# Roy-Shubhajit/FIT-GNN

Hardware: NVIDIA B200
Metric: subgraph-inference nodes/sec (higher is better)
Workload: dtype fp16 planes for every operand of the two wide transforms (aggregated features, hidden state, weights: 1 MMA per product), fp16 hidden state x fp16 hi/lo weights (2 MMAs) in the head; f32 accumulate

## Files before the change

fitgnn_b200/_lib.py:

```python
from __future__ import annotations

import ctypes as C
import os

_HERE = os.path.dirname(os.path.abspath(__file__))
LIB_PATH = os.environ.get("FITGNN_B200_LIB", os.path.join(_HERE, "libfitgnn_b200.so"))

c_i64, c_i32, c_void, c_size = C.c_int64, C.c_int, C.c_void_p, C.c_size_t


class FitgnnError(RuntimeError):
    pass


class PackStruct(C.Structure):
    _fields_ = [("n_rows", c_i64), ("nnz", c_i64), ("n_sub", c_i64), ("n_core", c_i64), ("n_src", c_i64),
                ("rowptr", c_void), ("col", c_void), ("dinv", c_void), ("gid", c_void), ("sub_ptr", c_void),
                ("core_rows", c_void), ("is_core", c_void), ("mask", c_void)]


class WeightsStruct(C.Structure):
    _fields_ = [("n_layers", C.c_int), ("in_features", C.c_int), ("hidden", C.c_int), ("n_classes", C.c_int),
                ("conv_weight", C.POINTER(c_void)), ("conv_bias", C.POINTER(c_void)), ("lt1_weight", c_void),
                ("lt1_bias", c_void)]


class PlanStruct(C.Structure):
    _fields_ = [("n_rows", c_i64), ("nnz", c_i64), ("n_sub", c_i64), ("n_core", c_i64), ("n_src", c_i64),
                ("fill_ws_bytes", c_i64), ("priv", c_i64 * 27)]


SIGNATURES = {
    "fitgnn_abi_version": (c_i32, []),
    "fitgnn_last_error": (c_i32, [C.c_char_p, c_size]),
    "fitgnn_device_info": (c_i32, [C.POINTER(c_i32), C.POINTER(c_i32)]),
    "fitgnn_tuning_set": (c_i32, [C.c_char_p, c_i32]),
    "fitgnn_tuning_get": (c_i32, [C.c_char_p, C.POINTER(c_i32)]),
    "fitgnn_csr_workspace_bytes": (c_size, [c_i64, c_i64]),
    "fitgnn_csr_plan": (c_i32, [c_void, c_i64, c_i64, c_void, c_size, C.POINTER(c_i64), c_void]),
    "fitgnn_csr_fill": (c_i32, [c_i64, c_void, c_size, c_void, c_void, c_void, c_void]),
    "fitgnn_pack_workspace_bytes": (c_size, [c_i64, c_i64, c_i64, c_i32, c_i64]),
    "fitgnn_pack_plan": (c_i32, [c_void, c_i64, c_i64, c_void, c_i64, c_i32, c_void, c_void, c_i64, c_void, c_size,
                                 C.POINTER(PlanStruct), c_void]),
    "fitgnn_pack_fill": (c_i32, [C.POINTER(PlanStruct), C.POINTER(PackStruct), c_void, c_size, c_void, c_size, c_void]),
    "fitgnn_spmm_symnorm": (c_i32, [c_void, c_void, c_void, c_void, c_i64, c_i32, c_void, c_void, c_i32, c_void, c_i64,
                                    c_void, c_void, c_i64, c_void]),
    "fitgnn_spmm_symnorm_grouped": (c_i32, [c_void, c_void, c_void, c_void, c_i64, c_i32, c_void, c_i64, c_i32, c_void,
                                            c_void, c_i64, c_i32, C.c_float, c_void]),
    "fitgnn_spmm_symnorm_grouped_f16": (c_i32, [c_void, c_void, c_void, c_void, c_i64, c_i32, c_void, c_i64, c_i32, c_void,
                                                c_i64, c_i32, C.c_float, c_void]),
    "fitgnn_spmm_symnorm_blocked": (c_i32, [c_void, c_void, c_void, c_void, c_i64, c_i32, c_void, c_void, c_i64, c_void,
                                            c_void, c_i32, c_void, c_void, c_i64, c_void]),
    "fitgnn_spmm_symnorm_mma": (c_i32, [c_void, c_void, c_void, c_void, c_i64, c_i32, c_void, c_void, c_i64, c_void,
                                        c_i32, c_void, c_void, c_i64, c_void]),
    "fitgnn_spmm_hubs": (c_i32, [c_void, c_void, c_i64, c_i32, c_void, c_void, c_i32, c_void]),
    "fitgnn_spmm_symnorm_hub": (c_i32, [c_void, c_void, c_void, c_void, c_i64, c_i32, c_void, c_void, c_i32, c_void,
                                        c_i64, c_void, c_void, c_i64, c_void, c_i32, c_i32, c_void]),
    "fitgnn_spmm_symnorm_devhub": (c_i32, [c_void, c_void, c_void, c_void, c_i64, c_i32, c_void, c_void, c_i32, c_void,
                                           c_i64, c_void, c_void, c_i64, c_void, c_void, c_i32, c_i32, c_void]),
    "fitgnn_gcn_forward_workspace_bytes": (c_size, [C.POINTER(PackStruct), C.POINTER(WeightsStruct), c_i32]),
    "fitgnn_gcn_forward": (c_i32, [C.POINTER(PackStruct), c_void, c_i64, C.POINTER(WeightsStruct), c_i32, c_i32, c_void,
                                   c_i64, c_void, c_size, c_void]),
    "fitgnn_gemm_tn_workspace_bytes": (c_size, [c_i64, c_i32, c_i32]),
    "fitgnn_gemm_tn": (c_i32, [c_void, c_i64, c_void, c_i64, c_i64, c_i32, c_i32, c_void, c_i64, c_void, c_size, c_void]),
    "fitgnn_dropout": (c_i32, [c_void, c_i64, c_i64, c_i32, C.c_float, C.c_uint64, C.c_uint64, c_void, c_i64, c_void]),
    "fitgnn_elu_dropout_backward": (c_i32, [c_void, c_i64, c_void, c_i64, c_i64, c_i32, c_i32, C.c_float, C.c_uint64,
                                            C.c_uint64, c_void, c_i64, c_void]),
    "fitgnn_adam_step": (c_i32, [c_void, c_void, c_void, c_void, c_i64, C.c_float, C.c_float, C.c_float, C.c_float,
                                 C.c_float, c_i64, c_void]),
    "fitgnn_spmm_symnorm_f16": (c_i32, [c_void, c_void, c_void, c_void, c_i64, c_i32, c_void, c_void, c_i32, c_void, c_i64,
                                        c_void, c_i64, c_void, c_void, c_i32, c_i32, c_void]),
    "fitgnn_split_f16": (c_i32, [c_void, c_i64, c_i64, c_i32, c_void, c_void, c_i64, c_void]),
    "fitgnn_gemm_f16": (c_i32, [c_void, c_i64, c_void, c_void, c_i64, c_void, c_void, c_i64, c_i32, c_i32, c_i32, c_i32, c_void,
                                c_i64, c_i32, c_void, c_void]),
    "fitgnn_gemm_f16_head_rows_peers": (c_i32, [c_void, c_i64, c_void, c_void, c_i64, c_void, c_i64, c_i32, c_i32, c_i32, c_i32,
                                                c_void, C.POINTER(c_void), c_i32, c_i64, c_void]),
    "fitgnn_gcn_transform_aggregate_f16": (c_i32, [c_i32, c_void, c_void, c_i64, c_void, c_void, c_i64, c_void, c_i64, c_i32,
                                                   c_i32, c_i32, c_void, c_void, c_i32, c_void, c_i64, c_void]),
    "fitgnn_gcn_conv_aligned_f16": (c_i32, [c_void, c_i64, c_void, c_void, c_i64, c_void, c_i64, c_i32, c_i32, c_i32, c_void, c_void,
                                            c_void, c_i64, c_void]),
    "fitgnn_gemm_bias_act": (c_i32, [c_i32, c_void, c_void, c_i64, c_void, c_void, c_i64, c_void, c_i64, c_i32, c_i32,
                                     c_i32, c_i32, c_void, c_i64, c_void]),
    "fitgnn_gemm_bias_act_split": (c_i32, [c_i32, c_void, c_void, c_i64, c_void, c_void, c_i64, c_void, c_i64, c_i32,
                                           c_i32, c_i32, c_i32, c_void, c_void, c_i64, c_void]),
    "fitgnn_gcn_layer_fused": (c_i32, [c_void, c_void, c_void, c_void, c_i64, c_i32, c_void, c_void, c_i64, c_void, c_void,
                                       c_i64, c_void, c_i32, c_i32, c_void, c_void, c_i64, c_void]),
    "fitgnn_pack_align_workspace_bytes": (c_size, [c_i64, c_i64]),
    "fitgnn_pack_align_plan": (c_i32, [C.POINTER(PackStruct), c_i32, c_i32, c_void, C.POINTER(c_i64), C.POINTER(c_i32),
                                       c_void, c_size, c_void]),
    "fitgnn_pack_align_fill": (c_i32, [C.POINTER(PackStruct), c_void, c_i32, c_i64, C.POINTER(PackStruct), c_void, c_void,
                                       c_void, C.POINTER(c_i32), c_void, c_size, c_void]),
    "fitgnn_gcn_transform_aggregate": (c_i32, [c_void, c_void, c_i64, c_void, c_void, c_i64, c_void, c_i64, c_i32, c_i32,
                                               c_i32, c_void, c_void, c_i32, c_void, c_void, c_i64, c_void]),
    "fitgnn_gemm_rowscale_bias_act_split": (c_i32, [c_i32, c_void, c_void, c_i64, c_void, c_void, c_i64, c_void, c_void, c_i64,
                                                    c_i32, c_i32, c_i32, c_i32, c_void, c_void, c_i64, c_void]),
    "fitgnn_gemm_head_rows": (c_i32, [c_void, c_void, c_i64, c_void, c_void, c_i64, c_void, c_i64, c_i32, c_i32, c_i32,
                                      c_i32, c_void, c_void, c_i64, c_void]),
    "fitgnn_gemm_head_rows_peers": (c_i32, [c_void, c_void, c_i64, c_void, c_void, c_i64, c_void, c_i64, c_i32, c_i32, c_i32,
                                            c_i32, c_void, C.POINTER(c_void), c_i32, c_i64, c_void]),
    "fitgnn_peer_push": (c_i32, [c_void, C.POINTER(c_void), c_i32, c_size, c_i32, c_void]),
    "fitgnn_peer_alloc": (c_i32, [c_size, C.POINTER(c_void), C.c_char_p]),
    "fitgnn_peer_open": (c_i32, [C.c_char_p, C.POINTER(c_void)]),
    "fitgnn_peer_close": (c_i32, [c_void]),
    "fitgnn_peer_free": (c_i32, [c_void]),
    "fitgnn_split_bf16": (c_i32, [c_void, c_i64, c_i64, c_i32, c_void, c_void, c_i64, c_void]),
    "fitgnn_segment_pool": (c_i32, [c_void, c_i64, c_i32, c_void, c_void, c_i64, c_i32, c_void, c_i64, c_void]),
    "fitgnn_group_workspace_bytes": (c_size, [c_i64, c_i64]),
    "fitgnn_group_by_part": (c_i32, [c_void, c_i64, c_i64, c_void, c_void, c_void, c_size, c_void]),
    "fitgnn_project_features": (c_i32, [c_void, c_void, c_i64, c_void, c_void, c_i64, c_i32, c_void, c_i64, c_void]),
    "fitgnn_project_adj_workspace_bytes": (c_size, [c_i64]),
    "fitgnn_project_adj_plan": (c_i32, [c_void, c_i64, c_i64, c_void, c_i64, c_void, c_size, C.POINTER(c_i64), c_void]),
    "fitgnn_project_adj_fill": (c_i32, [c_void, c_size, c_i64, c_void, c_void, c_void, c_void, c_void]),
    "fitgnn_sort_workspace_bytes": (c_size, [c_i64]),
    "fitgnn_sort_u64": (c_i32, [c_void, c_void, c_i64, c_i32, c_void, c_size, c_void]),
    "fitgnn_scan_i32": (c_i32, [c_void, c_void, c_i64, c_i32, c_void, c_size, c_void]),
    "fitgnn_scan_workspace_bytes": (c_size, [c_i64]),
}

_lib = None


def lib():
    global _lib
    if _lib is None:
        if not os.path.exists(LIB_PATH):
            raise FitgnnError(
                f"{LIB_PATH} is missing: build it with `python -c 'import __graft_entry__ as g; g.build()'` "
                "(or `make -C fitgnn_b200/csrc`). fitgnn_b200 has no CPU fallback.")
        handle = C.CDLL(LIB_PATH)
        for name, (res, args) in SIGNATURES.items():
            fn = getattr(handle, name)
            fn.restype, fn.argtypes = res, args
        if handle.fitgnn_abi_version() != 1:
            raise FitgnnError("libfitgnn_b200.so ABI version mismatch")
        _lib = handle
    return _lib


def last_error() -> str:
    buf = C.create_string_buffer(512)
    lib().fitgnn_last_error(buf, 512)
    return buf.value.decode(errors="replace")


def set_tuning(name: str, value: int) -> int:
    old = C.c_int(0)
    check(lib().fitgnn_tuning_get(name.encode(), C.byref(old)))
    check(lib().fitgnn_tuning_set(name.encode(), int(value)))
    return old.value


_CODES = {-1: "EINVAL", -2: "ECUDA", -3: "ERANGE", -4: "EWS", -5: "EUNSUP"}


def check(rc: int):
    if rc != 0:
        raise FitgnnError(f"fitgnn {_CODES.get(rc, rc)}: {last_error()}")


def ptr(t):
    if t is None:
        return None
    if not t.is_cuda:
        raise FitgnnError("fitgnn_b200 kernels take CUDA tensors only (there is no CPU path)")
    if not t.is_contiguous():
        raise FitgnnError("tensor must be contiguous")
    return C.c_void_p(t.data_ptr())


def stream_ptr():
    import torch
    return C.c_void_p(torch.cuda.current_stream().cuda_stream)
```

fitgnn_b200/csrc/capi.cu:

```cuda
#include <stdarg.h>
#include <stdio.h>
#include <stdlib.h>
#include <string.h>
#include "common.cuh"

namespace fitgnn {

static thread_local char g_err[512] = "";

void set_error(const char* fmt, ...) {
  va_list ap;
  va_start(ap, fmt);
  vsnprintf(g_err, sizeof(g_err), fmt, ap);
  va_end(ap);
}

int sm_count() {
  static int cached[64] = {};
  int dev = 0;
  if (cudaGetDevice(&dev) != cudaSuccess || dev < 0 || dev >= 64) return 148;
  if (!cached[dev]) {
    int n = 0;
    if (cudaDeviceGetAttribute(&n, cudaDevAttrMultiProcessorCount, dev) != cudaSuccess || n <= 0) n = 148;
    cached[dev] = n;
  }
  return cached[dev];
}

static int env_int(const char* name, int dflt) {
  const char* e = getenv(name);
  return (e && e[0]) ? atoi(e) : dflt;
}
static Tuning& tuning_mut() {
  static Tuning t{env_int("FITGNN_GEMM_WS", 1),   getenv("FITGNN_HEAD_BULK") ? 0 : 1, env_int("FITGNN_AGG_WIDE", 0),
                  env_int("FITGNN_GEMM_WIDE", 0), env_int("FITGNN_GEMM_PAIR", 1), env_int("FITGNN_SM_RESERVE", 0),
                  env_int("FITGNN_GEMM_PAIR_WS", 1), 0, env_int("FITGNN_GEMM_PREFETCH", 0)};
  return t;
}
const Tuning& tuning() { return tuning_mut(); }
static int* tuning_field(const char* name) {
  Tuning& t = tuning_mut();
  if (!name) return nullptr;
  if (!strcmp(name, "gemm_ws")) return &t.gemm_ws;
  if (!strcmp(name, "head_bulk")) return &t.head_bulk;
  if (!strcmp(name, "agg_wide")) return &t.agg_wide;
  if (!strcmp(name, "gemm_wide")) return &t.gemm_wide;
  if (!strcmp(name, "gemm_pair")) return &t.gemm_pair;
  if (!strcmp(name, "sm_reserve")) return &t.sm_reserve;
  if (!strcmp(name, "gemm_pair_ws")) return &t.gemm_pair_ws;
  if (!strcmp(name, "gemm_prefetch")) return &t.gemm_prefetch;
  if (!strcmp(name, "gemm_debug")) return &t.gemm_debug;
  return nullptr;
}

int gemm_fp32(const float* A, int64_t lda, const float* W, int64_t ldw, const float* bias, int64_t M, int K, int N,
              int act, float* Y, int64_t ldy, cudaStream_t st);
int row_softmax(float* Y, int64_t ldy, int64_t M, int N, int head, cudaStream_t st);
int gemm_bf16x3(const void* A_hi, const void* A_lo, int64_t lda, const void* W_hi, const void* W_lo, int64_t ldw,
                const float* bias, int64_t M, int K, int N, int act, int head, float* Y, void* Y_lo, int64_t ldy,
                const uint64_t* agg_desc, const float* agg_dinv, const int32_t* row_map, float* const* peers, int n_peers,
                const float* row_scale, int agg_defer_scale, cudaStream_t st, int64_t m_batch_rows = 0, int w_batch_rows = 0,
                int64_t w_rows_total = 0, int in_f16 = 0, int out_f16 = 0, int agg_pre = 0);

int gcn_layer_fused(const int32_t* rowptr, const int32_t* col, const float* dinv, const float* X, int64_t ldx, int width,
                    const int32_t* src_index, const int32_t* out_rows, int64_t M, const void* W_hi, const void* W_lo,
                    int64_t ldw, const float* bias, int N, int act, float* Y, void* Y_lo, int64_t ldy, cudaStream_t st);

}

using namespace fitgnn;

extern "C" int fitgnn_abi_version(void) { return FITGNN_ABI_VERSION; }

extern "C" int fitgnn_last_error(char* buf, size_t n) {
  const size_t len = strlen(g_err);
  if (buf && n > 0) {
    const size_t c = len < n - 1 ? len : n - 1;
    memcpy(buf, g_err, c);
    buf[c] = 0;
  }
  return (int)len;
}

extern "C" int fitgnn_tuning_set(const char* name, int value) {
  int* f = tuning_field(name);
  FG_REQUIRE(f, FITGNN_EINVAL, "tuning_set: unknown switch '%s'", name ? name : "(null)");
  *f = value;
  return FITGNN_OK;
}
extern "C" int fitgnn_tuning_get(const char* name, int* value) {
  int* f = tuning_field(name);
  FG_REQUIRE(f && value, FITGNN_EINVAL, "tuning_get: unknown switch '%s'", name ? name : "(null)");
  *value = *f;
  return FITGNN_OK;
}

extern "C" int fitgnn_device_info(int* sm_count, int* cc) {
  int dev = 0;
  FG_CUDA(cudaGetDevice(&dev));
  cudaDeviceProp p;
  FG_CUDA(cudaGetDeviceProperties(&p, dev));
  if (sm_count) *sm_count = p.multiProcessorCount;
  if (cc) *cc = p.major * 10 + p.minor;
  return FITGNN_OK;
}

extern "C" int fitgnn_gemm_rowscale_bias_act_split(int precision, const void* A, const void* A_lo, int64_t lda,
                                                   const void* W, const void* W_lo, int64_t ldw, const float* row_scale,
                                                   const float* bias, int64_t M, int K, int N, int act, int head, void* Yv,
                                                   void* Y_lo, int64_t ldy, void* stream) {
  float* Y = static_cast<float*>(Yv);
  FG_REQUIRE(!row_scale || precision == FITGNN_GEMM_BF16X3, FITGNN_EUNSUP, "gemm: row_scale needs FITGNN_GEMM_BF16X3");
  FG_REQUIRE(A && W && Y && M >= 0 && K > 0 && N > 0, FITGNN_EINVAL, "gemm: bad arguments (M=%lld K=%d N=%d)",
             (long long)M, K, N);
  FG_REQUIRE(lda >= K && ldw >= K && ldy >= N, FITGNN_EINVAL, "gemm: leading dimension smaller than the extent");
  FG_REQUIRE(act == FITGNN_ACT_NONE || act == FITGNN_ACT_ELU, FITGNN_EINVAL, "gemm: unknown act %d", act);
  FG_REQUIRE(head >= FITGNN_HEAD_IDENTITY && head <= FITGNN_HEAD_SOFTMAX, FITGNN_EINVAL, "gemm: unknown head %d", head);
  if (M == 0) return FITGNN_OK;
  cudaStream_t st = as_stream(stream);
  if (precision == FITGNN_GEMM_FP32) {
    FG_REQUIRE(!Y_lo, FITGNN_EUNSUP, "gemm: bf16 hi/lo output planes need FITGNN_GEMM_BF16X3");
    FG_TRY(gemm_fp32(static_cast<const float*>(A), lda, static_cast<const float*>(W), ldw, bias, M, K, N, act, Y, ldy,
                     st));
    return row_softmax(Y, ldy, M, N, head, st);
  }
  if (precision == FITGNN_GEMM_BF16X3) {
    FG_REQUIRE(A_lo && W_lo, FITGNN_EINVAL, "gemm: BF16X3 needs the lo planes");
    return gemm_bf16x3(A, A_lo, lda, W, W_lo, ldw, bias, M, K, N, act, head, Y, Y_lo, ldy, nullptr, nullptr, nullptr, nullptr, 0,
                       row_scale, 0, st);
  }
  set_error("gemm: unknown precision %d", precision);
  return FITGNN_EINVAL;
}

extern "C" int fitgnn_gemm_bias_act_split(int precision, const void* A, const void* A_lo, int64_t lda, const void* W,
                                          const void* W_lo, int64_t ldw, const float* bias, int64_t M, int K, int N,
                                          int act, int head, void* Yv, void* Y_lo, int64_t ldy, void* stream) {
  return fitgnn_gemm_rowscale_bias_act_split(precision, A, A_lo, lda, W, W_lo, ldw, nullptr, bias, M, K, N, act, head, Yv, Y_lo,
                                             ldy, stream);
}

extern "C" int fitgnn_gcn_transform_aggregate(const void* A_hi, const void* A_lo, int64_t lda, const void* W_hi,
                                              const void* W_lo, int64_t ldw, const float* bias, int64_t M, int K, int N,
                                              int act, const uint64_t* agg_desc, const float* dinv, int defer_row_scale,
                                              void* Y, void* Y_lo, int64_t ldy, void* stream) {
  FG_REQUIRE(A_hi && A_lo && W_hi && W_lo && Y && agg_desc && dinv && M >= 0 && K > 0 && N > 0, FITGNN_EINVAL,
             "gcn_transform_aggregate: bad arguments (M=%lld K=%d N=%d)", (long long)M, K, N);
  FG_REQUIRE(lda >= K && ldw >= K && ldy >= N, FITGNN_EINVAL, "gcn_transform_aggregate: leading dimension too small");
  FG_REQUIRE(act == FITGNN_ACT_NONE || act == FITGNN_ACT_ELU, FITGNN_EINVAL, "gcn_transform_aggregate: unknown act %d", act);
  if (M == 0) return FITGNN_OK;
  return gemm_bf16x3(A_hi, A_lo, lda, W_hi, W_lo, ldw, bias, M, K, N, act, FITGNN_HEAD_IDENTITY, static_cast<float*>(Y),
                     Y_lo, ldy, agg_desc, dinv, nullptr, nullptr, 0, nullptr, defer_row_scale, as_stream(stream));
}

extern "C" int fitgnn_gemm_head_rows(const void* A_hi, const void* A_lo, int64_t lda, const void* W_hi, const void* W_lo,
                                     int64_t ldw, const float* bias, int64_t M, int K, int N, int act, int head,
                                     const int32_t* row_map, float* Y, int64_t ldy, void* stream) {
  FG_REQUIRE(A_hi && A_lo && W_hi && W_lo && Y && row_map && M >= 0 && K > 0 && N > 0, FITGNN_EINVAL,
             "gemm_head_rows: bad arguments (M=%lld K=%d N=%d)", (long long)M, K, N);
  FG_REQUIRE(lda >= K && ldw >= K && ldy >= N, FITGNN_EINVAL, "gemm_head_rows: leading dimension too small");
  FG_REQUIRE(act == FITGNN_ACT_NONE || act == FITGNN_ACT_ELU, FITGNN_EINVAL, "gemm_head_rows: unknown act %d", act);
  FG_REQUIRE(head >= FITGNN_HEAD_IDENTITY && head <= FITGNN_HEAD_SOFTMAX, FITGNN_EINVAL, "gemm_head_rows: unknown head %d",
             head);
  if (M == 0) return FITGNN_OK;
  return gemm_bf16x3(A_hi, A_lo, lda, W_hi, W_lo, ldw, bias, M, K, N, act, head, Y, nullptr, ldy, nullptr, nullptr,
                     row_map, nullptr, 0, nullptr, 0, as_stream(stream));
}

extern "C" int fitgnn_gemm_head_rows_peers(const void* A_hi, const void* A_lo, int64_t lda, const void* W_hi,
                                           const void* W_lo, int64_t ldw, const float* bias, int64_t M, int K, int N,
                                           int act, int head, const int32_t* row_map, float* const* host_peer_bases,
                                           int n_peers, int64_t ldy, void* stream) {
  FG_REQUIRE(A_hi && A_lo && W_hi && W_lo && row_map && host_peer_bases && M >= 0 && K > 0 && N > 0, FITGNN_EINVAL,
             "gemm_head_rows_peers: bad arguments (M=%lld K=%d N=%d)", (long long)M, K, N);
  FG_REQUIRE(n_peers >= 1 && n_peers <= 8, FITGNN_EINVAL, "gemm_head_rows_peers: 1..8 peers (got %d)", n_peers);
  for (int p = 0; p < n_peers; ++p)
    FG_REQUIRE(host_peer_bases[p], FITGNN_EINVAL, "gemm_head_rows_peers: peer base %d is null", p);
  FG_REQUIRE(lda >= K && ldw >= K && ldy >= N, FITGNN_EINVAL, "gemm_head_rows_peers: leading dimension too small");
  FG_REQUIRE(act == FITGNN_ACT_NONE || act == FITGNN_ACT_ELU, FITGNN_EINVAL, "gemm_head_rows_peers: unknown act %d", act);
  FG_REQUIRE(head >= FITGNN_HEAD_IDENTITY && head <= FITGNN_HEAD_SOFTMAX, FITGNN_EINVAL,
             "gemm_head_rows_peers: unknown head %d", head);
  if (M == 0) return FITGNN_OK;
  return gemm_bf16x3(A_hi, A_lo, lda, W_hi, W_lo, ldw, bias, M, K, N, act, head, nullptr, nullptr, ldy, nullptr, nullptr,
                     row_map, host_peer_bases, n_peers, nullptr, 0, as_stream(stream));
}

extern "C" int fitgnn_gemm_bias_act(int precision, const void* A, const void* A_lo, int64_t lda, const void* W,
                                    const void* W_lo, int64_t ldw, const float* bias, int64_t M, int K, int N, int act,
                                    int head, float* Y, int64_t ldy, void* stream) {
  return fitgnn_gemm_bias_act_split(precision, A, A_lo, lda, W, W_lo, ldw, bias, M, K, N, act, head, Y, nullptr, ldy,
                                    stream);
}

extern "C" int fitgnn_gcn_layer_fused(const int32_t* rowptr, const int32_t* col, const float* dinv, const float* X,
                                      int64_t ldx, int width, const int32_t* src_index, const int32_t* out_rows,
                                      int64_t n_out, const void* W_hi, const void* W_lo, int64_t ldw, const float* bias,
                                      int N, int act, void* Y, void* Y_lo, int64_t ldy, void* stream) {
  FG_REQUIRE(rowptr && col && dinv && X && W_hi && W_lo && Y && n_out >= 0 && N > 0 && width > 0, FITGNN_EINVAL,
             "gcn_layer_fused: bad arguments");
  FG_REQUIRE(act == FITGNN_ACT_NONE || act == FITGNN_ACT_ELU, FITGNN_EINVAL, "gcn_layer_fused: unknown act %d", act);
  if (n_out == 0) return FITGNN_OK;
  return gcn_layer_fused(rowptr, col, dinv, X, ldx, width, src_index, out_rows, n_out, W_hi, W_lo, ldw, bias, N, act,
                         static_cast<float*>(Y), Y_lo, ldy, as_stream(stream));
}

extern "C" int fitgnn_gemm_f16(const void* A, int64_t lda, const void* W_hi, const void* W_lo, int64_t ldw,
                               const float* row_scale, const float* bias, int64_t M, int K, int N, int act, int head, void* Y,
                               int64_t ldy, int out_f16, const int32_t* row_map, void* stream) {
  FG_REQUIRE(A && W_hi && Y && M >= 0 && K > 0 && N > 0, FITGNN_EINVAL, "gemm_f16: bad arguments (M=%lld K=%d N=%d)",
             (long long)M, K, N);
  FG_REQUIRE(lda >= K && ldw >= K && ldy >= N, FITGNN_EINVAL, "gemm_f16: leading dimension smaller than the extent");
  FG_REQUIRE(act == FITGNN_ACT_NONE || act == FITGNN_ACT_ELU, FITGNN_EINVAL, "gemm_f16: unknown act %d", act);
  FG_REQUIRE(head >= FITGNN_HEAD_IDENTITY && head <= FITGNN_HEAD_SOFTMAX, FITGNN_EINVAL, "gemm_f16: unknown head %d", head);
  if (M == 0) return FITGNN_OK;
  return gemm_bf16x3(A, nullptr, lda, W_hi, W_lo, ldw, bias, M, K, N, act, head, static_cast<float*>(Y), nullptr, ldy, nullptr,
                     nullptr, row_map, nullptr, 0, row_scale, 0, as_stream(stream), 0, 0, 0, 1, out_f16 ? 1 : 0);
}

extern "C" int fitgnn_gcn_transform_aggregate_f16(int in_f16, const void* A_hi, const void* A_lo, int64_t lda, const void* W_hi,
                                                  const void* W_lo, int64_t ldw, const float* bias, int64_t M, int K, int N,
                                                  int act, const uint64_t* agg_desc, const float* dinv, int defer_row_scale,
                                                  void* Y, int64_t ldy, void* stream) {
  FG_REQUIRE(A_hi && W_hi && (W_lo || in_f16) && Y && (!agg_desc || dinv) && M >= 0 && K > 0 && N > 0, FITGNN_EINVAL,
             "gcn_transform_aggregate_f16: bad arguments (M=%lld K=%d N=%d)", (long long)M, K, N);
  FG_REQUIRE(in_f16 ? !A_lo : A_lo != nullptr, FITGNN_EINVAL, "gcn_transform_aggregate_f16: A_lo must match in_f16");
  FG_REQUIRE(lda >= K && ldw >= K && ldy >= N, FITGNN_EINVAL, "gcn_transform_aggregate_f16: leading dimension too small");
  FG_REQUIRE(act == FITGNN_ACT_NONE || act == FITGNN_ACT_ELU, FITGNN_EINVAL, "gcn_transform_aggregate_f16: unknown act %d", act);
  if (M == 0) return FITGNN_OK;
  return gemm_bf16x3(A_hi, A_lo, lda, W_hi, W_lo, ldw, bias, M, K, N, act, FITGNN_HEAD_IDENTITY, static_cast<float*>(Y), nullptr,
                     ldy, agg_desc, agg_desc ? dinv : nullptr, nullptr, nullptr, 0, nullptr, agg_desc ? defer_row_scale : 0,
                     as_stream(stream), 0, 0, 0, in_f16 ? 1 : 0, 1);
}

extern "C" int fitgnn_gcn_conv_aligned_f16(const void* A, int64_t lda, const void* W_hi, const void* W_lo, int64_t ldw,
                                           const float* bias, int64_t M, int K, int N, int act, const uint64_t* agg_desc,
                                           const float* dinv, void* Y, int64_t ldy, void* stream) {
  FG_REQUIRE(A && W_hi && Y && agg_desc && dinv && M >= 0 && K > 0 && N > 0, FITGNN_EINVAL,
             "gcn_conv_aligned_f16: bad arguments (M=%lld K=%d N=%d)", (long long)M, K, N);
  FG_REQUIRE(lda >= K && ldw >= K && ldy >= N, FITGNN_EINVAL, "gcn_conv_aligned_f16: leading dimension too small");
  FG_REQUIRE(act == FITGNN_ACT_NONE || act == FITGNN_ACT_ELU, FITGNN_EINVAL, "gcn_conv_aligned_f16: unknown act %d", act);
  if (M == 0) return FITGNN_OK;
  return gemm_bf16x3(A, nullptr, lda, W_hi, W_lo, ldw, bias, M, K, N, act, FITGNN_HEAD_IDENTITY, static_cast<float*>(Y), nullptr,
                     ldy, agg_desc, dinv, nullptr, nullptr, 0, dinv, 1, as_stream(stream), 0, 0, 0, 1, 1, 1);
}

extern "C" int fitgnn_gemm_f16_head_rows_peers(const void* A, int64_t lda, const void* W_hi, const void* W_lo, int64_t ldw,
                                               const float* bias, int64_t M, int K, int N, int act, int head,
                                               const int32_t* row_map, float* const* host_peer_bases, int n_peers, int64_t ldy,
                                               void* stream) {
  FG_REQUIRE(A && W_hi && W_lo && row_map && host_peer_bases && M >= 0 && K > 0 && N > 0, FITGNN_EINVAL,
             "gemm_f16_head_rows_peers: bad arguments (M=%lld K=%d N=%d)", (long long)M, K, N);
  FG_REQUIRE(n_peers >= 1 && n_peers <= 8, FITGNN_EINVAL, "gemm_f16_head_rows_peers: 1..8 peers (got %d)", n_peers);
  for (int p = 0; p < n_peers; ++p)
    FG_REQUIRE(host_peer_bases[p], FITGNN_EINVAL, "gemm_f16_head_rows_peers: peer base %d is null", p);
  FG_REQUIRE(lda >= K && ldw >= K && ldy >= N, FITGNN_EINVAL, "gemm_f16_head_rows_peers: leading dimension too small");
  FG_REQUIRE(act == FITGNN_ACT_NONE || act == FITGNN_ACT_ELU, FITGNN_EINVAL, "gemm_f16_head_rows_peers: unknown act %d", act);
  FG_REQUIRE(head >= FITGNN_HEAD_IDENTITY && head <= FITGNN_HEAD_SOFTMAX, FITGNN_EINVAL,
             "gemm_f16_head_rows_peers: unknown head %d", head);
  if (M == 0) return FITGNN_OK;
  return gemm_bf16x3(A, nullptr, lda, W_hi, W_lo, ldw, bias, M, K, N, act, head, nullptr, nullptr, ldy, nullptr, nullptr, row_map,
                     host_peer_bases, n_peers, nullptr, 0, as_stream(stream), 0, 0, 0, 1, 0);
}
```

fitgnn_b200/csrc/gemm_tcgen05.cu:

```cuda
#include <cuda.h>
#include <stdio.h>
#include <stdlib.h>
#include <cuda_bf16.h>
#include <type_traits>
#include "common.cuh"

namespace fitgnn {

namespace tc {

constexpr int BLOCK_M = 128;
constexpr int BLOCK_K = 64;
constexpr int UMMA_K = 16;
constexpr int EPI_WARPS = 8;
constexpr int EPI_WARPS_WIDE = 16;
constexpr int EPI_WARPS_12 = 12;
constexpr int THREADS = 64 + 32 * EPI_WARPS;
constexpr int GATHER_WARPS = 4;
constexpr int GATHER_WARP0 = 2 + EPI_WARPS;
constexpr int THREADS_GATHER = THREADS + 32 * GATHER_WARPS;

struct GatherArgs {
  const int32_t* rowptr;
  const int32_t* col;
  const float* dinv;
  const float* X;
  const int32_t* src_index;
  const int32_t* out_rows;
  int64_t ldx;
  int nq;
};
struct EpiArgs {
  const unsigned long long* agg_desc;
  const float* agg_dinv;
  const int32_t* row_map;
  float* peers[8];
  int n_peers;
  int bulk_rows;
  const float* row_scale;
  int agg_defer_scale;
  int64_t m_batch_rows;
  int w_batch_rows;
  int64_t w_rows_total;
  int a_planes;
  int f16;
  int out_f16;
  int w_planes;
  int l2_prefetch;
  int debug;
};
constexpr int EPI_WARP0 = 2;
constexpr int ACC_STAGES = 2;
constexpr uint32_t A_PLANE_BYTES = BLOCK_M * BLOCK_K * 2;
constexpr long long WAIT_BUDGET_CYCLES = 4000000000ll;

__device__ __forceinline__ uint32_t smem_u32(const void* p) { return (uint32_t)__cvta_generic_to_shared(p); }

__device__ __forceinline__ void mbar_init(uint32_t bar, uint32_t count) {
  asm volatile("mbarrier.init.shared::cta.b64 [%0], %1;" ::"r"(bar), "r"(count));
}
__device__ __forceinline__ void mbar_arrive(uint32_t bar) {
  asm volatile("mbarrier.arrive.shared::cta.b64 _, [%0];" ::"r"(bar) : "memory");
}
__device__ __forceinline__ void mbar_arrive_expect_tx(uint32_t bar, uint32_t bytes) {
  asm volatile("mbarrier.arrive.expect_tx.shared::cta.b64 _, [%0], %1;" ::"r"(bar), "r"(bytes) : "memory");
}
__device__ __forceinline__ bool mbar_try_wait(uint32_t bar, uint32_t parity) {
  uint32_t ok;
  asm volatile(
      "{\n\t.reg .pred p;\n\t"
      "mbarrier.try_wait.parity.shared::cta.b64 p, [%1], %2;\n\t"
      "selp.u32 %0, 1, 0, p;\n\t}"
      : "=r"(ok)
      : "r"(bar), "r"(parity)
      : "memory");
  return ok != 0;
}
__device__ __forceinline__ void mbar_wait(uint32_t bar, uint32_t parity) {
  if (mbar_try_wait(bar, parity)) return;
  const long long t0 = clock64();
  while (!mbar_try_wait(bar, parity)) {
    if (clock64() - t0 > WAIT_BUDGET_CYCLES) {
      printf("fitgnn gemm_bf16x3: mbarrier wait timed out (block %d thread %d)\n", blockIdx.x, threadIdx.x);
      __trap();
    }
  }
}

__device__ __forceinline__ void tma_load_2d(uint32_t dst, const CUtensorMap* map, uint32_t bar, int c0, int c1) {
  asm volatile(
      "cp.async.bulk.tensor.2d.shared::cluster.global.mbarrier::complete_tx::bytes [%0], [%1, {%3, %4}], [%2];"
      ::"r"(dst), "l"(map), "r"(bar), "r"(c0), "r"(c1)
      : "memory");
}

__device__ __forceinline__ void tma_prefetch_2d(const CUtensorMap* map, int c0, int c1) {
  asm volatile("cp.async.bulk.prefetch.tensor.2d.L2.global [%0, {%1, %2}];" ::"l"(map), "r"(c0), "r"(c1) : "memory");
}

__device__ __forceinline__ void tma_store_2d(const CUtensorMap* map, uint32_t src, int c0, int c1) {
  asm volatile("cp.async.bulk.tensor.2d.global.shared::cta.bulk_group [%0, {%2, %3}], [%1];" ::"l"(map), "r"(src),
               "r"(c0), "r"(c1)
               : "memory");
}
__device__ __forceinline__ void bulk_store_1d(void* dst, uint32_t src, uint32_t bytes) {
  asm volatile("cp.async.bulk.global.shared::cta.bulk_group [%0], [%1], %2;" ::"l"(dst), "r"(src), "r"(bytes) : "memory");
}
__device__ __forceinline__ void bulk_commit() { asm volatile("cp.async.bulk.commit_group;" ::: "memory"); }
template <int N>
__device__ __forceinline__ void bulk_wait_read() {
  asm volatile("cp.async.bulk.wait_group.read %0;" ::"n"(N) : "memory");
}
__device__ __forceinline__ void bulk_wait_all() { asm volatile("cp.async.bulk.wait_group 0;" ::: "memory"); }
__device__ __forceinline__ void fence_proxy_async() { asm volatile("fence.proxy.async.shared::cta;" ::: "memory"); }

__device__ __forceinline__ uint64_t umma_desc_sw128(uint32_t smem_addr) {
  uint64_t d = 0;
  d |= (uint64_t)((smem_addr & 0x3FFFFu) >> 4);
  d |= (uint64_t)0 << 16;
  d |= (uint64_t)(1024u >> 4) << 32;
  d |= (uint64_t)1 << 46;
  d |= (uint64_t)2 << 61;
  return d;
}

__host__ __device__ constexpr uint32_t umma_idesc_bf16(int m, int n) {
  return (1u << 4) | (1u << 7) | (1u << 10) | ((uint32_t)(n >> 3) << 17) | ((uint32_t)(m >> 4) << 24);
}

__host__ __device__ constexpr uint32_t umma_idesc_f16(int m, int n) {
  return (1u << 4) | ((uint32_t)(n >> 3) << 17) | ((uint32_t)(m >> 4) << 24);
}

__device__ __forceinline__ void umma_bf16(uint32_t tmem_d, uint64_t a_desc, uint64_t b_desc, uint32_t idesc,
                                          uint32_t accumulate) {
  asm volatile(
      "{\n\t.reg .pred p;\n\t"
      "setp.ne.b32 p, %4, 0;\n\t"
      "tcgen05.mma.cta_group::1.kind::f16 [%0], %1, %2, %3, p;\n\t}"
      ::"r"(tmem_d), "l"(a_desc), "l"(b_desc), "r"(idesc), "r"(accumulate)
      : "memory");
}
__device__ __forceinline__ uint32_t cluster_ctarank() {
  uint32_t r;
  asm volatile("mov.u32 %0, %%cluster_ctarank;" : "=r"(r));
  return r;
}
__device__ __forceinline__ uint32_t mapa_rank(uint32_t local_addr, uint32_t rank) {
  uint32_t r;
  asm volatile("mapa.shared::cluster.u32 %0, %1, %2;" : "=r"(r) : "r"(local_addr), "r"(rank));
  return r;
}
__device__ __forceinline__ void cluster_sync_all() {
  asm volatile("barrier.cluster.arrive.release.aligned;" ::: "memory");
  asm volatile("barrier.cluster.wait.acquire.aligned;" ::: "memory");
}
__device__ __forceinline__ void tma_load_2d_pair(uint32_t dst, const CUtensorMap* map, uint32_t leader_bar, int c0, int c1) {
  asm volatile(
      "cp.async.bulk.tensor.2d.cta_group::2.shared::cluster.global.mbarrier::complete_tx::bytes [%0], [%1, {%3, %4}], [%2];"
      ::"r"(dst), "l"(map), "r"(leader_bar), "r"(c0), "r"(c1)
      : "memory");
}
__device__ __forceinline__ void umma_bf16_pair(uint32_t tmem_d, uint64_t a_desc, uint64_t b_desc, uint32_t idesc,
                                               uint32_t accumulate) {
  asm volatile(
      "{\n\t.reg .pred p;\n\t"
      "setp.ne.b32 p, %4, 0;\n\t"
      "tcgen05.mma.cta_group::2.kind::f16 [%0], %1, %2, %3, p;\n\t}"
      ::"r"(tmem_d), "l"(a_desc), "l"(b_desc), "r"(idesc), "r"(accumulate)
      : "memory");
}
__device__ __forceinline__ void umma_commit_pair(uint32_t bar) {
  const uint16_t mask = 3;
  asm volatile("tcgen05.commit.cta_group::2.mbarrier::arrive::one.shared::cluster.multicast::cluster.b64 [%0], %1;" ::"r"(bar),
               "h"(mask)
               : "memory");
}
__device__ __forceinline__ void mbar_arrive_remote(uint32_t cluster_addr) {
  asm volatile("mbarrier.arrive.shared::cluster.b64 _, [%0];" ::"r"(cluster_addr) : "memory");
}
__device__ __forceinline__ bool elect_one() {
  uint32_t pred;
  asm volatile("{\n\t.reg .pred p;\n\telect.sync _|p, 0xffffffff;\n\tselp.b32 %0, 1, 0, p;\n\t}" : "=r"(pred));
  return pred != 0;
}
__device__ __forceinline__ void umma_commit(uint32_t bar) {
  asm volatile("tcgen05.commit.cta_group::1.mbarrier::arrive::one.shared::cluster.b64 [%0];" ::"r"(bar) : "memory");
}
__device__ __forceinline__ void tmem_ld16(uint32_t taddr, float (&v)[16]) {
  uint32_t r[16];
  asm volatile(
      "tcgen05.ld.sync.aligned.32x32b.x16.b32 {%0,%1,%2,%3,%4,%5,%6,%7,%8,%9,%10,%11,%12,%13,%14,%15}, [%16];"
      : "=r"(r[0]), "=r"(r[1]), "=r"(r[2]), "=r"(r[3]), "=r"(r[4]), "=r"(r[5]), "=r"(r[6]), "=r"(r[7]), "=r"(r[8]),
        "=r"(r[9]), "=r"(r[10]), "=r"(r[11]), "=r"(r[12]), "=r"(r[13]), "=r"(r[14]), "=r"(r[15])
      : "r"(taddr));
  asm volatile("tcgen05.wait::ld.sync.aligned;" ::: "memory");
#pragma unroll
  for (int i = 0; i < 16; ++i) v[i] = __uint_as_float(r[i]);
}
__device__ __forceinline__ void tmem_ld32(uint32_t taddr, float (&v)[32]) {
  uint32_t r[32];
  asm volatile(
      "tcgen05.ld.sync.aligned.32x32b.x32.b32 {%0,%1,%2,%3,%4,%5,%6,%7,%8,%9,%10,%11,%12,%13,%14,%15,%16,%17,%18,%19,"
      "%20,%21,%22,%23,%24,%25,%26,%27,%28,%29,%30,%31}, [%32];"
      : "=r"(r[0]), "=r"(r[1]), "=r"(r[2]), "=r"(r[3]), "=r"(r[4]), "=r"(r[5]), "=r"(r[6]), "=r"(r[7]), "=r"(r[8]),
        "=r"(r[9]), "=r"(r[10]), "=r"(r[11]), "=r"(r[12]), "=r"(r[13]), "=r"(r[14]), "=r"(r[15]), "=r"(r[16]),
        "=r"(r[17]), "=r"(r[18]), "=r"(r[19]), "=r"(r[20]), "=r"(r[21]), "=r"(r[22]), "=r"(r[23]), "=r"(r[24]),
        "=r"(r[25]), "=r"(r[26]), "=r"(r[27]), "=r"(r[28]), "=r"(r[29]), "=r"(r[30]), "=r"(r[31])
      : "r"(taddr));
  asm volatile("tcgen05.wait::ld.sync.aligned;" ::: "memory");
#pragma unroll
  for (int i = 0; i < 32; ++i) v[i] = __uint_as_float(r[i]);
}
__device__ __forceinline__ void tmem_ld32_issue(uint32_t taddr, uint32_t (&r)[32]) {
  asm volatile(
      "tcgen05.ld.sync.aligned.32x32b.x32.b32 {%0,%1,%2,%3,%4,%5,%6,%7,%8,%9,%10,%11,%12,%13,%14,%15,%16,%17,%18,%19,"
      "%20,%21,%22,%23,%24,%25,%26,%27,%28,%29,%30,%31}, [%32];"
      : "=r"(r[0]), "=r"(r[1]), "=r"(r[2]), "=r"(r[3]), "=r"(r[4]), "=r"(r[5]), "=r"(r[6]), "=r"(r[7]), "=r"(r[8]),
        "=r"(r[9]), "=r"(r[10]), "=r"(r[11]), "=r"(r[12]), "=r"(r[13]), "=r"(r[14]), "=r"(r[15]), "=r"(r[16]),
        "=r"(r[17]), "=r"(r[18]), "=r"(r[19]), "=r"(r[20]), "=r"(r[21]), "=r"(r[22]), "=r"(r[23]), "=r"(r[24]),
        "=r"(r[25]), "=r"(r[26]), "=r"(r[27]), "=r"(r[28]), "=r"(r[29]), "=r"(r[30]), "=r"(r[31])
      : "r"(taddr));
}
__device__ __forceinline__ void tmem_ld32_wait(uint32_t (&r)[32]) {
  asm volatile("tcgen05.wait::ld.sync.aligned;"
               : "+r"(r[0]), "+r"(r[1]), "+r"(r[2]), "+r"(r[3]), "+r"(r[4]), "+r"(r[5]), "+r"(r[6]), "+r"(r[7]), "+r"(r[8]),
                 "+r"(r[9]), "+r"(r[10]), "+r"(r[11]), "+r"(r[12]), "+r"(r[13]), "+r"(r[14]), "+r"(r[15]), "+r"(r[16]),
                 "+r"(r[17]), "+r"(r[18]), "+r"(r[19]), "+r"(r[20]), "+r"(r[21]), "+r"(r[22]), "+r"(r[23]), "+r"(r[24]),
                 "+r"(r[25]), "+r"(r[26]), "+r"(r[27]), "+r"(r[28]), "+r"(r[29]), "+r"(r[30]), "+r"(r[31])
               :
               : "memory");
}
__device__ __forceinline__ void fence_before() { asm volatile("tcgen05.fence::before_thread_sync;" ::: "memory"); }
__device__ __forceinline__ void fence_after() { asm volatile("tcgen05.fence::after_thread_sync;" ::: "memory"); }

__device__ __forceinline__ float elu1(float x) { return elu_fast(x); }

__host__ __device__ constexpr int tmem_cols(int n) { return n <= 32 ? 32 : n <= 64 ? 64 : n <= 128 ? 128 : n <= 256 ? 256 : 512; }
__host__ __device__ constexpr uint32_t stage_bytes(int block_n) { return 2 * A_PLANE_BYTES + 2 * (uint32_t)block_n * BLOCK_K * 2; }
constexpr uint32_t EPI_BOX_BYTES = 32 * 32 * 4;
__host__ __device__ constexpr int num_stages(int block_n) {
  int s = (int)((192 * 1024) / stage_bytes(block_n));
  return s > 8 ? 8 : s;
}

template <int BLOCK_N, bool GATHER, int AGG, int EW, bool CTA2 = false>
__global__ void __launch_bounds__(64 + 32 * EW + (GATHER ? 32 * GATHER_WARPS : 0), 1)
gemm_bf16x3_kernel(const GatherArgs ga, const EpiArgs ea, const __grid_constant__ CUtensorMap map_a_hi, const __grid_constant__ CUtensorMap map_a_lo,
                   const __grid_constant__ CUtensorMap map_w_hi, const __grid_constant__ CUtensorMap map_w_lo,
                   const __grid_constant__ CUtensorMap map_y, const __grid_constant__ CUtensorMap map_y_lo,
                   int tma_store, const float* __restrict__ bias, int64_t M, int K, int N, int act, int head,
                   float* __restrict__ Y, int64_t ldy, int w_stationary, int n_stages) {
  constexpr int STAGES = num_stages(BLOCK_N);
  constexpr int MAX_STAGES = 8;
  constexpr int B_ROWS = CTA2 ? BLOCK_N / 2 : BLOCK_N;
  constexpr uint32_t B_PLANE_BYTES = (uint32_t)B_ROWS * BLOCK_K * 2;
  constexpr int TMEM_COLS = tmem_cols(ACC_STAGES * BLOCK_N);
  constexpr uint32_t IDESC_BF16 = umma_idesc_bf16(CTA2 ? 2 * BLOCK_M : BLOCK_M, BLOCK_N);
  constexpr uint32_t IDESC_F16 = umma_idesc_f16(CTA2 ? 2 * BLOCK_M : BLOCK_M, BLOCK_N);
  const uint32_t IDESC = ea.f16 ? IDESC_F16 : IDESC_BF16;
  const bool a_single = ea.a_planes == 1;
  const bool w_single = ea.w_planes == 1;
  static_assert(!CTA2 || (!GATHER && BLOCK_N % 32 == 0), "CTA pairs: streaming plan, UMMA N multiple of 32 for M=256");
  const uint32_t cta_rank = CTA2 ? cluster_ctarank() : 0u;
  const bool leader = cta_rank == 0;
  static_assert(BLOCK_N % 16 == 0 && BLOCK_N >= 16 && BLOCK_N <= 256, "UMMA N for M=128");
  static_assert(STAGES >= 2, "need at least two smem stages");
  static_assert(EW == EPI_WARPS || (EW == EPI_WARPS_WIDE && !GATHER) || (EW == EPI_WARPS_12 && !GATHER && BLOCK_N == 256),
                "2, 3 (256-column tile with an fp16-plane output) or 4 epilogue warps per TMEM lane quadrant");
  constexpr bool HALF_STAGE = BLOCK_N == 256 && (EW == EPI_WARPS_12 || (AGG && EW == EPI_WARPS_WIDE));
  const uint32_t WARP_STAGE = (HALF_STAGE || (CTA2 && ea.out_f16)) ? EPI_BOX_BYTES / 2 : EPI_BOX_BYTES;
  const uint32_t STAGING_BYTES = EW * WARP_STAGE;

  extern __shared__ uint8_t smem_raw[];
  uint8_t* smem = reinterpret_cast<uint8_t*>(((uintptr_t)smem_raw + 1023) & ~(uintptr_t)1023);
  const int k_blocks = (K + BLOCK_K - 1) / BLOCK_K;
  const uint32_t b_bytes = (w_single ? 1u : 2u) * B_PLANE_BYTES;
  const uint32_t w_region_bytes = w_stationary ? (uint32_t)k_blocks * b_bytes : 0u;
  const uint32_t a_bytes = (a_single ? 1u : 2u) * A_PLANE_BYTES;
  const uint32_t stage_bytes_rt = w_stationary ? a_bytes : a_bytes + b_bytes;
  uint8_t* staging = smem + w_region_bytes + (size_t)n_stages * stage_bytes_rt;
  uint64_t* bars = reinterpret_cast<uint64_t*>(staging + STAGING_BYTES);
  uint32_t* tmem_slot = reinterpret_cast<uint32_t*>(bars + 2 * MAX_STAGES + 2 * ACC_STAGES + 1);
  const uint32_t smem_base = smem_u32(smem) + w_region_bytes;
  const uint32_t w_base = smem_u32(smem);
  const uint32_t bar_base = smem_u32(bars);
  auto full_bar = [&](int s) { return bar_base + 8u * s; };
  auto empty_bar = [&](int s) { return bar_base + 8u * (MAX_STAGES + s); };
  auto tfull_bar = [&](int s) { return bar_base + 8u * (2 * MAX_STAGES + s); };
  auto tempty_bar = [&](int s) { return bar_base + 8u * (2 * MAX_STAGES + ACC_STAGES + s); };
  const uint32_t wfull_bar = bar_base + 8u * (2 * MAX_STAGES + 2 * ACC_STAGES);

  const int warp = threadIdx.x >> 5, lane = threadIdx.x & 31;
  const int n_tiles = (N + BLOCK_N - 1) / BLOCK_N;
  constexpr int TILE_M = CTA2 ? 2 * BLOCK_M : BLOCK_M;
  const int64_t m_tiles = (M + TILE_M - 1) / TILE_M;
  const int64_t tiles = m_tiles * n_tiles;
  struct Walk { int mb, nt; };
  const int ctas_per_n = (int)gridDim.x / n_tiles;
  Walk w0;
  int walk_dm, walk_dn, walk_carry;
  if (CTA2) {
    const int p = (int)(blockIdx.x >> 1), np = (int)(gridDim.x >> 1);
    if (w_stationary) { w0 = Walk{p / n_tiles, p % n_tiles}; walk_dm = np / n_tiles; walk_dn = 0; walk_carry = 0; }
    else { w0 = Walk{p, 0}; walk_dm = 0; walk_dn = 1; walk_carry = np; }
  } else if (w_stationary) {
    w0 = Walk{(int)blockIdx.x / n_tiles, (int)blockIdx.x % n_tiles}; walk_dm = ctas_per_n; walk_dn = 0; walk_carry = 0;
  } else {
    w0 = Walk{(int)blockIdx.x / n_tiles, (int)blockIdx.x % n_tiles};
    walk_dm = (int)gridDim.x / n_tiles; walk_dn = (int)gridDim.x % n_tiles; walk_carry = 1;
  }
  auto advance = [&](Walk& w) {
    w.nt += walk_dn;
    w.mb += walk_dm;
    if (w.nt >= n_tiles) { w.nt -= n_tiles; w.mb += walk_carry; }
  };
  auto valid = [&](const Walk& w) { return (int64_t)w.mb < m_tiles; };
  auto tile_row0 = [&](const Walk& w) { return (int64_t)w.mb * TILE_M + (int64_t)cta_rank * BLOCK_M; };
  auto w_batch_off = [&](const Walk& w) -> int {
    return ea.m_batch_rows ? (int)(((int64_t)w.mb * TILE_M) / ea.m_batch_rows) * ea.w_batch_rows : 0;
  };
  const int64_t t_first = blockIdx.x;
  const int64_t t_step = (int64_t)ctas_per_n * n_tiles;

  if (warp == 0 && lane == 0) {
    for (int s = 0; s < n_stages; ++s) {
      mbar_init(full_bar(s), GATHER ? GATHER_WARPS : 1);
      mbar_init(empty_bar(s), 1);
    }
    mbar_init(wfull_bar, 1);
    for (int s = 0; s < ACC_STAGES; ++s) {
      mbar_init(tfull_bar(s), 1);
      mbar_init(tempty_bar(s), CTA2 ? 2 * EW : EW);
    }
    asm volatile("fence.mbarrier_init.release.cluster;" ::: "memory");
  }
  if (warp == 1) {
    if (CTA2) {
      asm volatile("tcgen05.alloc.cta_group::2.sync.aligned.shared::cta.b32 [%0], %1;" ::"r"(smem_u32(tmem_slot)),
                   "r"((uint32_t)TMEM_COLS)
                   : "memory");
      asm volatile("tcgen05.relinquish_alloc_permit.cta_group::2.sync.aligned;" ::: "memory");
    } else {
      asm volatile("tcgen05.alloc.cta_group::1.sync.aligned.shared::cta.b32 [%0], %1;" ::"r"(smem_u32(tmem_slot)),
                   "r"((uint32_t)TMEM_COLS)
                   : "memory");
      asm volatile("tcgen05.relinquish_alloc_permit.cta_group::1.sync.aligned;" ::: "memory");
    }
  }
  fence_before();
  __syncthreads();
  if (CTA2) cluster_sync_all();
  fence_after();
  const uint32_t tmem_base = *tmem_slot;

  if (warp == 0) {
    {
      uint32_t stage = 0, phase = 0;
      if (w_stationary && valid(w0)) {
        const int n0 = w0.nt * BLOCK_N;
        if (elect_one()) {
          if (CTA2) {
            const uint32_t lbar = mapa_rank(wfull_bar, 0);
            if (leader) mbar_arrive_expect_tx(wfull_bar, 2 * w_region_bytes);
            for (int kb = 0; kb < k_blocks; ++kb) {
              tma_load_2d_pair(w_base + kb * b_bytes, &map_w_hi, lbar, kb * BLOCK_K, n0 + (int)cta_rank * B_ROWS);
              if (!w_single)
                tma_load_2d_pair(w_base + kb * b_bytes + B_PLANE_BYTES, &map_w_lo, lbar, kb * BLOCK_K, n0 + (int)cta_rank * B_ROWS);
            }
          } else {
            mbar_arrive_expect_tx(wfull_bar, w_region_bytes);
            for (int kb = 0; kb < k_blocks; ++kb) {
              tma_load_2d(w_base + kb * b_bytes, &map_w_hi, wfull_bar, kb * BLOCK_K, n0);
              if (!w_single) tma_load_2d(w_base + kb * b_bytes + B_PLANE_BYTES, &map_w_lo, wfull_bar, kb * BLOCK_K, n0);
            }
          }
        }
        __syncwarp();
      }
      int prev_mb = -1;
      for (Walk w = w0; valid(w) && !GATHER; advance(w)) {
        const int m0 = (int)tile_row0(w);
        const int n0 = w.nt * BLOCK_N + w_batch_off(w);
        int pf_m0 = -1;
        if (w.mb != prev_mb) {
          Walk pf = w;
          for (int i = 0; i < n_tiles && valid(pf) && pf.mb == w.mb; ++i) advance(pf);
          if (valid(pf) && pf.mb != w.mb) pf_m0 = (int)tile_row0(pf);
        }
        prev_mb = w.mb;
        for (int kb = 0; kb < k_blocks; ++kb) {
          if (pf_m0 >= 0 && ea.l2_prefetch) {
            if (elect_one()) {
              tma_prefetch_2d(&map_a_hi, kb * BLOCK_K, pf_m0);
              if (!a_single) tma_prefetch_2d(&map_a_lo, kb * BLOCK_K, pf_m0);
            }
            __syncwarp();
          }
          mbar_wait(empty_bar(stage), phase ^ 1);
          const uint32_t dst = smem_base + stage * stage_bytes_rt;
          const uint32_t tx_bytes = stage_bytes_rt;
          __syncwarp();
          if (elect_one()) {
            if (CTA2) {
              const uint32_t lbar = mapa_rank(full_bar(stage), 0);
              if (leader) mbar_arrive_expect_tx(full_bar(stage), 2 * tx_bytes);
              tma_load_2d_pair(dst, &map_a_hi, lbar, kb * BLOCK_K, m0);
              if (!a_single) tma_load_2d_pair(dst + A_PLANE_BYTES, &map_a_lo, lbar, kb * BLOCK_K, m0);
              if (!w_stationary) {
                tma_load_2d_pair(dst + a_bytes, &map_w_hi, lbar, kb * BLOCK_K, n0 + (int)cta_rank * B_ROWS);
                if (!w_single)
                  tma_load_2d_pair(dst + a_bytes + B_PLANE_BYTES, &map_w_lo, lbar, kb * BLOCK_K, n0 + (int)cta_rank * B_ROWS);
              }
            } else {
              mbar_arrive_expect_tx(full_bar(stage), tx_bytes);
              tma_load_2d(dst, &map_a_hi, full_bar(stage), kb * BLOCK_K, m0);
              if (!a_single) tma_load_2d(dst + A_PLANE_BYTES, &map_a_lo, full_bar(stage), kb * BLOCK_K, m0);
              if (!w_stationary) {
                tma_load_2d(dst + a_bytes, &map_w_hi, full_bar(stage), kb * BLOCK_K, n0);
                if (!w_single) tma_load_2d(dst + a_bytes + B_PLANE_BYTES, &map_w_lo, full_bar(stage), kb * BLOCK_K, n0);
              }
            }
          }
          __syncwarp();
          if (++stage == (uint32_t)n_stages) { stage = 0; phase ^= 1; }
        }
      }
    }
  } else if (warp == 1) {
    auto mma_loop = [&](auto a1_t, auto w1_t) {
      constexpr bool A1 = decltype(a1_t)::value, W1 = decltype(w1_t)::value;
      uint32_t stage = 0, phase = 0;
      uint32_t it = 0;
      if (w_stationary && valid(w0)) mbar_wait(wfull_bar, 0);
      for (Walk w = w0; valid(w); ++it, advance(w)) {
        const uint32_t acc = it % ACC_STAGES;
        const uint32_t acc_phase = (it / ACC_STAGES) & 1u;
        mbar_wait(tempty_bar(acc), acc_phase ^ 1);
        fence_after();
        const uint32_t tmem_d = tmem_base + acc * BLOCK_N;
        for (int kb = 0; kb < k_blocks; ++kb) {
          mbar_wait(full_bar(stage), phase);
          fence_after();
          const uint32_t a_hi = smem_base + stage * stage_bytes_rt;
          const uint32_t w_hi = w_stationary ? w_base + kb * b_bytes : a_hi + a_bytes;
          const uint64_t d_a_hi = umma_desc_sw128(a_hi);
          const uint64_t d_a_lo = umma_desc_sw128(a_hi + A_PLANE_BYTES);
          const uint64_t d_w_hi = umma_desc_sw128(w_hi);
          const uint64_t d_w_lo = umma_desc_sw128(w_hi + B_PLANE_BYTES);
          __syncwarp();
          if (elect_one()) {
#pragma unroll
            for (int k = 0; k < BLOCK_K / UMMA_K; ++k) {
              const uint64_t adv = (uint64_t)((k * UMMA_K * 2) >> 4);
              if (CTA2) {
                umma_bf16_pair(tmem_d, d_a_hi + adv, d_w_hi + adv, IDESC, (kb | k) != 0);
                if (!A1) umma_bf16_pair(tmem_d, d_a_lo + adv, d_w_hi + adv, IDESC, 1);
                if (!W1) umma_bf16_pair(tmem_d, d_a_hi + adv, d_w_lo + adv, IDESC, 1);
              } else {
                umma_bf16(tmem_d, d_a_hi + adv, d_w_hi + adv, IDESC, (kb | k) != 0);
                if (!A1) umma_bf16(tmem_d, d_a_lo + adv, d_w_hi + adv, IDESC, 1);
                if (!W1) umma_bf16(tmem_d, d_a_hi + adv, d_w_lo + adv, IDESC, 1);
              }
            }
            if (CTA2) {
              umma_commit_pair(empty_bar(stage));
              if (kb == k_blocks - 1) umma_commit_pair(tfull_bar(acc));
            } else {
              umma_commit(empty_bar(stage));
              if (kb == k_blocks - 1) umma_commit(tfull_bar(acc));
            }
          }
          __syncwarp();
          if (++stage == (uint32_t)n_stages) { stage = 0; phase ^= 1; }
        }
      }
    };
    if (leader) {
      if (a_single && w_single) mma_loop(std::true_type{}, std::true_type{});
      else if (a_single) mma_loop(std::true_type{}, std::false_type{});
      else mma_loop(std::false_type{}, std::false_type{});
    }
    __syncwarp();
  } else if (GATHER && warp >= GATHER_WARP0) {
    constexpr int LPR = 8, STEPS = BLOCK_M / (GATHER_WARPS * 4);
    constexpr unsigned FULL = 0xffffffffu;
    const int gw = warp - GATHER_WARP0, sub = lane & (LPR - 1), grp = lane / LPR;
    const int64_t my_tiles = (t_first < tiles) ? (tiles - 1 - t_first) / t_step + 1 : 0;
    const int64_t total_steps = my_tiles * STEPS;
    struct RI { int beg, end; float dr; };
    auto load_info = [&](int64_t step) {
      RI ri{0, 0, 0.f};
      if (step < total_steps) {
        const int64_t t = t_first + (step / STEPS) * t_step;
        const int64_t i = (t / n_tiles) * BLOCK_M + gw * 32 + (int)(step % STEPS) * 4 + grp;
        if (i < M) {
          const int r = ga.out_rows ? __ldg(ga.out_rows + i) : (int)i;
          ri.beg = __ldg(ga.rowptr + r);
          ri.end = __ldg(ga.rowptr + r + 1);
          ri.dr = __ldg(ga.dinv + r);
        }
      }
      return ri;
    };
    auto load_col = [&](const RI& ri, int e0) { return (e0 + sub < ri.end) ? __ldg(ga.col + e0 + sub) : -1; };
    auto load_w = [&](int c) { return c >= 0 ? __ldg(ga.dinv + c) : 0.f; };
    auto load_s = [&](int c) { return c >= 0 ? (ga.src_index ? __ldg(ga.src_index + c) : c) : 0; };
    auto gather_chunk = [&](float4 (&acc)[4], int cnt, float w, int sidx) {
      const int maxcnt = __reduce_max_sync(FULL, cnt);
      for (int j = 0; j < maxcnt; j += 2) {
        float wj[2];
        const float* pj[2];
        bool on[2];
#pragma unroll
        for (int u = 0; u < 2; ++u) {
          wj[u] = __shfl_sync(FULL, w, j + u, LPR);
          const int sj = __shfl_sync(FULL, sidx, j + u, LPR);
          pj[u] = ga.X + (int64_t)sj * ga.ldx;
          on[u] = j + u < cnt;
        }
        float4 x[2][4];
#pragma unroll
        for (int u = 0; u < 2; ++u)
#pragma unroll
          for (int v = 0; v < 4; ++v) {
            const int q = sub + LPR * v;
            x[u][v] = (on[u] && q < ga.nq) ? __ldg(reinterpret_cast<const float4*>(pj[u]) + q) : make_float4(0.f, 0.f, 0.f, 0.f);
          }
#pragma unroll
        for (int u = 0; u < 2; ++u)
#pragma unroll
          for (int v = 0; v < 4; ++v) {
            acc[v].x = fmaf(wj[u], x[u][v].x, acc[v].x); acc[v].y = fmaf(wj[u], x[u][v].y, acc[v].y);
            acc[v].z = fmaf(wj[u], x[u][v].z, acc[v].z); acc[v].w = fmaf(wj[u], x[u][v].w, acc[v].w);
          }
      }
    };
    RI ia = load_info(0), ib = load_info(1), ic = load_info(2);
    int ca = load_col(ia, ia.beg), cb = load_col(ib, ib.beg);
    float wa = load_w(ca);
    int sa = load_s(ca);
    uint32_t stage = 0, phase = 0;
    for (int64_t step = 0; step < total_steps; ++step) {
      const RI id = load_info(step + 3);
      const int cc = load_col(ic, ic.beg);
      const float wb = load_w(cb);
      const int sb = load_s(cb);
      const int s_in_tile = (int)(step % STEPS);
      if (s_in_tile == 0) {
        if (lane == 0)
          for (int kb = 0; kb < k_blocks; ++kb) mbar_wait(empty_bar(stage + kb), phase ^ 1);
        __syncwarp();
      }
      const int deg = ia.end - ia.beg;
      float4 acc[4];
#pragma unroll
      for (int v = 0; v < 4; ++v) acc[v] = make_float4(0.f, 0.f, 0.f, 0.f);
      gather_chunk(acc, min(deg, LPR), wa, sa);
      const bool long_row = deg > LPR;
      for (int e0 = ia.beg + LPR; __any_sync(FULL, long_row && e0 < ia.end); e0 += LPR) {
        const int c = long_row ? load_col(ia, e0) : -1;
        gather_chunk(acc, long_row ? max(0, min(ia.end - e0, LPR)) : 0, load_w(c), load_s(c));
      }
      const int lr = gw * 32 + s_in_tile * 4 + grp;
#pragma unroll
      for (int v = 0; v < 4; ++v) {
        const int c = 4 * (sub + LPR * v);
        const int kb = c >> 6;
        if (kb < k_blocks) {
          const float x[4] = {acc[v].x * ia.dr, acc[v].y * ia.dr, acc[v].z * ia.dr, acc[v].w * ia.dr};
          uint32_t hi[2], lo[2];
#pragma unroll
          for (int u = 0; u < 2; ++u) split_bf16x2(x[2 * u], x[2 * u + 1], hi[u], lo[u]);
          const int cc64 = c & 63;
          const uint32_t a = smem_base + (stage + kb) * stage_bytes_rt + lr * 128 +
                             ((uint32_t)(cc64 >> 3) ^ (uint32_t)(lr & 7)) * 16 + ((cc64 & 7) >> 2) * 8;
          asm volatile("st.shared.v2.b32 [%0], {%1, %2};" ::"r"(a), "r"(hi[0]), "r"(hi[1]) : "memory");
          asm volatile("st.shared.v2.b32 [%0], {%1, %2};" ::"r"(a + A_PLANE_BYTES), "r"(lo[0]), "r"(lo[1]) : "memory");
        }
      }
      if (s_in_tile == STEPS - 1) {
        fence_proxy_async();
        __syncwarp();
        if (lane == 0)
          for (int kb = 0; kb < k_blocks; ++kb) mbar_arrive(full_bar(stage + kb));
        stage += k_blocks;
        if (stage >= (uint32_t)n_stages) { stage = 0; phase ^= 1; }
      }
      ia = ib; ib = ic; ic = id;
      ca = cb; cb = cc;
      wa = wb; sa = sb;
    }
  } else {
    const int quad = warp & 3;
    const int row_in_tile = quad * 32 + lane;
    bool vec_ok = (ldy % 4 == 0) && (((uintptr_t)Y & 15) == 0);
#pragma unroll
    for (int p = 0; p < 8; ++p)
      if (p < ea.n_peers) vec_ok = vec_ok && (((uintptr_t)ea.peers[p] & 15) == 0);
    const bool bias_vec = (((uintptr_t)bias & 15) == 0);
    constexpr int N_BOXES = (BLOCK_N + 31) / 32;
    constexpr bool FAST_HEAD = N_BOXES <= 2 && EW == EPI_WARPS;
    const bool use_fast_head = FAST_HEAD && head != FITGNN_HEAD_IDENTITY;
    float2* exch = reinterpret_cast<float2*>(reinterpret_cast<uint8_t*>(bars) + 256);
    const int ew = warp - EPI_WARP0;
    const int col_group = ew >> 2;
    constexpr int GROUPS = EW / 4;
    constexpr int BOXES_PER_GROUP = (N_BOXES + GROUPS - 1) / GROUPS;
    const bool one_group = head != FITGNN_HEAD_IDENTITY && !FAST_HEAD;
    const int box_beg = one_group ? (col_group == 0 ? 0 : N_BOXES) : min(N_BOXES, col_group * BOXES_PER_GROUP);
    const int box_end = one_group ? N_BOXES : min(N_BOXES, box_beg + BOXES_PER_GROUP);
    uint32_t it = 0;
    unsigned long long desc_next = 0ull;
    float dr_next = 0.f, rs_next = 1.f;
    auto load_agg = [&](const Walk& wt) {
      desc_next = 0ull;
      dr_next = 0.f;
      rs_next = 1.f;
      if ((AGG || ea.row_scale) && valid(wt)) {
        const int64_t mm = tile_row0(wt) + row_in_tile;
        if (mm < M) {
          if (AGG) {
            desc_next = __ldg(ea.agg_desc + mm);
            dr_next = __ldg(ea.agg_dinv + mm);
          }
          if (ea.row_scale) rs_next = __ldg(ea.row_scale + mm);
        }
      }
    };
    load_agg(w0);
    Walk w_next = w0;
    for (Walk w = w0; valid(w); ++it, w = w_next) {
      const uint32_t acc = it % ACC_STAGES;
      const uint32_t acc_phase = (it / ACC_STAGES) & 1u;
      const int64_t tile_m0 = tile_row0(w);
      const int64_t m = tile_m0 + row_in_tile;
      const int n0 = w.nt * BLOCK_N;
      const unsigned long long desc = desc_next;
      const float dr = dr_next;
      const float rs = rs_next;
      advance(w_next);
      load_agg(w_next);
      const int agg_cnt = (int)(desc & 15ull);
      const int agg_max = AGG ? __reduce_max_sync(0xffffffffu, agg_cnt) : 0;
      mbar_wait(tfull_bar(acc), acc_phase);
      fence_after();
      const uint32_t taddr = tmem_base + ((uint32_t)(quad * 32) << 16) + acc * BLOCK_N;
      const int64_t dest_row = (ea.row_map && m < M) ? (int64_t)__ldg(ea.row_map + m) : m;
      float* yrow = Y + dest_row * ldy + n0;
      float row_max = -INFINITY, row_sum = 0.f;
      bool exchanged = false, staged = false;
      const bool bulk_rows = FAST_HEAD && ea.bulk_rows != 0;
      const uint32_t qbuf = smem_u32(staging) + (uint32_t)quad * 2u * EPI_BOX_BYTES;
      const uint32_t row_bytes = (uint32_t)ldy * 4u;
      auto stage_and_store = [&](const float (&vals)[32], bool have, int c0, int ncols) {
        if (col_group == 0 && lane == 0) bulk_wait_read<0>();
        asm volatile("bar.sync %0, 64;" ::"r"(1 + quad) : "memory");
        if (have) {
#pragma unroll
          for (int j = 0; j < 32; j += 4) {
            if (j < ncols && c0 + j < (int)ldy) {
              const float x0 = (n0 + c0 + j < N) ? vals[j] : 0.f, x1 = (n0 + c0 + j + 1 < N) ? vals[j + 1] : 0.f;
              const float x2 = (n0 + c0 + j + 2 < N) ? vals[j + 2] : 0.f, x3 = (n0 + c0 + j + 3 < N) ? vals[j + 3] : 0.f;
              asm volatile("st.shared.v4.f32 [%0], {%1, %2, %3, %4};" ::"r"(qbuf + lane * row_bytes + (uint32_t)(c0 + j) * 4u),
                           "f"(x0), "f"(x1), "f"(x2), "f"(x3) : "memory");
            }
          }
        }
        fence_proxy_async();
        asm volatile("bar.sync %0, 64;" ::"r"(1 + quad) : "memory");
        if (col_group == 0) {
          const int dr_ = (m < M) ? (int)dest_row : -1;
          const int prev = __shfl_up_sync(0xffffffffu, dr_, 1);
          const unsigned valid = __ballot_sync(0xffffffffu, dr_ >= 0);
          const unsigned starts = __ballot_sync(0xffffffffu, dr_ >= 0 && (lane == 0 || prev < 0 || dr_ != prev + 1));
          unsigned rem = starts;
          while (rem) {
            const int s0 = __ffs(rem) - 1;
            rem &= rem - 1;
            const unsigned stop = (rem | ~valid) & ~((2u << s0) - 1u);
            const int s1 = stop ? __ffs(stop) - 1 : 32;
            const int d0 = __shfl_sync(0xffffffffu, dr_, s0);
            if (lane == 0) {
              const int n_dst = ea.n_peers > 0 ? ea.n_peers : 1;
#pragma unroll
              for (int p = 0; p < 8; ++p) {
                if (p < n_dst) {
                  float* base = ea.n_peers > 0 ? ea.peers[p] : Y;
                  bulk_store_1d(base + (int64_t)d0 * ldy, qbuf + (uint32_t)s0 * row_bytes, (uint32_t)(s1 - s0) * row_bytes);
                }
              }
            }
          }
          if (lane == 0) bulk_commit();
        }
        staged = true;
      };
      auto exchange_stats = [&](float lmax, float lsum) {
        float2* mine = exch + ((it & 1) * EW + ew) * 32 + lane;
        const float2* theirs = exch + ((it & 1) * EW + (ew ^ 4)) * 32 + lane;
        *mine = make_float2(lmax, lsum);
        asm volatile("bar.sync %0, 64;" ::"r"(1 + quad) : "memory");
        const float2 o = *theirs;
        row_max = fmaxf(lmax, o.x);
        row_sum = (lsum > 0.f ? lsum * __expf(lmax - row_max) : 0.f) + (o.y > 0.f ? o.y * __expf(o.x - row_max) : 0.f);
        exchanged = true;
      };
      if (head != FITGNN_HEAD_IDENTITY && !FAST_HEAD && col_group == 0) {
        for (int c0 = 0; c0 < BLOCK_N; c0 += 16) {
          float v[16];
          tmem_ld16(taddr + c0, v);
#pragma unroll
          for (int j = 0; j < 16; ++j) {
            const int n = n0 + c0 + j;
            if (n < N) {
              float x = v[j] + (bias ? __ldg(bias + n) : 0.f);
              if (act == FITGNN_ACT_ELU) x = elu1(x);
              const float nm = fmaxf(row_max, x);
              row_sum = row_sum * __expf(row_max - nm) + __expf(x - nm);
              row_max = nm;
            }
          }
        }
      }
      float log_sum = 0.f, inv_sum = 0.f;
      if (head != FITGNN_HEAD_IDENTITY && !FAST_HEAD) {
        log_sum = logf(row_sum);
        inv_sum = 1.f / row_sum;
      }
      const uint32_t buf = smem_u32(staging) + (uint32_t)(warp - EPI_WARP0) * WARP_STAGE;
      const int m_base = (int)tile_m0 + quad * 32;
      for (int box = box_beg; box < box_end; ++box) {
        const int c0 = box * 32;
        if (n0 + c0 >= N) break;
        const int box_cols = (BLOCK_N - c0 >= 32) ? 32 : 16;
        float v[32];
        constexpr bool BIAS_PRE = !(AGG && EW != EPI_WARPS);
        const bool bias_full = bias && bias_vec && n0 + c0 + 32 <= N;
        const bool bias_pre = BIAS_PRE && bias_full;
        float4 bq[8];
        auto bias4 = [&](int j) -> float4 {
          return BIAS_PRE ? bq[j >> 2] : __ldg(reinterpret_cast<const float4*>(bias + n0 + c0 + j));
        };
        if (box_cols == 32) {
          uint32_t r[32];
          tmem_ld32_issue(taddr + c0, r);
          if (bias_pre) {
#pragma unroll
            for (int j = 0; j < 8; ++j) bq[j] = __ldg(reinterpret_cast<const float4*>(bias + n0 + c0) + j);
          }
          tmem_ld32_wait(r);
#pragma unroll
          for (int j = 0; j < 32; ++j) v[j] = __uint_as_float(r[j]);
        } else {
          if (bias_pre) {
#pragma unroll
            for (int j = 0; j < 8; ++j) bq[j] = __ldg(reinterpret_cast<const float4*>(bias + n0 + c0) + j);
          }
          float lo16[16];
          tmem_ld16(taddr + c0, lo16);
#pragma unroll
          for (int j = 0; j < 16; ++j) { v[j] = lo16[j]; v[16 + j] = 0.f; }
        }
        auto aggregate = [&](float (&v)[32]) {
#ifndef FG_AGG_W12
#define FG_AGG_W12 32
#endif
          constexpr int AGG_W = EW == EPI_WARPS_WIDE ? 16 : EW == EPI_WARPS_12 ? FG_AGG_W12 : 32;
#pragma unroll
          for (int h0 = 0; h0 < 32; h0 += AGG_W) {
            float u[AGG_W];
#pragma unroll
            for (int j = 0; j < AGG_W; ++j) {
              u[j] = v[h0 + j] * dr;
              v[h0 + j] = u[j];
            }
            for (int sl = 0; sl < agg_max; ++sl) {
              const bool on = sl < agg_cnt;
              const int src = on ? (int)((desc >> (4 + 5 * sl)) & 31ull) : lane;
#pragma unroll
              for (int j = 0; j < AGG_W; ++j) {
                const float tv = __shfl_sync(0xffffffffu, u[j], src);
                if (on) v[h0 + j] += tv;
              }
            }
            if (!ea.agg_defer_scale) {
#pragma unroll
              for (int j = 0; j < AGG_W; ++j) v[h0 + j] *= dr;
            }
          }
        };
        if (AGG == 2) aggregate(v);
        if (ea.row_scale) {
          if (bias_full) {
#pragma unroll
            for (int j = 0; j < 32; j += 4) {
              const float4 b4 = bias4(j);
              v[j] = fmaf(v[j], rs, b4.x); v[j + 1] = fmaf(v[j + 1], rs, b4.y);
              v[j + 2] = fmaf(v[j + 2], rs, b4.z); v[j + 3] = fmaf(v[j + 3], rs, b4.w);
            }
          } else {
#pragma unroll
            for (int j = 0; j < 32; ++j) v[j] = fmaf(v[j], rs, (bias && n0 + c0 + j < N) ? __ldg(bias + n0 + c0 + j) : 0.f);
          }
        } else if (bias) {
          if (bias_full) {
#pragma unroll
            for (int j = 0; j < 32; j += 4) {
              const float4 b4 = bias4(j);
              v[j] += b4.x; v[j + 1] += b4.y; v[j + 2] += b4.z; v[j + 3] += b4.w;
            }
          } else {
#pragma unroll
            for (int j = 0; j < 32; ++j)
              if (n0 + c0 + j < N) v[j] += __ldg(bias + n0 + c0 + j);
          }
        }
        if (act == FITGNN_ACT_ELU) {
#pragma unroll
          for (int j = 0; j < 32; ++j) v[j] = elu1(v[j]);
        }
        if (AGG == 1) aggregate(v);
        if (use_fast_head) {
          float lmax = -INFINITY, lsum = 0.f;
#pragma unroll
          for (int j = 0; j < 32; ++j)
            if (j < box_cols && n0 + c0 + j < N) lmax = fmaxf(lmax, v[j]);
#pragma unroll
          for (int j = 0; j < 32; ++j)
            if (j < box_cols && n0 + c0 + j < N) lsum += __expf(v[j] - lmax);
          exchange_stats(lmax, lsum);
          log_sum = logf(row_sum);
          inv_sum = 1.f / row_sum;
        }
        if (head == FITGNN_HEAD_LOG_SOFTMAX) {
#pragma unroll
          for (int j = 0; j < 32; ++j) v[j] = v[j] - row_max - log_sum;
        } else if (head == FITGNN_HEAD_SOFTMAX) {
#pragma unroll
          for (int j = 0; j < 32; ++j) v[j] = __expf(v[j] - row_max) * inv_sum;
        }
        if (bulk_rows) {
          stage_and_store(v, true, c0, box_cols);
        } else if (tma_store) {
          if (elect_one()) bulk_wait_read<0>();
          __syncwarp();
          if (tma_store == 3) {
#pragma unroll
            for (int j = 0; j < 4; ++j) {
              uint32_t h[4];
#pragma unroll
              for (int u = 0; u < 4; ++u) h[u] = pack_f16x2_rn(v[8 * j + 2 * u], v[8 * j + 2 * u + 1]);
              const uint32_t a = buf + lane * 64 + ((uint32_t)j ^ (uint32_t)((lane >> 1) & 3)) * 16;
              asm volatile("st.shared.v4.b32 [%0], {%1, %2, %3, %4};" ::"r"(a), "r"(h[0]), "r"(h[1]), "r"(h[2]), "r"(h[3])
                           : "memory");
            }
          } else if (tma_store == 2) {
#pragma unroll
            for (int j = 0; j < 4; ++j) {
              uint32_t hi[4], lo[4];
#pragma unroll
              for (int u = 0; u < 4; ++u) split_bf16x2(v[8 * j + 2 * u], v[8 * j + 2 * u + 1], hi[u], lo[u]);
              const uint32_t a = buf + lane * 64 + ((uint32_t)j ^ (uint32_t)((lane >> 1) & 3)) * 16;
              asm volatile("st.shared.v4.b32 [%0], {%1, %2, %3, %4};" ::"r"(a), "r"(hi[0]), "r"(hi[1]), "r"(hi[2]),
                           "r"(hi[3]) : "memory");
              asm volatile("st.shared.v4.b32 [%0], {%1, %2, %3, %4};" ::"r"(a + EPI_BOX_BYTES / 2), "r"(lo[0]),
                           "r"(lo[1]), "r"(lo[2]), "r"(lo[3]) : "memory");
            }
          } else {
#pragma unroll
            for (int j = 0; j < 8; ++j) {
              const uint32_t a = buf + lane * 128 + ((uint32_t)j ^ (uint32_t)(lane & 7)) * 16;
              asm volatile("st.shared.v4.f32 [%0], {%1, %2, %3, %4};" ::"r"(a), "f"(v[4 * j]), "f"(v[4 * j + 1]),
                           "f"(v[4 * j + 2]), "f"(v[4 * j + 3]) : "memory");
            }
          }
          fence_proxy_async();
          __syncwarp();
          if (elect_one() && !(ea.debug & 1)) {
            tma_store_2d(&map_y, buf, n0 + c0, m_base);
            if (tma_store == 2) tma_store_2d(&map_y_lo, buf + EPI_BOX_BYTES / 2, n0 + c0, m_base);
            bulk_commit();
          }
        } else if (m < M && dest_row >= 0) {
          const int n_end = (ea.row_map && ldy == (int64_t)((N + 3) & ~3)) ? (int)ldy : N;
          if (n0 + c0 + 32 > N) {
#pragma unroll
            for (int j = 0; j < 32; ++j)
              if (n0 + c0 + j >= N) v[j] = 0.f;
          }
          const int n_dst = ea.n_peers > 0 ? ea.n_peers : 1;
#pragma unroll
          for (int p = 0; p < 8; ++p) {
            if (p >= n_dst) break;
            float* yp = ea.n_peers > 0 ? ea.peers[p] + dest_row * ldy + n0 : yrow;
#pragma unroll
            for (int j = 0; j < 32; j += 4) {
              if (vec_ok && j + 4 <= box_cols && n0 + c0 + j + 4 <= n_end) {
                *reinterpret_cast<float4*>(yp + c0 + j) = make_float4(v[j], v[j + 1], v[j + 2], v[j + 3]);
              } else {
#pragma unroll
                for (int u = 0; u < 4; ++u)
                  if (j + u < box_cols && n0 + c0 + j + u < n_end) yp[c0 + j + u] = v[j + u];
              }
            }
          }
        }
      }
      if (use_fast_head && !exchanged) exchange_stats(-INFINITY, 0.f);
      if (bulk_rows && !staged) {
        const float none[32] = {};
        stage_and_store(none, false, 0, 0);
      }
      fence_before();
      __syncwarp();
      if (lane == 0) {
        if (CTA2 && !leader) mbar_arrive_remote(mapa_rank(tempty_bar(acc), 0));
        else mbar_arrive(tempty_bar(acc));
      }
    }
    if (tma_store || ea.bulk_rows) {
      if (lane == 0) bulk_wait_all();
      __syncwarp();
      if (elect_one()) bulk_wait_all();
    }
  }

  fence_before();
  __syncthreads();
  if (CTA2) cluster_sync_all();
  if (warp == 1) {
    fence_after();
    if (CTA2)
      asm volatile("tcgen05.dealloc.cta_group::2.sync.aligned.b32 %0, %1;" ::"r"(tmem_base), "r"((uint32_t)TMEM_COLS)
                   : "memory");
    else
      asm volatile("tcgen05.dealloc.cta_group::1.sync.aligned.b32 %0, %1;" ::"r"(tmem_base), "r"((uint32_t)TMEM_COLS)
                   : "memory");
  }
}

typedef CUresult (*EncodeTiledFn)(CUtensorMap*, CUtensorMapDataType, cuuint32_t, void*, const cuuint64_t*,
                                  const cuuint64_t*, const cuuint32_t*, const cuuint32_t*, CUtensorMapInterleave,
                                  CUtensorMapSwizzle, CUtensorMapL2promotion, CUtensorMapFloatOOBfill);

static EncodeTiledFn encode_fn() {
  static EncodeTiledFn fn = nullptr;
  if (!fn) {
    void* p = nullptr;
    cudaDriverEntryPointQueryResult q;
    if (cudaGetDriverEntryPoint("cuTensorMapEncodeTiled", &p, cudaEnableDefault, &q) == cudaSuccess &&
        q == cudaDriverEntryPointSuccess)
      fn = reinterpret_cast<EncodeTiledFn>(p);
  }
  return fn;
}

static int make_map(CUtensorMap* map, const void* base, int64_t rows, int64_t cols, int64_t ld, int box_rows) {
  EncodeTiledFn fn = encode_fn();
  FG_REQUIRE(fn, FITGNN_ECUDA, "gemm_bf16x3: cuTensorMapEncodeTiled is not available from the driver");
  FG_REQUIRE(((uintptr_t)base & 15) == 0 && (ld * 2) % 16 == 0, FITGNN_EUNSUP,
             "gemm_bf16x3: bf16 planes need 16-byte aligned bases and a pitch that is a multiple of 8 elements");
  const cuuint64_t dims[2] = {(cuuint64_t)cols, (cuuint64_t)rows};
  const cuuint64_t strides[1] = {(cuuint64_t)ld * 2};
  const cuuint32_t box[2] = {(cuuint32_t)BLOCK_K, (cuuint32_t)box_rows};
  const cuuint32_t estr[2] = {1, 1};
  CUresult r = fn(map, CU_TENSOR_MAP_DATA_TYPE_BFLOAT16, 2, const_cast<void*>(base), dims, strides, box, estr,
                  CU_TENSOR_MAP_INTERLEAVE_NONE, CU_TENSOR_MAP_SWIZZLE_128B, CU_TENSOR_MAP_L2_PROMOTION_L2_256B,
                  CU_TENSOR_MAP_FLOAT_OOB_FILL_NONE);
  FG_REQUIRE(r == CUDA_SUCCESS, FITGNN_ECUDA, "gemm_bf16x3: cuTensorMapEncodeTiled failed (%d)", (int)r);
  return FITGNN_OK;
}

static int make_store_map(CUtensorMap* map, float* base, int64_t rows, int64_t cols, int64_t ld) {
  EncodeTiledFn fn = encode_fn();
  FG_REQUIRE(fn, FITGNN_ECUDA, "gemm_bf16x3: cuTensorMapEncodeTiled is not available from the driver");
  const cuuint64_t dims[2] = {(cuuint64_t)cols, (cuuint64_t)rows};
  const cuuint64_t strides[1] = {(cuuint64_t)ld * 4};
  const cuuint32_t box[2] = {32, 32};
  const cuuint32_t estr[2] = {1, 1};
  CUresult r = fn(map, CU_TENSOR_MAP_DATA_TYPE_FLOAT32, 2, base, dims, strides, box, estr, CU_TENSOR_MAP_INTERLEAVE_NONE,
                  CU_TENSOR_MAP_SWIZZLE_128B, CU_TENSOR_MAP_L2_PROMOTION_NONE, CU_TENSOR_MAP_FLOAT_OOB_FILL_NONE);
  FG_REQUIRE(r == CUDA_SUCCESS, FITGNN_ECUDA, "gemm_bf16x3: cuTensorMapEncodeTiled (store) failed (%d)", (int)r);
  return FITGNN_OK;
}

static int make_store_map_bf16(CUtensorMap* map, void* base, int64_t rows, int64_t cols, int64_t ld) {
  EncodeTiledFn fn = encode_fn();
  FG_REQUIRE(fn, FITGNN_ECUDA, "gemm_bf16x3: cuTensorMapEncodeTiled is not available from the driver");
  const cuuint64_t dims[2] = {(cuuint64_t)cols, (cuuint64_t)rows};
  const cuuint64_t strides[1] = {(cuuint64_t)ld * 2};
  const cuuint32_t box[2] = {32, 32};
  const cuuint32_t estr[2] = {1, 1};
  CUresult r = fn(map, CU_TENSOR_MAP_DATA_TYPE_BFLOAT16, 2, base, dims, strides, box, estr, CU_TENSOR_MAP_INTERLEAVE_NONE,
                  CU_TENSOR_MAP_SWIZZLE_64B, CU_TENSOR_MAP_L2_PROMOTION_NONE, CU_TENSOR_MAP_FLOAT_OOB_FILL_NONE);
  FG_REQUIRE(r == CUDA_SUCCESS, FITGNN_ECUDA, "gemm_bf16x3: cuTensorMapEncodeTiled (bf16 store) failed (%d)", (int)r);
  return FITGNN_OK;
}

#ifndef FG_AGG12_DEFAULT
#define FG_AGG12_DEFAULT 1
#endif
template <int BLOCK_N, bool GATHER, int AGG, int EW = EPI_WARPS, bool CTA2 = false>
static int launch(const GatherArgs& ga, const EpiArgs& ea, const CUtensorMap& a_hi, const CUtensorMap& a_lo, const void* W_hi, const void* W_lo, int64_t ldw,
                  const float* bias, int64_t M, int K, int N, int act, int head, float* Y, void* Y_lo, int64_t ldy,
                  int sms, cudaStream_t st) {
  CUtensorMap w_hi, w_lo;
  const int64_t w_rows = ea.m_batch_rows ? ea.w_rows_total : (int64_t)N;
  FG_TRY(make_map(&w_hi, W_hi, w_rows, K, ldw, CTA2 ? BLOCK_N / 2 : BLOCK_N));
  FG_TRY(make_map(&w_lo, W_lo ? W_lo : W_hi, w_rows, K, ldw, CTA2 ? BLOCK_N / 2 : BLOCK_N));
  const size_t w_planes = ea.w_planes == 1 ? 1 : 2;
  CUtensorMap y_map, y_lo_map;
  int tma_store = ((ldy * 4) % 16 == 0 && ((uintptr_t)Y & 15) == 0) ? 1 : 0;
  y_map = w_hi;
  y_lo_map = w_hi;
  if (ea.out_f16) {
    FG_REQUIRE(!Y_lo && !ea.row_map && (ldy * 2) % 16 == 0 && ((uintptr_t)Y & 15) == 0, FITGNN_EUNSUP,
               "gemm: fp16-plane output needs a 16-byte aligned plane with a pitch that is a multiple of 8, and no row map");
    tma_store = 3;
    FG_TRY(make_store_map_bf16(&y_map, Y, M, N, ldy));
  } else if (Y_lo) {
    FG_REQUIRE((ldy * 2) % 16 == 0 && ((uintptr_t)Y & 15) == 0 && ((uintptr_t)Y_lo & 15) == 0, FITGNN_EUNSUP,
               "gemm_bf16x3: split output needs 16-byte aligned planes and a pitch that is a multiple of 8");
    tma_store = 2;
    FG_TRY(make_store_map_bf16(&y_map, Y, M, N, ldy));
    FG_TRY(make_store_map_bf16(&y_lo_map, Y_lo, M, N, ldy));
  } else if (ea.row_map) {
    tma_store = 0;
  } else if (tma_store) {
    FG_TRY(make_store_map(&y_map, Y, M, N, ldy));
  }
  constexpr size_t SMEM_LIMIT = 227 * 1024;
  constexpr bool HALF_STAGE = BLOCK_N == 256 && (EW == EPI_WARPS_12 || (AGG && EW == EPI_WARPS_WIDE));
  const bool half_stage = HALF_STAGE || (CTA2 && ea.out_f16);
  const size_t FIXED = (size_t)EW * (half_stage ? EPI_BOX_BYTES / 2 : EPI_BOX_BYTES) + 1024 + 256 +
                       (BLOCK_N <= 64 ? 2 * EW * 32 * 8 : 0);
  FG_REQUIRE(!HALF_STAGE || ea.out_f16, FITGNN_EINVAL, "gemm: the 12/16-epilogue-warp 256-column tile stages one fp16 plane only");
  constexpr int NTHREADS = 64 + 32 * EW + (GATHER ? 32 * GATHER_WARPS : 0);
  const int k_blocks = (K + BLOCK_K - 1) / BLOCK_K;
  const int n_tiles = (int)ceil_div(N, BLOCK_N);
  const int64_t m_tiles = ceil_div(M, BLOCK_M);
  const int64_t tiles = m_tiles * n_tiles;
  const size_t a_bytes = (size_t)(ea.a_planes == 1 ? 1 : 2) * A_PLANE_BYTES;
  const size_t stage_b = a_bytes + w_planes * BLOCK_N * BLOCK_K * 2;
  int n_stages = (int)((SMEM_LIMIT - FIXED) / stage_b);
  if (n_stages > 8) n_stages = 8;
  int grid = (int)(tiles < sms ? tiles : sms);
  size_t smem = (size_t)n_stages * stage_b + FIXED;
  int w_stationary = 0;
  const size_t w_bytes = (size_t)k_blocks * w_planes * BLOCK_N * BLOCK_K * 2;
  if (!ea.m_batch_rows && w_bytes + 2 * a_bytes + FIXED <= SMEM_LIMIT && sms >= n_tiles && m_tiles >= 4 * (sms / n_tiles)) {
    w_stationary = 1;
    n_stages = (int)((SMEM_LIMIT - FIXED - w_bytes) / a_bytes);
    if (n_stages > 8) n_stages = 8;
    grid = (sms / n_tiles) * n_tiles;
    smem = w_bytes + (size_t)n_stages * a_bytes + FIXED;
  }
  if (!tuning().gemm_ws && w_stationary) {
    w_stationary = 0;
    n_stages = (int)((SMEM_LIMIT - FIXED) / stage_b);
    if (n_stages > 8) n_stages = 8;
    grid = (int)(tiles < sms ? tiles : sms);
    smem = (size_t)n_stages * stage_b + FIXED;
  }
  if (GATHER) {
    FG_REQUIRE(w_stationary && k_blocks <= 2 && n_stages >= k_blocks, FITGNN_EUNSUP,
               "gcn_layer_fused: shape not eligible (needs K <= 128 and enough row blocks for the W-stationary plan)");
    n_stages = (n_stages / k_blocks) * k_blocks;
    smem = w_bytes + (size_t)n_stages * a_bytes + FIXED;
  }
  auto kern = gemm_bf16x3_kernel<BLOCK_N, GATHER, AGG, EW, CTA2>;
  static size_t smem_configured = 0;
  if (smem > smem_configured) {
    FG_CUDA(cudaFuncSetAttribute(kern, cudaFuncAttributeMaxDynamicSharedMemorySize, (int)SMEM_LIMIT));
    smem_configured = SMEM_LIMIT;
  }
  if (CTA2) {
    const size_t b_half = w_planes * (size_t)(BLOCK_N / 2) * BLOCK_K * 2;
    const size_t STAGE2 = a_bytes + b_half;
    w_stationary = 0;
    n_stages = (int)((SMEM_LIMIT - FIXED) / STAGE2);
    if (n_stages > 8) n_stages = 8;
    smem = (size_t)n_stages * STAGE2 + FIXED;
    const int64_t m_pair_tiles = ceil_div(M, 2 * BLOCK_M);
    const int64_t pair_tiles = m_pair_tiles * n_tiles;
    int64_t pairs = pair_tiles < sms / 2 ? pair_tiles : sms / 2;
    const size_t w_res = (size_t)k_blocks * b_half;
    const int64_t ws_pairs = (pairs / n_tiles) * n_tiles;
    if (tuning().gemm_pair_ws && !ea.m_batch_rows && w_res + 3 * a_bytes + FIXED <= SMEM_LIMIT && ws_pairs >= n_tiles &&
        m_pair_tiles >= 4 * (ws_pairs / n_tiles)) {
      w_stationary = 1;
      pairs = ws_pairs;
      n_stages = (int)((SMEM_LIMIT - FIXED - w_res) / a_bytes);
      if (n_stages > 8) n_stages = 8;
      smem = w_res + (size_t)n_stages * a_bytes + FIXED;
    }
    cudaLaunchConfig_t cfg = {};
    cfg.gridDim = dim3((unsigned)(2 * pairs));
    cfg.blockDim = dim3(NTHREADS);
    cfg.dynamicSmemBytes = smem;
    cfg.stream = st;
    cudaLaunchAttribute attr[1];
    attr[0].id = cudaLaunchAttributeClusterDimension;
    attr[0].val.clusterDim.x = 2;
    attr[0].val.clusterDim.y = 1;
    attr[0].val.clusterDim.z = 1;
    cfg.attrs = attr;
    cfg.numAttrs = 1;
    FG_CUDA(cudaLaunchKernelEx(&cfg, kern, ga, ea, a_hi, a_lo, w_hi, w_lo, y_map, y_lo_map, tma_store, bias, M, K, N, act, head,
                               Y, ldy, w_stationary, n_stages));
    return FITGNN_OK;
  }
  kern<<<grid, NTHREADS, smem, st>>>(ga, ea, a_hi, a_lo, w_hi, w_lo, y_map, y_lo_map, tma_store, bias,
                                                              M, K, N, act, head, Y, ldy, w_stationary, n_stages);
  FG_LAUNCH_CHECK();
  return FITGNN_OK;
}

}

int gemm_bf16x3(const void* A_hi, const void* A_lo, int64_t lda, const void* W_hi, const void* W_lo, int64_t ldw,
                const float* bias, int64_t M, int K, int N, int act, int head, float* Y, void* Y_lo, int64_t ldy,
                const uint64_t* agg_desc, const float* agg_dinv, const int32_t* row_map, float* const* peers, int n_peers,
                const float* row_scale, int agg_defer_scale, cudaStream_t st, int64_t m_batch_rows, int w_batch_rows,
                int64_t w_rows_total, int in_f16, int out_f16, int agg_pre) {
  FG_REQUIRE(!agg_pre || agg_desc, FITGNN_EINVAL, "gemm: agg_pre needs the aggregation descriptors");
  FG_REQUIRE(W_lo || in_f16, FITGNN_EINVAL, "gemm: a single-plane W (W_lo = NULL) needs the fp16 operand format");
  FG_REQUIRE(!in_f16 || !A_lo, FITGNN_EINVAL, "gemm: FP16X2 takes ONE fp16 A plane (A_lo must be NULL)");
  FG_REQUIRE(in_f16 || A_lo, FITGNN_EINVAL, "gemm: BF16X3 needs the A_lo plane");
  FG_REQUIRE(!out_f16 || (head == FITGNN_HEAD_IDENTITY && !Y_lo && !row_map), FITGNN_EUNSUP,
             "gemm: an fp16-plane output cannot carry a head, a lo plane or a row map");
  FG_REQUIRE(m_batch_rows == 0 || (m_batch_rows % 256 == 0 && M % m_batch_rows == 0 && w_batch_rows >= N && !agg_desc &&
                                   !row_map && head == FITGNN_HEAD_IDENTITY && w_rows_total >= (M / m_batch_rows) * w_batch_rows),
             FITGNN_EINVAL, "gemm_bf16x3: bad batching (m_batch_rows must be a multiple of 256 dividing M)");
  FG_REQUIRE(!Y_lo || head == FITGNN_HEAD_IDENTITY, FITGNN_EUNSUP, "gemm_bf16x3: split output cannot carry a head");
  FG_REQUIRE(n_peers >= 0 && n_peers <= 8 && (n_peers == 0 || (peers && row_map)), FITGNN_EINVAL,
             "gemm_bf16x3: peer stores need 1..8 peer bases and a row map");
  FG_REQUIRE(!agg_desc || (agg_dinv && head == FITGNN_HEAD_IDENTITY && !row_map && N > 128), FITGNN_EUNSUP,
             "gemm_bf16x3: the fused aggregation needs dinv, no head, no row map and a wide output (N > 128)");
  FG_REQUIRE(!row_map || !Y_lo, FITGNN_EUNSUP, "gemm_bf16x3: a row map needs fp32 output");
  FG_REQUIRE(head == FITGNN_HEAD_IDENTITY || N <= 256, FITGNN_EUNSUP,
             "gemm_bf16x3: a fused (log-)softmax head needs N <= 256 (got %d)", N);
  FG_REQUIRE(M < (1ll << 31) - 128, FITGNN_ERANGE, "gemm_bf16x3: M exceeds the TMA coordinate range");
  int sms = sm_count() - tuning().sm_reserve;
  if (sms < 2) sms = 2;
  CUtensorMap a_hi, a_lo;
  FG_TRY(tc::make_map(&a_hi, A_hi, M, K, lda, tc::BLOCK_M));
  FG_TRY(tc::make_map(&a_lo, A_lo ? A_lo : A_hi, M, K, lda, tc::BLOCK_M));
  const tc::GatherArgs ga{};
  tc::EpiArgs ea{reinterpret_cast<const unsigned long long*>(agg_desc), agg_dinv, row_map, {}, n_peers, 0, row_scale,
                 agg_defer_scale, m_batch_rows, w_batch_rows, w_rows_total, in_f16 ? 1 : 2, in_f16 ? 1 : 0, out_f16 ? 1 : 0,
                 W_lo ? 2 : 1, tuning().gemm_prefetch, tuning().gemm_debug};
  for (int p = 0; p < n_peers; ++p) ea.peers[p] = peers[p];
  if (n_peers > 0) Y = peers[0];
  if (row_map && N <= 64 && ldy == (N + 3) / 4 * 4 && tuning().head_bulk) {
    bool aligned = ((uintptr_t)Y & 15) == 0;
    for (int p = 0; p < n_peers; ++p) aligned = aligned && ((uintptr_t)peers[p] & 15) == 0;
    ea.bulk_rows = aligned ? 1 : 0;
  }
  if (agg_desc && agg_pre) {
    if (K > 128 && out_f16 && in_f16 && M >= 4096 && tuning().gemm_pair)
      return tc::launch<256, false, 2, tc::EPI_WARPS_12, true>(ga, ea, a_hi, a_lo, W_hi, W_lo, ldw, bias, M, K, N, act, head, Y,
                                                               Y_lo, ldy, sms, st);
    return tc::launch<256, false, 2>(ga, ea, a_hi, a_lo, W_hi, W_lo, ldw, bias, M, K, N, act, head, Y, Y_lo, ldy, sms, st);
  }
  if (agg_desc) {
    if (tuning().agg_wide == 1)
      return tc::launch<128, false, true, tc::EPI_WARPS_WIDE>(ga, ea, a_hi, a_lo, W_hi, W_lo, ldw, bias, M, K, N, act, head, Y,
                                                              Y_lo, ldy, sms, st);
    if (out_f16 && tuning().agg_wide == 3)
      return tc::launch<256, false, true, tc::EPI_WARPS_WIDE>(ga, ea, a_hi, a_lo, W_hi, W_lo, ldw, bias, M, K, N, act, head, Y,
                                                              Y_lo, ldy, sms, st);
    if (out_f16 && (tuning().agg_wide == 2 || (tuning().agg_wide == 0 && FG_AGG12_DEFAULT)))
      return tc::launch<256, false, true, tc::EPI_WARPS_12>(ga, ea, a_hi, a_lo, W_hi, W_lo, ldw, bias, M, K, N, act, head, Y,
                                                            Y_lo, ldy, sms, st);
    return tc::launch<256, false, true>(ga, ea, a_hi, a_lo, W_hi, W_lo, ldw, bias, M, K, N, act, head, Y, Y_lo, ldy, sms, st);
  }
#define FG_TC(BN) \
  return tc::launch<BN, false, false>(ga, ea, a_hi, a_lo, W_hi, W_lo, ldw, bias, M, K, N, act, head, Y, Y_lo, ldy, sms, st)
  if (N <= 16) FG_TC(16);
  if (N <= 32) FG_TC(32);
  if (N <= 48) FG_TC(48);
  if (N <= 64) FG_TC(64);
  if (N <= 128) FG_TC(128);
  if (K <= 128 && out_f16 && head == FITGNN_HEAD_IDENTITY && !row_map && tuning().gemm_wide >= 0 && FG_AGG12_DEFAULT)
    return tc::launch<256, false, false, tc::EPI_WARPS_12>(ga, ea, a_hi, a_lo, W_hi, W_lo, ldw, bias, M, K, N, act, head, Y,
                                                           Y_lo, ldy, sms, st);
  if (K <= 128 && head == FITGNN_HEAD_IDENTITY && tuning().gemm_wide)
    return tc::launch<128, false, false, tc::EPI_WARPS_WIDE>(ga, ea, a_hi, a_lo, W_hi, W_lo, ldw, bias, M, K, N, act, head, Y,
                                                             Y_lo, ldy, sms, st);
  if (K > 128 && head == FITGNN_HEAD_IDENTITY && !row_map && M >= 4096 && tuning().gemm_pair && out_f16 && tuning().gemm_wide >= 0)
    return tc::launch<256, false, false, tc::EPI_WARPS_12, true>(ga, ea, a_hi, a_lo, W_hi, W_lo, ldw, bias, M, K, N, act, head, Y,
                                                                 Y_lo, ldy, sms, st);
  if (K > 128 && head == FITGNN_HEAD_IDENTITY && !row_map && M >= 4096 && tuning().gemm_pair)
    return tc::launch<256, false, false, tc::EPI_WARPS, true>(ga, ea, a_hi, a_lo, W_hi, W_lo, ldw, bias, M, K, N, act, head, Y,
                                                              Y_lo, ldy, sms, st);
  FG_TC(256);
#undef FG_TC
}


int gcn_layer_fused(const int32_t* rowptr, const int32_t* col, const float* dinv, const float* X, int64_t ldx, int width,
                    const int32_t* src_index, const int32_t* out_rows, int64_t M, const void* W_hi, const void* W_lo,
                    int64_t ldw, const float* bias, int N, int act, float* Y, void* Y_lo, int64_t ldy, cudaStream_t st) {
  FG_REQUIRE(width % 4 == 0 && width <= 128 && ldx % 4 == 0 && ((uintptr_t)X & 15) == 0, FITGNN_EUNSUP,
             "gcn_layer_fused: feature width must be a multiple of 4 and <= 128 (got %d)", width);
  FG_REQUIRE(N > 128, FITGNN_EUNSUP, "gcn_layer_fused: only the wide-output tile (N > 128) is instantiated");
  FG_REQUIRE(M < (1ll << 31) - 128, FITGNN_ERANGE, "gcn_layer_fused: M exceeds the coordinate range");
  const int sms = sm_count();
  const int K = (width + 7) / 8 * 8;
  tc::GatherArgs ga{rowptr, col, dinv, X, src_index, out_rows, ldx, width / 4};
  CUtensorMap dummy;
  FG_TRY(tc::make_map(&dummy, W_hi, N, K, ldw, 16));
  const tc::EpiArgs ea{nullptr, nullptr, nullptr, {}, 0, 0, nullptr, 0, 0, 0, 0, 2, 0, 0, 2, 0, 0};
  return tc::launch<256, true, false>(ga, ea, dummy, dummy, W_hi, W_lo, ldw, bias, M, K, N, act, FITGNN_HEAD_IDENTITY, Y,
                                      Y_lo, ldy, sms, st);
}

}
```

fitgnn_b200/engine.py:

```python
from __future__ import annotations

import torch

from . import ops
from .pack import Pack

_HEADS = {"identity": ops.HEAD_IDENTITY, "log_softmax": ops.HEAD_LOG_SOFTMAX, "softmax": ops.HEAD_SOFTMAX}


def conv_layers(sd):
    return len({k.split(".")[1] for k in sd if k.startswith("conv.")})


class PackedForward:

    def __init__(self, pack: Pack, state_dict, head="log_softmax", rows="core", precision="bf16x3",
                 with_head=True, fuse_layer0=False, fuse_aggregate="auto", align_policy="degree", out_map=None,
                 blocked_spmm="auto", dense_spmm="lds", conv_fused=False):
        if precision not in ("bf16x3", "fp32", "fp16x2", "fp16"):
            raise ValueError(f"precision={precision!r}")
        self.pack = pack
        dev = pack.device
        self.f16_hidden = precision in ("fp16x2", "fp16")
        self.w_single = precision == "fp16"
        self.precision = ops.GEMM_FP32 if precision == "fp32" else ops.GEMM_BF16X3
        self.kalign = 8 if self.precision == ops.GEMM_BF16X3 else 4
        self.L = conv_layers(state_dict)
        assert self.L >= 1
        self.head = _HEADS[head]
        self.with_head = with_head
        f32 = dict(dtype=torch.float32, device=dev)
        self.W, self.b = [], []
        for i in range(self.L):
            w = state_dict[f"conv.{i}.lin.weight"].detach().to(**f32)
            self.W.append(self._prep_weight(w))
            self.b.append(state_dict[f"conv.{i}.bias"].detach().to(**f32).contiguous())
        self.F = state_dict["conv.0.lin.weight"].shape[1]
        self.H = state_dict["conv.0.lin.weight"].shape[0]
        assert self.H % 4 == 0, "hidden width must be a multiple of 4"
        if with_head:
            self.Wl = self._prep_weight(state_dict["lt1.weight"].detach().to(**f32))
            self.bl = state_dict["lt1.bias"].detach().to(**f32).contiguous()
            self.C = state_dict["lt1.weight"].shape[0]
        if rows == "core":
            self.out_rows = pack.core_rows
        elif rows == "mask":
            self.out_rows = pack.mask_rows()
        elif rows == "all":
            self.out_rows = None
        else:
            self.out_rows = rows.to(device=dev, dtype=torch.int32).contiguous()
        if self.out_rows is not None and self.out_rows.numel() == pack.n_rows and bool(
                (self.out_rows.long() == torch.arange(pack.n_rows, device=dev)).all()):
            self.out_rows = None
        self.n_out = pack.n_rows if self.out_rows is None else self.out_rows.numel()
        self.Fp = self._kpad(self.F)
        self.transform_first = self.F > self.H
        self.hubs_all = ops.find_hubs(pack.rowptr, None, pack.n_rows)
        self.hubs_out = self.hubs_all if self.out_rows is None else ops.find_hubs(pack.rowptr, self.out_rows, self.n_out)
        self.launches = 0
        self._blk = None
        import os
        min_deg = float(os.environ.get("FITGNN_BLOCKED_MIN", "8"))
        if blocked_spmm is True or (blocked_spmm == "auto" and pack.n_rows > 0 and pack.nnz >= min_deg * pack.n_rows):
            if bool((pack.sub_ptr[1:] >= pack.sub_ptr[:-1]).all()):
                self._blk = ops.row_blocks(pack.sub_ptr, pack.n_rows, window=16, compact=True)
                self._blk_order = ops.block_row_order(pack.rowptr, self._blk)
        import os
        self._dense_spmm = os.environ.get("FITGNN_DENSE_SPMM", dense_spmm)
        self.fused_layer0 = None if fuse_layer0 else False
        self.prof = None
        self._nnz_cache = {}
        self.apack = None
        self._planes0 = None
        eligible = (self.precision == ops.GEMM_BF16X3 and self.L >= 2 and not self.transform_first and with_head
                    and self.out_rows is None and self.H > 128 and self.H % 8 == 0 and pack.n_rows > 0)
        if fuse_aggregate and eligible:
            ap = pack.aligned(32, align_policy)
            if ap is not None and ap.agg_ok:
                self.apack = ap
                self.hubs_aligned = ops.find_hubs(ap.rowptr, None, ap.n_rows)
                import os
                tricks = os.environ.get("FITGNN_ENGINE_TRICKS", "1") != "0"
                self.grouped_spmm = os.environ.get("FITGNN_SPMM_GROUPED", "1") != "0"
                self.defer_scale = tricks
                self.fold_bias = tricks and self.Fp > ops.pad4(self.F)
                if self.fold_bias:
                    w0 = state_dict["conv.0.lin.weight"].detach().to(**f32)
                    w0 = torch.nn.functional.pad(w0, (0, ops.pad4(self.F) - self.F))
                    self.W0_fold = self._prep_weight(torch.cat([w0, self.b[0][:, None]], 1))
        if fuse_aggregate is True and self.apack is None:
            raise ValueError("fuse_aggregate=True but the pack / model is not eligible for the fused aggregation")
        self.f16_classic = (self.f16_hidden and self.apack is None and self.precision == ops.GEMM_BF16X3 and self.L >= 2
                            and not self.transform_first and with_head and self.H % 8 == 0 and self.H >= 32)
        if self.f16_hidden and self.apack is None and not self.f16_classic:
            self.f16_hidden = False
        self.f16_layer0 = bool(self.f16_hidden and self.w_single and self.apack is not None
                               and getattr(self, "grouped_spmm", False) and ops.pad4(self.F) <= 128
                               and os.environ.get("FITGNN_F16_LAYER0", "1") != "0")
        if self.f16_layer0:
            w0 = state_dict["conv.0.lin.weight"].detach().to(**f32)
            if self.fold_bias:
                w0 = torch.cat([torch.nn.functional.pad(w0, (0, ops.pad4(self.F) - self.F)), self.b[0][:, None]], 1)
            self.W0_f16 = ops.split_f16(w0.contiguous(), ldo=self._kpad(w0.shape[1]), lo=False)
        if self.f16_hidden:
            for i in range(1, self.L):
                self.W[i] = ops.split_f16(state_dict[f"conv.{i}.lin.weight"].detach().to(**f32).contiguous(), ldo=self._kpad(self.H),
                                          lo=not self.w_single)
            self.Wl = ops.split_f16(state_dict["lt1.weight"].detach().to(**f32).contiguous(), ldo=self._kpad(self.H),
                                    lo=not (self.w_single and os.environ.get("FITGNN_HEAD_W1", "0") == "1"))
        import os
        cf = os.environ.get("FITGNN_CONV_FUSED", "")
        conv_fused = {"0": False, "1": True}.get(cf, conv_fused)
        self.conv_fused = bool(conv_fused) and self.f16_hidden and self.apack is not None and self.H > 128
        self.out_map = None
        if out_map is not None:
            assert with_head, "out_map needs the head"
            self.out_map = out_map.to(device=dev, dtype=torch.int32).contiguous()
            assert self.out_map.numel() == self.n_out
        self._head_map = None
        if self.apack is not None:
            self._head_map = self.apack.orig_row
            if self.out_map is not None:
                o = self.apack.orig_row.long()
                self._head_map = torch.where(o >= 0, self.out_map.long()[o.clamp(min=0)], o).to(torch.int32).contiguous()

    def enable_profile(self, on=True):
        self.prof = {} if on else None

    def _timed(self, name, fn, nbytes=0, flops=0):
        if self.prof is None:
            return fn()
        st = torch.cuda.current_stream()
        a, b = torch.cuda.Event(enable_timing=True), torch.cuda.Event(enable_timing=True)
        a.record(st)
        out = fn()
        b.record(st)
        rec = self.prof.setdefault(name, dict(events=[], bytes=nbytes, flops=flops))
        rec["events"].append((a, b))
        return out

    def profile_summary(self):
        out = {}
        for name, rec in (self.prof or {}).items():
            ms = [a.elapsed_time(b) for a, b in rec["events"]]
            out[name] = dict(ms=sum(ms) / len(ms), launches=len(ms), bytes=rec["bytes"], flops=rec["flops"])
        return out

    def _spmm_bytes(self, width, src_index, last, n_src_rows, out_elem=4, in_elem=4):
        p = self.pack
        key = ("nnz", last)
        if key not in self._nnz_cache:
            if last and self.out_rows is not None:
                r = self.out_rows.long()
                rp = p.rowptr.long()
                nnz = int((rp[r + 1] - rp[r]).sum())
            else:
                nnz = p.nnz
            self._nnz_cache[key] = nnz
        nnz = self._nnz_cache[key]
        r_out = self.n_out if last else p.n_rows
        b = 4 * (r_out + 1) + 4 * nnz + in_elem * n_src_rows * width + out_elem * r_out * width + 4 * width + 4 * n_src_rows
        if src_index is not None:
            b += 4 * p.n_rows
        if last and self.out_rows is not None:
            b += 4 * r_out
        return b

    def _spmm_bytes_aligned(self, width, src_index, n_src_rows):
        ap = self.apack
        b = 4 * (ap.n_rows + 1) + 4 * ap.nnz + 4 * ap.n_rows + 4 * (n_src_rows if src_index is not None else ap.n_rows) * width \
            + 4 * ap.n_rows * width
        return b + (4 * ap.n_rows if src_index is not None else 0)

    def _kpad(self, k):
        return (k + self.kalign - 1) // self.kalign * self.kalign

    def _prep_weight(self, w):
        kp = self._kpad(w.shape[1])
        if self.precision == ops.GEMM_BF16X3:
            return ops.split_bf16(w.contiguous(), ldo=kp)
        if kp != w.shape[1]:
            w = torch.nn.functional.pad(w, (0, kp - w.shape[1]))
        return w.contiguous()

    def _gemm(self, A, W, bias, act, head=ops.HEAD_IDENTITY, N=None, K=None, name="gemm", out=None, split_out=False,
              row_scale=None):
        self.launches += 1 + (1 if (head != ops.HEAD_IDENTITY and self.precision == ops.GEMM_FP32) else 0)
        M = (A[0] if isinstance(A, tuple) else A).shape[0]
        return self._timed(name, lambda: ops.gemm_bias_act(A, W, bias, act, head, precision=self.precision, N=N, K=K,
                                                           out=out, split_out=split_out, row_scale=row_scale),
                           nbytes=4 * (M * K + K * N + M * N), flops=2 * M * K * N)

    def _spmm(self, X, width, src_index, bias, act, last, split, name="spmm", pack=None, out=None):
        p = self.pack if pack is None else pack
        rows = self.out_rows if last else None
        hubs = self.hubs_out if last else self.hubs_all
        if pack is not None:
            hubs = self.hubs_aligned
        n_src_rows = X.shape[0] if src_index is not None else p.n_rows
        if rows is None and pack is None and self._blk is not None and self._dense_spmm == "mma":
            self.launches += 1
            return self._timed(name, lambda: ops.spmm_symnorm_mma(p.rowptr, p.col, p.dinv, X, self._blk, width, src_index, bias,
                                                                  act, out=out, split=split),
                               nbytes=self._spmm_bytes(width, src_index, last, n_src_rows))
        if rows is None and pack is None and self._blk is not None:
            self.launches += 1
            return self._timed(name, lambda: ops.spmm_symnorm_blocked(p.rowptr, p.col, p.dinv, X, self._blk, width, src_index,
                                                                      bias, act, out=out, split=split,
                                                                      row_order=self._blk_order),
                               nbytes=self._spmm_bytes(width, src_index, last, n_src_rows))
        self.launches += 1 + (1 if hubs[1] > 0 else 0)
        return self._timed(name, lambda: ops.spmm_symnorm(p.rowptr, p.col, p.dinv, X, width, src_index, bias, act, rows,
                                                          split=split, hubs=hubs, out=out),
                           nbytes=self._spmm_bytes(width, src_index, last, n_src_rows))

    def _fused_layer0(self, X, last):
        from ._lib import FitgnnError
        p = self.pack
        rows = self.out_rows if last else None
        n_rows = self.n_out if last else p.n_rows
        to_head = last and self.with_head and self.H % 8 == 0
        nbytes = self._spmm_bytes(self.Fp, p.gid, last, X.shape[0], out_elem=0) + 4 * n_rows * self.H
        flops = 2 * n_rows * self.Fp * self.H
        try:
            out = self._timed("layer0_fused", lambda: ops.gcn_layer_fused(
                p.rowptr, p.col, p.dinv, X, self.Fp, self.W[0], self.b[0], ops.ACT_ELU, src_index=p.gid, out_rows=rows,
                N=self.H, split_out=to_head), nbytes=nbytes, flops=flops)
        except FitgnnError as e:
            if "EUNSUP" not in str(e):
                raise
            self.fused_layer0 = False
            if self.prof is not None:
                self.prof.pop("layer0_fused", None)
            return None
        self.fused_layer0 = True
        self.launches += 1
        return out

    def pad_features(self, X):
        if X.shape[1] == self.Fp and X.is_contiguous():
            return X
        Xp = torch.zeros(X.shape[0], self.Fp, dtype=torch.float32, device=X.device)
        Xp[:, : X.shape[1]].copy_(X)
        return Xp

    def pack_features(self, X):
        ap = self.apack if self.apack is not None else self.pack
        if X.shape[1] % 4 != 0:
            X = torch.nn.functional.pad(X, (0, ops.pad4(X.shape[1]) - X.shape[1]))
        return X[ap.gid.long().clamp_(min=0)].contiguous()

    def _forward_aligned(self, X, out, peer_ptrs=None, packed=False):
        ap = self.apack
        M = ap.n_rows
        Wd = ops.pad4(self.F)
        fold = self.fold_bias
        src = None if packed else ap.gid
        if self.f16_layer0:
            if self._planes0 is None or self._planes0.device != X.device:
                self._planes0 = torch.zeros(M, self.Fp, dtype=torch.float16, device=X.device)
                if fold:
                    self._planes0[:, Wd] = 1.0
            self.launches += 1
            b4 = self._spmm_bytes_aligned(Wd, src, X.shape[0])
            A = self._timed("spmm0", lambda: ops.spmm_symnorm_grouped_f16(ap.rowptr, ap.col, ap.dinv, X, Wd, src, out=self._planes0,
                                                                          pad_value=(1.0 if fold else 0.0)),
                            nbytes=b4 - 2 * ap.n_rows * Wd)
        elif self._planes0 is None or self._planes0[0].device != X.device:
            hi = torch.zeros(M, self.Fp, dtype=torch.bfloat16, device=X.device)
            lo = torch.zeros(M, self.Fp, dtype=torch.bfloat16, device=X.device)
            if fold:
                hi[:, Wd] = 1.0
            self._planes0 = (hi, lo)
        if self.f16_layer0:
            pass
        elif self.grouped_spmm and Wd <= 128:
            self.launches += 1
            A = self._timed("spmm0", lambda: ops.spmm_symnorm_grouped(ap.rowptr, ap.col, ap.dinv, X, Wd, src, split=True,
                                                                      out=self._planes0,
                                                                      pad_value=(1.0 if fold else 0.0)),
                            nbytes=self._spmm_bytes_aligned(Wd, src, X.shape[0]))
        else:
            A = self._spmm(X, Wd, src, None, ops.ACT_NONE, False, split=True, name="spmm0", pack=ap, out=self._planes0)
        K = Wd + 1 if fold else Wd
        if self.conv_fused:
            return self._tail_conv_fused(A, K, M, X, out, peer_ptrs)
        for i in range(self.L - 1):
            Ai, Ki = A, K
            Wi, bi = (self.W0_fold, None) if (i == 0 and fold) else (self.W[i], self.b[i])
            if i == 0 and self.f16_layer0:
                Wi = self.W0_f16
            defer = self.defer_scale and i == self.L - 2
            self.launches += 1
            if self.f16_hidden:
                a_b = 2 if not isinstance(Ai, tuple) else 4
                A = self._timed(f"gemm{i}_agg", lambda: ops.gcn_transform_aggregate_f16(
                    Ai, Wi, bi, ops.ACT_ELU, ap.agg_desc, ap.dinv, K=Ki, N=self.H, defer_row_scale=defer),
                    nbytes=a_b * M * Ki + 4 * Ki * self.H + 2 * M * self.H + 12 * M, flops=2 * M * Ki * self.H)
            else:
                A = self._timed(f"gemm{i}_agg", lambda: ops.gcn_transform_aggregate(
                    Ai, Wi, bi, ops.ACT_ELU, ap.agg_desc, ap.dinv, K=Ki, N=self.H, defer_row_scale=defer),
                    nbytes=4 * (M * Ki + Ki * self.H + M * self.H) + 12 * M, flops=2 * M * Ki * self.H)
            K = self.H
        i = self.L - 1
        if self.f16_hidden:
            self.launches += 2
            h = self._timed(f"gemm{i}", lambda: ops.gemm_f16(A, self.W[i], self.b[i], ops.ACT_ELU, row_scale=ap.dinv if self.defer_scale else None,
                                                              out_f16=True, K=K, N=self.H),
                            nbytes=2 * M * K + 4 * K * self.H + 2 * M * self.H, flops=2 * M * K * self.H)
            nb16 = 2 * M * self.H + 4 * self.H * self.C + 4 * self.n_out * self.C + 4 * M
            if peer_ptrs is not None:
                self._timed("head", lambda: ops.gemm_f16_head_rows_peers(h, self.Wl, self.bl, ops.ACT_NONE, self.head, self._head_map,
                                                                         peer_ptrs, ops.pad4(self.C), K=self.H, N=self.C),
                            nbytes=nb16 + 4 * (len(peer_ptrs) - 1) * self.n_out * self.C, flops=2 * M * self.H * self.C)
                return None
            view = None
            if out is None:
                out = torch.empty(self.n_out, ops.pad4(self.C), dtype=torch.float32, device=X.device)
                view = out[:, : self.C]
            self._timed("head", lambda: ops.gemm_f16(h, self.Wl, self.bl, ops.ACT_NONE, self.head, row_map=self._head_map, out=out,
                                                     K=self.H, N=self.C),
                        nbytes=nb16, flops=2 * M * self.H * self.C)
            return out if view is None else view
        h = self._gemm(A, self.W[i], self.b[i], ops.ACT_ELU, N=self.H, K=K, name=f"gemm{i}", split_out=True,
                       row_scale=ap.dinv if self.defer_scale else None)
        view = None
        self.launches += 1
        nb = 4 * (M * self.H + self.H * self.C + self.n_out * self.C) + 4 * M
        if peer_ptrs is not None:
            self._timed("head", lambda: ops.gemm_head_rows_peers(h, self.Wl, self.bl, ops.ACT_NONE, self.head, self._head_map,
                                                                 peer_ptrs, ops.pad4(self.C), K=self.H, N=self.C),
                        nbytes=nb + 4 * (len(peer_ptrs) - 1) * self.n_out * self.C, flops=2 * M * self.H * self.C)
            return None
        if out is None:
            out = torch.empty(self.n_out, ops.pad4(self.C), dtype=torch.float32, device=X.device)
            view = out[:, : self.C]
        self._timed("head", lambda: ops.gemm_head_rows(h, self.Wl, self.bl, ops.ACT_NONE, self.head, self._head_map, out,
                                                       K=self.H, N=self.C), nbytes=nb, flops=2 * M * self.H * self.C)
        return out if view is None else view

    def _tail_conv_fused(self, A, K, M, X, out, peer_ptrs):
        ap, H = self.apack, self.H
        fold = self.fold_bias
        W0, b0 = (self.W0_fold, None) if fold else (self.W[0], self.b[0])
        if self.f16_layer0:
            W0 = self.W0_f16
        self.launches += 1
        h = self._timed("gemm0", lambda: ops.gcn_transform_aggregate_f16(A, W0, b0, ops.ACT_ELU, None, None, K=K, N=H),
                        nbytes=4 * M * K + 4 * K * H + 2 * M * H, flops=2 * M * K * H)
        for i in range(1, self.L):
            hi_, Wi, bi = h, self.W[i], self.b[i]
            self.launches += 1
            h = self._timed(f"conv{i}", lambda: ops.gcn_conv_aligned_f16(hi_, Wi, bi, ops.ACT_ELU, ap.agg_desc, ap.dinv, K=H, N=H),
                            nbytes=2 * M * H + 4 * H * H + 2 * M * H + 12 * M, flops=2 * M * H * H)
        self.launches += 1
        nb16 = 2 * M * H + 4 * H * self.C + 4 * self.n_out * self.C + 4 * M
        if peer_ptrs is not None:
            self._timed("head", lambda: ops.gemm_f16_head_rows_peers(h, self.Wl, self.bl, ops.ACT_NONE, self.head, self._head_map,
                                                                     peer_ptrs, ops.pad4(self.C), K=H, N=self.C),
                        nbytes=nb16 + 4 * (len(peer_ptrs) - 1) * self.n_out * self.C, flops=2 * M * H * self.C)
            return None
        view = None
        if out is None:
            out = torch.empty(self.n_out, ops.pad4(self.C), dtype=torch.float32, device=X.device)
            view = out[:, : self.C]
        self._timed("head", lambda: ops.gemm_f16(h, self.Wl, self.bl, ops.ACT_NONE, self.head, row_map=self._head_map, out=out,
                                                 K=H, N=self.C), nbytes=nb16, flops=2 * M * H * self.C)
        return out if view is None else view

    @torch.no_grad()
    def __call__(self, X, out=None, peer_ptrs=None, packed=False):
        assert peer_ptrs is None or self.apack is not None, "peer stores need the group-aligned schedule"
        assert self.out_map is None or (out is not None and peer_ptrs is None), "out_map needs the `out` tensor"
        p = self.pack
        assert X.is_cuda and X.dtype == torch.float32
        n_in = (self.apack if self.apack is not None else p).n_rows if packed else p.n_src
        assert X.shape[0] == n_in and X.shape[1] in (self.F, ops.pad4(self.F), self.Fp), tuple(X.shape)
        bf = self.precision == ops.GEMM_BF16X3
        if self.apack is not None:
            if not (X.is_contiguous() and X.shape[1] % 4 == 0):
                X = self.pad_features(X)
            return self._forward_aligned(X, out, peer_ptrs, packed)
        X = self.pad_features(X)
        gid0 = None if packed else p.gid
        h = None
        if self.f16_classic:
            return self._forward_classic_f16(X, gid0, out)
        for i in range(self.L):
            last = i == self.L - 1
            if i == 0 and self.transform_first:
                A = ops.split_bf16(X) if bf else X
                if bf:
                    self.launches += 1
                Z = self._gemm(A, self.W[0], None, ops.ACT_NONE, N=self.H, K=self.Fp, name="gemm0_unique_rows")
                h = self._spmm(Z, self.H, gid0, self.b[0], ops.ACT_ELU, last, split=False, name="spmm0")
            elif i == 0 and bf and self.fused_layer0 is not False and self.Fp <= 128 and self.H > 128 and not packed:
                h = self._fused_layer0(X, last)
                if h is None:
                    A = self._spmm(X, self.Fp, gid0, None, ops.ACT_NONE, last, split=bf, name="spmm0")
                    h = self._gemm(A, self.W[0], self.b[0], ops.ACT_ELU, N=self.H, K=self.Fp, name="gemm0",
                                   split_out=bf and last and self.with_head and self.H % 8 == 0)
            else:
                src, width, idx = (X, self.Fp, gid0) if i == 0 else (h, self.H, None)
                A = self._spmm(src, width, idx, None, ops.ACT_NONE, last, split=bf, name=f"spmm{i}")
                to_head = bf and last and self.with_head and self.H % 8 == 0
                h = self._gemm(A, self.W[i], self.b[i], ops.ACT_ELU, N=self.H, K=width, name=f"gemm{i}",
                               split_out=to_head)
        if not self.with_head:
            return h
        if bf and not isinstance(h, tuple):
            h = self._timed("split_head", lambda: ops.split_bf16(h), nbytes=8 * h.numel())
            self.launches += 1
        view = None
        if self.out_map is not None:
            if bf:
                self.launches += 1
                self._timed("head", lambda: ops.gemm_head_rows(h, self.Wl, self.bl, ops.ACT_NONE, self.head, self.out_map, out,
                                                               K=self.H, N=self.C),
                            nbytes=4 * (self.n_out * self.H + self.H * self.C + self.n_out * self.C) + 4 * self.n_out,
                            flops=2 * self.n_out * self.H * self.C)
            else:
                res = self._gemm(h, self.Wl, self.bl, ops.ACT_NONE, self.head, N=self.C, K=self.H, name="head")
                out[self.out_map.long(), : self.C] = res
            return out
        if out is None and self.C % 4 != 0:
            out = torch.empty(self.n_out, ops.pad4(self.C), dtype=torch.float32, device=X.device)
            view = out[:, : self.C]
        res = self._gemm(h, self.Wl, self.bl, ops.ACT_NONE, self.head, N=self.C, K=self.H, name="head", out=out)
        return res if view is None else view

    def _forward_classic_f16(self, X, gid0, out):
        p = self.pack
        H, Fp = self.H, self.Fp
        A = self._spmm(X, Fp, gid0, None, ops.ACT_NONE, False, split=True, name="spmm0")
        self.launches += 1
        M = p.n_rows
        h = self._timed("gemm0", lambda: ops.gcn_transform_aggregate_f16(A, self.W[0], self.b[0], ops.ACT_ELU, None, None,
                                                                         K=Fp, N=H),
                        nbytes=4 * M * Fp + 4 * Fp * H + 2 * M * H, flops=2 * M * Fp * H)
        for i in range(1, self.L):
            last = i == self.L - 1
            rows = self.out_rows if last else None
            hubs = self.hubs_out if last else self.hubs_all
            n_rows = self.n_out if last else p.n_rows
            src = h
            self.launches += 1 + (1 if hubs[1] > 0 else 0)
            A = self._timed(f"spmm{i}", lambda: ops.spmm_symnorm_f16(p.rowptr, p.col, p.dinv, src, H, None, None, ops.ACT_NONE,
                                                                      rows, hubs=hubs),
                            nbytes=self._spmm_bytes(H, None, last, p.n_rows, out_elem=2, in_elem=2))
            self.launches += 1
            h = self._timed(f"gemm{i}", lambda: ops.gemm_f16(A, self.W[i], self.b[i], ops.ACT_ELU, out_f16=True, K=H, N=H),
                            nbytes=2 * n_rows * H + 4 * H * H + 2 * n_rows * H, flops=2 * n_rows * H * H)
        n = self.n_out
        self.launches += 1
        nb = 2 * n * H + 4 * H * self.C + 4 * n * self.C
        fl = 2 * n * H * self.C
        if self.out_map is not None:
            self._timed("head", lambda: ops.gemm_f16(h, self.Wl, self.bl, ops.ACT_NONE, self.head, row_map=self.out_map, out=out,
                                                     K=H, N=self.C), nbytes=nb + 4 * n, flops=fl)
            return out
        view = None
        if out is None:
            out = torch.empty(n, ops.pad4(self.C), dtype=torch.float32, device=X.device)
        if out.shape[1] != self.C:
            view = out[:, : self.C]
        self._timed("head", lambda: ops.gemm_f16(h, self.Wl, self.bl, ops.ACT_NONE, self.head, out=out, K=H, N=self.C),
                    nbytes=nb, flops=fl)
        return out if view is None else view

    def capture(self, X_example):
        static_x = self.pad_features(X_example).clone()
        side = torch.cuda.Stream()
        side.wait_stream(torch.cuda.current_stream())
        with torch.cuda.stream(side):
            for _ in range(2):
                self(static_x)
        torch.cuda.current_stream().wait_stream(side)
        graph = torch.cuda.CUDAGraph()
        with torch.cuda.graph(graph):
            static_out = self(static_x)

        def run(X):
            static_x[:, : X.shape[1]].copy_(X)
            graph.replay()
            return static_out

        run.graph, run.static_out = graph, static_out
        return run

    def scatter_to_nodes(self, out, n_nodes=None):
        n_nodes = self.pack.n_nodes if n_nodes is None else n_nodes
        full = torch.empty(n_nodes, out.shape[1], dtype=out.dtype, device=out.device)
        full[self.pack.core_gid.long()] = out
        return full
```

fitgnn_b200/ops.py:

```python
from __future__ import annotations

import ctypes as C

import torch

from . import _lib
from ._lib import check, lib, ptr, stream_ptr

ACT_NONE, ACT_ELU = 0, 1
HEAD_IDENTITY, HEAD_LOG_SOFTMAX, HEAD_SOFTMAX = 0, 1, 2
MODE_NONE, MODE_EXTRA, MODE_CLUSTER = 0, 1, 2
POOL_MAX, POOL_MEAN = 0, 1
GEMM_FP32, GEMM_BF16X3 = 0, 1
MODES = {"none": MODE_NONE, "extra": MODE_EXTRA, "cluster": MODE_CLUSTER}


def _ws(nbytes, device):
    return torch.empty(max(int(nbytes), 256), dtype=torch.uint8, device=device)


def pad4(n):
    return (int(n) + 3) // 4 * 4


def sort_u64(keys, vals=None, key_bits=64):
    assert keys.dtype == torch.int64 and (vals is None or vals.dtype == torch.int32)
    ws = _ws(lib().fitgnn_sort_workspace_bytes(keys.numel()), keys.device)
    check(lib().fitgnn_sort_u64(ptr(keys), ptr(vals), keys.numel(), key_bits, ptr(ws), ws.numel(), stream_ptr()))
    return keys, vals


def scan_i32(x, with_total=True):
    assert x.dtype == torch.int32
    out = torch.empty(x.numel() + (1 if with_total else 0), dtype=torch.int32, device=x.device)
    ws = _ws(lib().fitgnn_scan_workspace_bytes(x.numel()), x.device)
    check(lib().fitgnn_scan_i32(ptr(x), ptr(out), x.numel(), int(with_total), ptr(ws), ws.numel(), stream_ptr()))
    return out


def csr_from_coo(edge_index, n):
    assert edge_index.dtype == torch.int64 and edge_index.dim() == 2 and edge_index.shape[0] == 2
    ei = edge_index.contiguous()
    E = ei.shape[1]
    ws = _ws(lib().fitgnn_csr_workspace_bytes(E, n), ei.device)
    nnz = C.c_int64(0)
    check(lib().fitgnn_csr_plan(ptr(ei), E, n, ptr(ws), ws.numel(), C.byref(nnz), stream_ptr()))
    rowptr = torch.empty(n + 1, dtype=torch.int32, device=ei.device)
    col = torch.empty(max(nnz.value, 1), dtype=torch.int32, device=ei.device)[: nnz.value]
    dinv = torch.empty(n, dtype=torch.float32, device=ei.device)
    check(lib().fitgnn_csr_fill(n, ptr(ws), ws.numel(), ptr(rowptr), ptr(col), ptr(dinv), stream_ptr()))
    return rowptr, col, dinv


def spmm_symnorm(rowptr, col, dinv, X, width=None, src_index=None, bias=None, act=ACT_NONE, out_rows=None,
                 out=None, split=False, hubs=None):
    assert X.dtype == torch.float32 and X.dim() == 2
    ldx = X.stride(0)
    width = X.shape[1] if width is None else width
    n_out = out_rows.numel() if out_rows is not None else rowptr.numel() - 1
    if split:
        if out is None:
            out = (torch.empty(n_out, width, dtype=torch.bfloat16, device=X.device),
                   torch.empty(n_out, width, dtype=torch.bfloat16, device=X.device))
        y, ylo, ldy = out[0], out[1], out[0].stride(0)
    else:
        if out is None:
            out = torch.empty(n_out, width, dtype=torch.float32, device=X.device)
        y, ylo, ldy = out, None, out.stride(0)
    if hubs is not None and hubs[1] > 0:
        hub_list, n_hub, hub_deg = hubs
        check(lib().fitgnn_spmm_symnorm_hub(ptr(rowptr), ptr(col), ptr(dinv), ptr(X), ldx, width, ptr(src_index),
                                            ptr(bias), act, ptr(out_rows), n_out, ptr(y), ptr(ylo), ldy,
                                            ptr(hub_list), n_hub, hub_deg, stream_ptr()))
    else:
        check(lib().fitgnn_spmm_symnorm(ptr(rowptr), ptr(col), ptr(dinv), ptr(X), ldx, width, ptr(src_index),
                                        ptr(bias), act, ptr(out_rows), n_out, ptr(y), ptr(ylo), ldy, stream_ptr()))
    return out


def spmm_symnorm_f16(rowptr, col, dinv, X, width=None, src_index=None, bias=None, act=ACT_NONE, out_rows=None, out=None,
                     hubs=None):
    assert X.dtype == torch.float16 and X.dim() == 2
    width = X.shape[1] if width is None else width
    n_out = out_rows.numel() if out_rows is not None else rowptr.numel() - 1
    if out is None:
        out = torch.empty(n_out, width, dtype=torch.float16, device=X.device)
    hub_list, n_hub, hub_deg = hubs if (hubs is not None and hubs[1] > 0) else (None, 0, 0)
    check(lib().fitgnn_spmm_symnorm_f16(ptr(rowptr), ptr(col), ptr(dinv), ptr(X), X.stride(0), width, ptr(src_index), ptr(bias),
                                        act, ptr(out_rows), n_out, ptr(out), out.stride(0), ptr(hub_list), None, n_hub, hub_deg,
                                        stream_ptr()))
    return out


def spmm_symnorm_grouped(rowptr, col, dinv, X, width=None, src_index=None, out=None, split=False, group=32,
                         pad_value=None):
    assert X.dtype == torch.float32 and X.dim() == 2
    width = X.shape[1] if width is None else width
    n = rowptr.numel() - 1
    if split:
        if out is None:
            out = (torch.empty(n, width, dtype=torch.bfloat16, device=X.device),
                   torch.empty(n, width, dtype=torch.bfloat16, device=X.device))
        y, ylo, ldy = out[0], out[1], out[0].stride(0)
    else:
        if out is None:
            out = torch.empty(n, width, dtype=torch.float32, device=X.device)
        y, ylo, ldy = out, None, out.stride(0)
    check(lib().fitgnn_spmm_symnorm_grouped(ptr(rowptr), ptr(col), ptr(dinv), ptr(X), X.stride(0), width, ptr(src_index),
                                            n, group, ptr(y), ptr(ylo), ldy, int(pad_value is not None),
                                            float(pad_value or 0.0), stream_ptr()))
    return out


def spmm_symnorm_grouped_f16(rowptr, col, dinv, X, width=None, src_index=None, out=None, pad_value=None):
    assert X.dtype == torch.float32 and X.dim() == 2
    width = X.shape[1] if width is None else width
    n = rowptr.numel() - 1
    if out is None:
        out = torch.empty(n, width, dtype=torch.float16, device=X.device)
    assert out.dtype == torch.float16 and out.shape[0] == n
    check(lib().fitgnn_spmm_symnorm_grouped_f16(ptr(rowptr), ptr(col), ptr(dinv), ptr(X), X.stride(0), width, ptr(src_index), n,
                                                32, ptr(out), out.stride(0), int(pad_value is not None), float(pad_value or 0.0),
                                                stream_ptr()))
    return out


def row_blocks(sub_ptr, n_rows, window=64, compact=False):
    sp = sub_ptr.long()
    nb = (int(n_rows) + window - 1) // window
    first = torch.searchsorted(sp[:-1].contiguous(), torch.arange(nb, device=sp.device) * window)
    blk = torch.cat([sp[first.clamp(max=sp.numel() - 1)], sp[-1:]])
    if compact:
        blk = torch.unique_consecutive(blk)
        if blk.numel() < 2:
            blk = torch.stack([sp[0], sp[-1]])
    return blk.to(torch.int32).contiguous()


def block_row_order(rowptr, blk_ptr):
    n = rowptr.numel() - 1
    deg = (rowptr[1:] - rowptr[:-1]).long()
    rows = torch.arange(n, device=rowptr.device)
    blk = torch.searchsorted(blk_ptr[1:].long().contiguous(), rows, right=True)
    key = blk * (int(deg.max()) + 1 if n else 1) + (int(deg.max()) - deg if n else deg)
    return torch.sort(key, stable=True).indices.to(torch.int32).contiguous()


def spmm_symnorm_blocked(rowptr, col, dinv, X, blk_ptr, width=None, src_index=None, bias=None, act=ACT_NONE, out=None,
                         split=False, row_order=None):
    assert X.dtype == torch.float32 and X.dim() == 2 and blk_ptr.dtype == torch.int32
    width = X.shape[1] if width is None else width
    n = rowptr.numel() - 1
    if split:
        if out is None:
            out = (torch.empty(n, width, dtype=torch.bfloat16, device=X.device),
                   torch.empty(n, width, dtype=torch.bfloat16, device=X.device))
        y, ylo, ldy = out[0], out[1], out[0].stride(0)
    else:
        if out is None:
            out = torch.empty(n, width, dtype=torch.float32, device=X.device)
        y, ylo, ldy = out, None, out.stride(0)
    check(lib().fitgnn_spmm_symnorm_blocked(ptr(rowptr), ptr(col), ptr(dinv), ptr(X), X.stride(0), width, ptr(src_index),
                                            ptr(blk_ptr), blk_ptr.numel() - 1, ptr(row_order), ptr(bias), act, ptr(y),
                                            ptr(ylo), ldy, stream_ptr()))
    return out


def spmm_symnorm_mma(rowptr, col, dinv, X, blk_ptr, width=None, src_index=None, bias=None, act=ACT_NONE, out=None, split=False):
    assert X.dtype == torch.float32 and X.dim() == 2 and blk_ptr.dtype == torch.int32
    width = X.shape[1] if width is None else width
    n = rowptr.numel() - 1
    if split:
        if out is None:
            out = (torch.empty(n, width, dtype=torch.bfloat16, device=X.device),
                   torch.empty(n, width, dtype=torch.bfloat16, device=X.device))
        y, ylo, ldy = out[0], out[1], out[0].stride(0)
    else:
        if out is None:
            out = torch.empty(n, width, dtype=torch.float32, device=X.device)
        y, ylo, ldy = out, None, out.stride(0)
    check(lib().fitgnn_spmm_symnorm_mma(ptr(rowptr), ptr(col), ptr(dinv), ptr(X), X.stride(0), width, ptr(src_index),
                                        ptr(blk_ptr), blk_ptr.numel() - 1, ptr(bias), act, ptr(y), ptr(ylo), ldy, stream_ptr()))
    return out


def find_hubs(rowptr, out_rows, n_out, hub_deg=256, cap=None):
    cap = int(cap if cap is not None else max(1024, n_out // 64))
    hub_list = torch.empty(cap, dtype=torch.int32, device=rowptr.device)
    cnt = torch.zeros(1, dtype=torch.int32, device=rowptr.device)
    check(lib().fitgnn_spmm_hubs(ptr(rowptr), ptr(out_rows), n_out, hub_deg, ptr(hub_list), ptr(cnt), cap,
                                 stream_ptr()))
    n = int(cnt.item())
    if n > cap:
        return find_hubs(rowptr, out_rows, n_out, hub_deg, n)
    hub_list = torch.sort(hub_list[:n]).values.contiguous() if n > 0 else hub_list[:0]
    return hub_list, n, hub_deg


def gemm_bias_act(A, W, bias=None, act=ACT_NONE, head=HEAD_IDENTITY, out=None, K=None, N=None, precision=GEMM_FP32,
                  split_out=False, row_scale=None):
    if precision == GEMM_FP32:
        a_hi, a_lo, w_hi, w_lo = A, None, W, None
        assert A.dtype == torch.float32 and W.dtype == torch.float32
    else:
        (a_hi, a_lo), (w_hi, w_lo) = A, W
        assert a_hi.dtype == torch.bfloat16 and w_hi.dtype == torch.bfloat16
    M = a_hi.shape[0]
    K = a_hi.shape[1] if K is None else K
    N = w_hi.shape[0] if N is None else N
    if split_out:
        if out is None:
            out = (torch.empty(M, N, dtype=torch.bfloat16, device=a_hi.device),
                   torch.empty(M, N, dtype=torch.bfloat16, device=a_hi.device))
        check(lib().fitgnn_gemm_rowscale_bias_act_split(precision, ptr(a_hi), ptr(a_lo), a_hi.stride(0), ptr(w_hi),
                                                        ptr(w_lo), w_hi.stride(0), ptr(row_scale), ptr(bias), M, K, N, act,
                                                        head, ptr(out[0]), ptr(out[1]), out[0].stride(0), stream_ptr()))
        return out
    if out is None:
        out = torch.empty(M, N, dtype=torch.float32, device=a_hi.device)
    check(lib().fitgnn_gemm_rowscale_bias_act_split(precision, ptr(a_hi), ptr(a_lo), a_hi.stride(0), ptr(w_hi), ptr(w_lo),
                                                    w_hi.stride(0), ptr(row_scale), ptr(bias), M, K, N, act, head, ptr(out),
                                                    None, out.stride(0), stream_ptr()))
    return out


def pad8(n):
    return (int(n) + 7) // 8 * 8


def linear_tc(x, weight, bias=None, act=ACT_NONE, head=HEAD_IDENTITY, x_planes=None):
    N, K = weight.shape
    Kp = pad8(K)
    w_pl = split_bf16(weight.detach().contiguous(), ldo=Kp)
    a_pl = x_planes if x_planes is not None else split_bf16(x, cols=K, ldo=Kp)
    return gemm_bias_act(a_pl, w_pl, bias, act, head, K=Kp, N=N, precision=GEMM_BF16X3)


def gcn_layer_fused(rowptr, col, dinv, X, width, W, bias=None, act=ACT_NONE, src_index=None, out_rows=None, N=None,
                    split_out=False):
    w_hi, w_lo = W
    N = w_hi.shape[0] if N is None else N
    n_out = out_rows.numel() if out_rows is not None else rowptr.numel() - 1
    if split_out:
        out = (torch.empty(n_out, N, dtype=torch.bfloat16, device=X.device),
               torch.empty(n_out, N, dtype=torch.bfloat16, device=X.device))
        y, ylo, ldy = out[0], out[1], N
    else:
        out = torch.empty(n_out, N, dtype=torch.float32, device=X.device)
        y, ylo, ldy = out, None, N
    check(lib().fitgnn_gcn_layer_fused(ptr(rowptr), ptr(col), ptr(dinv), ptr(X), X.stride(0), width, ptr(src_index),
                                       ptr(out_rows), n_out, ptr(w_hi), ptr(w_lo), w_hi.stride(0), ptr(bias), N, act,
                                       ptr(y), ptr(ylo), ldy, stream_ptr()))
    return out


def gcn_transform_aggregate(A, W, bias, act, agg_desc, dinv, K=None, N=None, split_out=True, defer_row_scale=False):
    (a_hi, a_lo), (w_hi, w_lo) = A, W
    assert a_hi.dtype == torch.bfloat16 and w_hi.dtype == torch.bfloat16 and agg_desc.dtype == torch.int64
    M = a_hi.shape[0]
    K = a_hi.shape[1] if K is None else K
    N = w_hi.shape[0] if N is None else N
    assert agg_desc.numel() == M and dinv.numel() == M
    if split_out:
        out = (torch.empty(M, N, dtype=torch.bfloat16, device=a_hi.device),
               torch.empty(M, N, dtype=torch.bfloat16, device=a_hi.device))
        y, ylo, ldy = out[0], out[1], N
    else:
        out = torch.empty(M, N, dtype=torch.float32, device=a_hi.device)
        y, ylo, ldy = out, None, N
    check(lib().fitgnn_gcn_transform_aggregate(ptr(a_hi), ptr(a_lo), a_hi.stride(0), ptr(w_hi), ptr(w_lo), w_hi.stride(0),
                                               ptr(bias), M, K, N, act, ptr(agg_desc), ptr(dinv), int(defer_row_scale),
                                               ptr(y), ptr(ylo), ldy, stream_ptr()))
    return out


def gemm_head_rows(A, W, bias, act, head, row_map, out, K=None, N=None):
    (a_hi, a_lo), (w_hi, w_lo) = A, W
    M = a_hi.shape[0]
    K = a_hi.shape[1] if K is None else K
    N = w_hi.shape[0] if N is None else N
    assert row_map.dtype == torch.int32 and row_map.numel() == M and out.dtype == torch.float32
    check(lib().fitgnn_gemm_head_rows(ptr(a_hi), ptr(a_lo), a_hi.stride(0), ptr(w_hi), ptr(w_lo), w_hi.stride(0), ptr(bias),
                                      M, K, N, act, head, ptr(row_map), ptr(out), out.stride(0), stream_ptr()))
    return out


def gemm_head_rows_peers(A, W, bias, act, head, row_map, peer_ptrs, ldy, K=None, N=None):
    (a_hi, a_lo), (w_hi, w_lo) = A, W
    M = a_hi.shape[0]
    K = a_hi.shape[1] if K is None else K
    N = w_hi.shape[0] if N is None else N
    assert row_map.dtype == torch.int32 and row_map.numel() == M
    bases = (C.c_void_p * len(peer_ptrs))(*[C.c_void_p(int(p)) for p in peer_ptrs])
    check(lib().fitgnn_gemm_head_rows_peers(ptr(a_hi), ptr(a_lo), a_hi.stride(0), ptr(w_hi), ptr(w_lo), w_hi.stride(0),
                                            ptr(bias), M, K, N, act, head, ptr(row_map), bases, len(peer_ptrs), ldy,
                                            stream_ptr()))


def gcn_forward(pack, X, state_dict, head=HEAD_LOG_SOFTMAX, precision=GEMM_BF16X3, out=None):
    from ._lib import WeightsStruct
    dev = X.device
    L = len({k.split(".")[1] for k in state_dict if k.startswith("conv.")})
    f32 = dict(dtype=torch.float32, device=dev)
    cw = [state_dict[f"conv.{i}.lin.weight"].detach().to(**f32).contiguous() for i in range(L)]
    cb = [state_dict[f"conv.{i}.bias"].detach().to(**f32).contiguous() for i in range(L)]
    lw = state_dict["lt1.weight"].detach().to(**f32).contiguous()
    lb = state_dict["lt1.bias"].detach().to(**f32).contiguous()
    F_, H, Cn = cw[0].shape[1], cw[0].shape[0], lw.shape[0]
    assert X.dtype == torch.float32 and X.shape[0] == pack.n_src and X.shape[1] >= F_
    if X.shape[1] % 4 != 0 or not X.is_contiguous():
        Xp = torch.zeros(X.shape[0], pad4(X.shape[1]), **f32)
        Xp[:, : X.shape[1]].copy_(X)
        X = Xp
    wptr = (C.c_void_p * L)(*[C.c_void_p(t.data_ptr()) for t in cw])
    bptr = (C.c_void_p * L)(*[C.c_void_p(t.data_ptr()) for t in cb])
    ws_ = WeightsStruct(L, F_, H, Cn, wptr, bptr, lw.data_ptr(), lb.data_ptr())
    st = pack.struct()
    nbytes = lib().fitgnn_gcn_forward_workspace_bytes(C.byref(st), C.byref(ws_), precision)
    if nbytes == 0:
        raise _lib.FitgnnError(f"fitgnn_gcn_forward_workspace_bytes: {_lib.last_error()}")
    ws = _ws(nbytes, dev)
    if out is None:
        out = torch.empty(pack.n_core, pad4(Cn), **f32)
    check(lib().fitgnn_gcn_forward(C.byref(st), ptr(X), X.stride(0), C.byref(ws_), head, precision, ptr(out), out.stride(0),
                                   ptr(ws), ws.numel(), stream_ptr()))
    return out[:, :Cn]


def gemm_tn(G, A):
    assert G.dtype == torch.float32 and A.dtype == torch.float32 and G.shape[0] == A.shape[0] and G.dim() == 2 and A.dim() == 2
    if G.stride(1) != 1:
        G = G.contiguous()
    if A.stride(1) != 1:
        A = A.contiguous()
    R, out, inn = G.shape[0], G.shape[1], A.shape[1]
    dW = torch.empty(out, inn, dtype=torch.float32, device=G.device)
    if R == 0:
        return dW.zero_()
    ws = _ws(lib().fitgnn_gemm_tn_workspace_bytes(R, out, inn), G.device)
    check(lib().fitgnn_gemm_tn(C.c_void_p(G.data_ptr()), G.stride(0), C.c_void_p(A.data_ptr()), A.stride(0), R, out, inn,
                               ptr(dW), dW.stride(0), ptr(ws), ws.numel(), stream_ptr()))
    return dW


def dropout(X, p, seed, offset=0, out=None):
    assert X.dtype == torch.float32 and X.dim() == 2 and X.stride(1) == 1
    if out is None:
        out = torch.empty(X.shape, dtype=torch.float32, device=X.device)
    check(lib().fitgnn_dropout(C.c_void_p(X.data_ptr()), X.stride(0), X.shape[0], X.shape[1], float(p), int(seed), int(offset),
                               ptr(out), out.stride(0), stream_ptr()))
    return out


def elu_dropout_backward(G, H, act=ACT_ELU, p=0.0, seed=0, offset=0):
    assert G.dtype == torch.float32 and H.dtype == torch.float32 and G.shape == H.shape and G.dim() == 2
    G = G if G.stride(1) == 1 else G.contiguous()
    H = H if H.stride(1) == 1 else H.contiguous()
    out = torch.empty(G.shape, dtype=torch.float32, device=G.device)
    check(lib().fitgnn_elu_dropout_backward(C.c_void_p(G.data_ptr()), G.stride(0), C.c_void_p(H.data_ptr()), H.stride(0),
                                            G.shape[0], G.shape[1], act, float(p),
                                            int(seed), int(offset), ptr(out), out.stride(0), stream_ptr()))
    return out


def adam_step(param, grad, exp_avg, exp_avg_sq, step, lr=0.01, betas=(0.9, 0.999), eps=1e-8, weight_decay=0.0):
    n = param.numel()
    assert all(t.dtype == torch.float32 and t.is_contiguous() and t.numel() == n for t in (param, grad, exp_avg, exp_avg_sq))
    check(lib().fitgnn_adam_step(ptr(param), ptr(grad), ptr(exp_avg), ptr(exp_avg_sq), n, float(lr), float(betas[0]),
                                 float(betas[1]), float(eps), float(weight_decay), int(step), stream_ptr()))


def raw_tensor(ptr_value, shape, device, owner=None):
    class _Raw:
        pass

    raw = _Raw()
    raw.__cuda_array_interface__ = {"shape": tuple(int(d) for d in shape), "typestr": "<f4", "data": (int(ptr_value), False),
                                    "version": 2, "strides": None}
    t = torch.as_tensor(raw, device=torch.device(device))
    t._fitgnn_owner = owner
    return t


class PeerBuffer:

    def __init__(self, nbytes, device):
        self.nbytes, self.device = int(nbytes), torch.device(device)
        p, h = C.c_void_p(), C.create_string_buffer(64)
        with torch.cuda.device(self.device):
            check(lib().fitgnn_peer_alloc(self.nbytes, C.byref(p), h))
        self.ptr, self.handle, self.opened = p.value, h.raw, {}

    def tensor(self, shape, dtype=torch.float32):
        n = 1
        for d in shape:
            n *= int(d)
        assert n * torch.empty(0, dtype=dtype).element_size() <= self.nbytes

        return raw_tensor(self.ptr, shape, self.device, owner=self)

    def open_peer(self, rank, handle):
        p = C.c_void_p()
        with torch.cuda.device(self.device):
            check(lib().fitgnn_peer_open(handle, C.byref(p)))
        self.opened[rank] = p.value
        return p.value

    def close(self):
        for p in self.opened.values():
            lib().fitgnn_peer_close(C.c_void_p(p))
        self.opened = {}
        if self.ptr:
            lib().fitgnn_peer_free(C.c_void_p(self.ptr))
            self.ptr = None


def split_bf16(X, cols=None, ldo=None):
    rows = X.shape[0]
    cols = X.shape[1] if cols is None else cols
    ldo = cols if ldo is None else ldo
    hi = torch.empty(rows, ldo, dtype=torch.bfloat16, device=X.device)
    lo = torch.empty(rows, ldo, dtype=torch.bfloat16, device=X.device)
    check(lib().fitgnn_split_bf16(ptr(X), X.stride(0), rows, cols, ptr(hi), ptr(lo), ldo, stream_ptr()))
    return hi, lo


def _segment_pool_raw(X, rows, seg_ptr, pool, width=None):
    width = X.shape[1] if width is None else width
    n_seg = seg_ptr.numel() - 1
    out = torch.empty(n_seg, width, dtype=torch.float32, device=X.device)
    check(lib().fitgnn_segment_pool(ptr(X), X.stride(0), width, ptr(rows), ptr(seg_ptr), n_seg, pool, ptr(out),
                                    out.stride(0), stream_ptr()))
    return out


class _SegmentPoolFn(torch.autograd.Function):

    @staticmethod
    def forward(ctx, X, rows, seg_ptr, pool):
        Xc = X.detach().contiguous()
        out = _segment_pool_raw(Xc, rows, seg_ptr, pool)
        ctx.pool, ctx.n_rows = pool, X.shape[0]
        ctx.save_for_backward(Xc, rows if rows is not None else torch.empty(0, dtype=torch.int32, device=X.device), seg_ptr, out)
        ctx.has_rows = rows is not None
        return out

    @staticmethod
    def backward(ctx, g):
        X, rows, seg_ptr, out = ctx.saved_tensors
        n_seg = seg_ptr.numel() - 1
        counts = (seg_ptr[1:] - seg_ptr[:-1]).long()
        R = int(seg_ptr[-1])
        sel = rows.long() if ctx.has_rows else torch.arange(R, device=X.device)
        seg_of = torch.repeat_interleave(torch.arange(n_seg, device=X.device), counts)
        g = g.contiguous()
        if ctx.pool == POOL_MEAN:
            gr = g[seg_of] / counts[seg_of].clamp(min=1).to(g.dtype)[:, None]
        else:
            xr = X[sel]
            idx = torch.arange(R, device=X.device)[:, None].expand(R, X.shape[1])
            cand = torch.where(xr == out[seg_of], idx, torch.full_like(idx, R))
            first = torch.full((n_seg, X.shape[1]), R, dtype=torch.long, device=X.device)
            first.scatter_reduce_(0, seg_of[:, None].expand(R, X.shape[1]), cand, reduce="amin")
            gr = torch.where(idx == first[seg_of], g[seg_of], torch.zeros((), dtype=g.dtype, device=g.device))
        gx = torch.zeros(ctx.n_rows, X.shape[1], dtype=g.dtype, device=g.device)
        gx.index_add_(0, sel, gr)
        return gx, None, None, None


def split_f16(X, cols=None, ldo=None, lo=True):
    rows = X.shape[0]
    cols = X.shape[1] if cols is None else cols
    ldo = cols if ldo is None else ldo
    hi = torch.empty(rows, ldo, dtype=torch.float16, device=X.device)
    lo_t = torch.empty(rows, ldo, dtype=torch.float16, device=X.device) if lo else None
    check(lib().fitgnn_split_f16(ptr(X), X.stride(0), rows, cols, ptr(hi), ptr(lo_t), ldo, stream_ptr()))
    return hi, lo_t


def gemm_f16(A, W, bias=None, act=ACT_NONE, head=HEAD_IDENTITY, row_scale=None, out_f16=False, row_map=None, out=None,
             K=None, N=None):
    w_hi, w_lo = W
    assert A.dtype == torch.float16 and w_hi.dtype == torch.float16
    M = A.shape[0]
    K = A.shape[1] if K is None else K
    N = w_hi.shape[0] if N is None else N
    if out is None:
        assert row_map is None
        out = torch.empty(M, N if (out_f16 or N % 4 == 0) else pad4(N), dtype=torch.float16 if out_f16 else torch.float32,
                          device=A.device)
    check(lib().fitgnn_gemm_f16(ptr(A), A.stride(0), ptr(w_hi), ptr(w_lo), w_hi.stride(0), ptr(row_scale), ptr(bias), M, K, N,
                                act, head, ptr(out), out.stride(0), int(out_f16), ptr(row_map), stream_ptr()))
    return out


def gemm_f16_head_rows_peers(A, W, bias, act, head, row_map, peer_ptrs, ldy, K=None, N=None):
    w_hi, w_lo = W
    M = A.shape[0]
    K = A.shape[1] if K is None else K
    N = w_hi.shape[0] if N is None else N
    assert A.dtype == torch.float16 and row_map.dtype == torch.int32 and row_map.numel() == M
    bases = (C.c_void_p * len(peer_ptrs))(*[C.c_void_p(int(p)) for p in peer_ptrs])
    check(lib().fitgnn_gemm_f16_head_rows_peers(ptr(A), A.stride(0), ptr(w_hi), ptr(w_lo), w_hi.stride(0), ptr(bias), M, K, N, act,
                                                head, ptr(row_map), bases, len(peer_ptrs), ldy, stream_ptr()))


def gcn_transform_aggregate_f16(A, W, bias, act, agg_desc, dinv, K=None, N=None, defer_row_scale=False):
    w_hi, w_lo = W
    in_f16 = not isinstance(A, tuple)
    a_hi, a_lo = (A, None) if in_f16 else A
    M = a_hi.shape[0]
    K = a_hi.shape[1] if K is None else K
    N = w_hi.shape[0] if N is None else N
    out = torch.empty(M, N, dtype=torch.float16, device=a_hi.device)
    check(lib().fitgnn_gcn_transform_aggregate_f16(int(in_f16), ptr(a_hi), ptr(a_lo), a_hi.stride(0), ptr(w_hi), ptr(w_lo),
                                                   w_hi.stride(0), ptr(bias), M, K, N, act, ptr(agg_desc), ptr(dinv),
                                                   int(defer_row_scale), ptr(out), out.stride(0), stream_ptr()))
    return out


def gcn_conv_aligned_f16(A, W, bias, act, agg_desc, dinv, K=None, N=None):
    w_hi, w_lo = W
    assert A.dtype == torch.float16 and w_hi.dtype == torch.float16
    M = A.shape[0]
    K = A.shape[1] if K is None else K
    N = w_hi.shape[0] if N is None else N
    out = torch.empty(M, N, dtype=torch.float16, device=A.device)
    check(lib().fitgnn_gcn_conv_aligned_f16(ptr(A), A.stride(0), ptr(w_hi), ptr(w_lo), w_hi.stride(0), ptr(bias), M, K, N, act,
                                            ptr(agg_desc), ptr(dinv), ptr(out), out.stride(0), stream_ptr()))
    return out


def segment_pool(X, rows, seg_ptr, pool, width=None):
    if torch.is_grad_enabled() and X.requires_grad:
        assert width is None or width == X.shape[1]
        return _SegmentPoolFn.apply(X, rows, seg_ptr, pool)
    return _segment_pool_raw(X, rows, seg_ptr, pool, width)


def group_by_part(part, k):
    assert part.dtype == torch.int32
    N = part.numel()
    members = torch.empty(N, dtype=torch.int32, device=part.device)
    member_ptr = torch.empty(k + 1, dtype=torch.int32, device=part.device)
    ws = _ws(lib().fitgnn_group_workspace_bytes(N, k), part.device)
    check(lib().fitgnn_group_by_part(ptr(part), N, k, ptr(members), ptr(member_ptr), ptr(ws), ws.numel(),
                                     stream_ptr()))
    return members, member_ptr


def project_features(members, member_ptr, cweight, X):
    assert cweight.dtype == torch.float64 and X.dtype == torch.float32
    k = member_ptr.numel() - 1
    F = X.shape[1]
    Xc = torch.empty(k, F, dtype=torch.float32, device=X.device)
    check(lib().fitgnn_project_features(ptr(members), ptr(member_ptr), k, ptr(cweight), ptr(X), X.stride(0), F,
                                        ptr(Xc), Xc.stride(0), stream_ptr()))
    return Xc


def project_adj(edge_index, part, k, want_rowptr=True):
    ei = edge_index.contiguous()
    E = ei.shape[1]
    N = part.numel()
    ws = _ws(lib().fitgnn_project_adj_workspace_bytes(E), ei.device)
    nnz = C.c_int64(0)
    check(lib().fitgnn_project_adj_plan(ptr(ei), E, N, ptr(part), k, ptr(ws), ws.numel(), C.byref(nnz), stream_ptr()))
    n = nnz.value
    row = torch.empty(max(n, 1), dtype=torch.int64, device=ei.device)[:n]
    col = torch.empty(max(n, 1), dtype=torch.int64, device=ei.device)[:n]
    cnt = torch.empty(max(n, 1), dtype=torch.int32, device=ei.device)[:n]
    rowptr = torch.empty(k + 1, dtype=torch.int32, device=ei.device) if want_rowptr else None
    check(lib().fitgnn_project_adj_fill(ptr(ws), ws.numel(), k, ptr(row), ptr(col), ptr(cnt), ptr(rowptr),
                                        stream_ptr()))
    return row, col, cnt, rowptr
```

include/fitgnn.h:

```cpp
#ifndef FITGNN_H_
#define FITGNN_H_

#include <stddef.h>
#include <stdint.h>

#ifdef __cplusplus
extern "C" {
#endif

#define FITGNN_ABI_VERSION 1

enum {
  FITGNN_OK = 0,
  FITGNN_EINVAL = -1,
  FITGNN_ECUDA = -2,
  FITGNN_ERANGE = -3,
  FITGNN_EWS = -4,
  FITGNN_EUNSUP = -5
};

enum { FITGNN_ACT_NONE = 0, FITGNN_ACT_ELU = 1 };

enum { FITGNN_HEAD_IDENTITY = 0, FITGNN_HEAD_LOG_SOFTMAX = 1, FITGNN_HEAD_SOFTMAX = 2 };

enum { FITGNN_MODE_NONE = 0, FITGNN_MODE_EXTRA = 1, FITGNN_MODE_CLUSTER = 2 };

enum { FITGNN_POOL_MAX = 0, FITGNN_POOL_MEAN = 1 };

enum { FITGNN_GEMM_FP32 = 0, FITGNN_GEMM_BF16X3 = 1, FITGNN_GEMM_FP16X2 = 2  };

typedef struct fitgnn_pack {
  int64_t n_rows;
  int64_t nnz;
  int64_t n_sub;
  int64_t n_core;
  int64_t n_src;
  const int32_t* rowptr;
  const int32_t* col;
  const float* dinv;
  const int32_t* gid;
  const int32_t* sub_ptr;
  const int32_t* core_rows;
  const uint8_t* is_core;
  const uint8_t* mask;
} fitgnn_pack;

typedef struct fitgnn_plan {
  int64_t n_rows, nnz, n_sub, n_core, n_src;
  int64_t fill_ws_bytes;
  int64_t priv[27];
} fitgnn_plan;

int fitgnn_abi_version(void);
int fitgnn_last_error(char* buf, size_t n);
int fitgnn_device_info(int* sm_count, int* cc);
int fitgnn_tuning_set(const char* name, int value);
int fitgnn_tuning_get(const char* name, int* value);

size_t fitgnn_csr_workspace_bytes(int64_t E, int64_t n);
int fitgnn_csr_plan(const int64_t* edge_index, int64_t E, int64_t n, void* ws, size_t ws_bytes,
                    int64_t* host_nnz, void* stream);
int fitgnn_csr_fill(int64_t n, void* ws, size_t ws_bytes, int32_t* rowptr ,
                    int32_t* col , float* dinv , void* stream);

size_t fitgnn_pack_workspace_bytes(int64_t E, int64_t N, int64_t k, int mode, int64_t ac_nnz);
int fitgnn_pack_plan(const int64_t* edge_index, int64_t E, int64_t N, const int32_t* part, int64_t k,
                     int mode, const int32_t* ac_rowptr, const int32_t* ac_col, int64_t ac_nnz,
                     void* ws, size_t ws_bytes, fitgnn_plan* host_plan, void* stream);
int fitgnn_pack_fill(const fitgnn_plan* host_plan, const fitgnn_pack* out, void* ws, size_t ws_bytes,
                     void* ws2, size_t ws2_bytes, void* stream);

int fitgnn_spmm_symnorm(const int32_t* rowptr, const int32_t* col, const float* dinv,
                        const float* X, int64_t ldx, int width, const int32_t* src_index,
                        const float* bias, int act, const int32_t* out_rows, int64_t n_out,
                        void* Y, void* Y_lo, int64_t ldy, void* stream);
int fitgnn_spmm_symnorm_grouped(const int32_t* rowptr, const int32_t* col, const float* dinv,
                                const float* X, int64_t ldx, int width, const int32_t* src_index,
                                int64_t n_rows, int group, void* Y, void* Y_lo, int64_t ldy,
                                int fill_pad, float pad_value, void* stream);
int fitgnn_spmm_symnorm_grouped_f16(const int32_t* rowptr, const int32_t* col, const float* dinv,
                                    const float* X, int64_t ldx, int width, const int32_t* src_index,
                                    int64_t n_rows, int group, void* Y, int64_t ldy, int fill_pad,
                                    float pad_value, void* stream);
int fitgnn_spmm_symnorm_blocked(const int32_t* rowptr, const int32_t* col, const float* dinv,
                                const float* X, int64_t ldx, int width, const int32_t* src_index,
                                const int32_t* blk_ptr, int64_t n_blk, const int32_t* row_order,
                                const float* bias, int act, void* Y, void* Y_lo, int64_t ldy, void* stream);
int fitgnn_spmm_symnorm_mma(const int32_t* rowptr, const int32_t* col, const float* dinv,
                            const float* X, int64_t ldx, int width, const int32_t* src_index,
                            const int32_t* blk_ptr, int64_t n_blk, const float* bias, int act,
                            void* Y, void* Y_lo, int64_t ldy, void* stream);
int fitgnn_spmm_hubs(const int32_t* rowptr, const int32_t* out_rows, int64_t n_out, int hub_deg,
                     int32_t* hub_list , int32_t* hub_count , int hub_cap,
                     void* stream);
int fitgnn_spmm_symnorm_hub(const int32_t* rowptr, const int32_t* col, const float* dinv,
                            const float* X, int64_t ldx, int width, const int32_t* src_index,
                            const float* bias, int act, const int32_t* out_rows, int64_t n_out,
                            void* Y, void* Y_lo, int64_t ldy, const int32_t* hub_list, int n_hub,
                            int hub_deg, void* stream);

int fitgnn_spmm_symnorm_devhub(const int32_t* rowptr, const int32_t* col, const float* dinv,
                               const float* X, int64_t ldx, int width, const int32_t* src_index,
                               const float* bias, int act, const int32_t* out_rows, int64_t n_out,
                               void* Y, void* Y_lo, int64_t ldy, const int32_t* hub_list,
                               const int32_t* hub_count , int hub_cap, int hub_deg, void* stream);

int fitgnn_gemm_bias_act(int precision, const void* A, const void* A_lo, int64_t lda,
                         const void* W, const void* W_lo, int64_t ldw, const float* bias,
                         int64_t M, int K, int N, int act, int head, float* Y, int64_t ldy,
                         void* stream);
int fitgnn_gemm_bias_act_split(int precision, const void* A, const void* A_lo, int64_t lda,
                               const void* W, const void* W_lo, int64_t ldw, const float* bias,
                               int64_t M, int K, int N, int act, int head, void* Y, void* Y_lo,
                               int64_t ldy, void* stream);
int fitgnn_gcn_layer_fused(const int32_t* rowptr, const int32_t* col, const float* dinv, const float* X,
                           int64_t ldx, int width, const int32_t* src_index, const int32_t* out_rows,
                           int64_t n_out, const void* W_hi, const void* W_lo, int64_t ldw,
                           const float* bias, int N, int act, void* Y, void* Y_lo, int64_t ldy,
                           void* stream);
enum { FITGNN_ALIGN_IN_ORDER = 0, FITGNN_ALIGN_BY_DEGREE = 1 };
size_t fitgnn_pack_align_workspace_bytes(int64_t n_sub, int64_t n_rows_aligned);
int fitgnn_pack_align_plan(const fitgnn_pack* in, int group, int policy, int32_t* new_sub_ptr,
                           int64_t* host_n_rows_aligned, int* host_alignable, void* ws, size_t ws_bytes,
                           void* stream);
int fitgnn_pack_align_fill(const fitgnn_pack* in, const int32_t* new_sub_ptr, int group,
                           int64_t n_rows_aligned, const fitgnn_pack* out, int32_t* orig_row,
                           int32_t* new_of_old, uint64_t* agg_desc, int* host_flags, void* ws,
                           size_t ws_bytes, void* stream);
int fitgnn_gcn_transform_aggregate(const void* A_hi, const void* A_lo, int64_t lda, const void* W_hi,
                                   const void* W_lo, int64_t ldw, const float* bias, int64_t M, int K,
                                   int N, int act, const uint64_t* agg_desc, const float* dinv,
                                   int defer_row_scale, void* Y, void* Y_lo, int64_t ldy, void* stream);
int fitgnn_gemm_rowscale_bias_act_split(int precision, const void* A, const void* A_lo, int64_t lda,
                                        const void* W, const void* W_lo, int64_t ldw,
                                        const float* row_scale, const float* bias, int64_t M, int K,
                                        int N, int act, int head, void* Y, void* Y_lo, int64_t ldy,
                                        void* stream);
int fitgnn_split_f16(const float* X, int64_t ldx, int64_t rows, int cols, void* hi, void* lo, int64_t ldo, void* stream);
int fitgnn_gemm_f16(const void* A, int64_t lda, const void* W_hi, const void* W_lo, int64_t ldw,
                    const float* row_scale, const float* bias, int64_t M, int K, int N, int act, int head,
                    void* Y, int64_t ldy, int out_f16, const int32_t* row_map, void* stream);
int fitgnn_spmm_symnorm_f16(const int32_t* rowptr, const int32_t* col, const float* dinv, const void* X, int64_t ldx,
                            int width, const int32_t* src_index, const float* bias, int act, const int32_t* out_rows,
                            int64_t n_out, void* Y, int64_t ldy, const int32_t* hub_list, const int32_t* hub_count,
                            int hub_cap, int hub_deg, void* stream);
int fitgnn_gcn_conv_aligned_f16(const void* A, int64_t lda, const void* W_hi, const void* W_lo, int64_t ldw,
                                const float* bias, int64_t M, int K, int N, int act, const uint64_t* agg_desc,
                                const float* dinv, void* Y, int64_t ldy, void* stream);
int fitgnn_gemm_f16_head_rows_peers(const void* A, int64_t lda, const void* W_hi, const void* W_lo, int64_t ldw,
                                    const float* bias, int64_t M, int K, int N, int act, int head,
                                    const int32_t* row_map, float* const* host_peer_bases, int n_peers,
                                    int64_t ldy, void* stream);
int fitgnn_gcn_transform_aggregate_f16(int in_f16, const void* A_hi, const void* A_lo, int64_t lda, const void* W_hi,
                                       const void* W_lo, int64_t ldw, const float* bias, int64_t M, int K, int N,
                                       int act, const uint64_t* agg_desc, const float* dinv, int defer_row_scale,
                                       void* Y, int64_t ldy, void* stream);
int fitgnn_gemm_head_rows(const void* A_hi, const void* A_lo, int64_t lda, const void* W_hi,
                          const void* W_lo, int64_t ldw, const float* bias, int64_t M, int K, int N,
                          int act, int head, const int32_t* row_map, float* Y, int64_t ldy, void* stream);
int fitgnn_gemm_head_rows_peers(const void* A_hi, const void* A_lo, int64_t lda, const void* W_hi,
                                const void* W_lo, int64_t ldw, const float* bias, int64_t M, int K,
                                int N, int act, int head, const int32_t* row_map,
                                float* const* host_peer_bases, int n_peers, int64_t ldy, void* stream);
int fitgnn_peer_push(const void* src, void* const* host_dst, int n_dst, size_t bytes, int n_ctas, void* stream);
int fitgnn_peer_alloc(size_t bytes, void** dev_ptr, uint8_t* handle_out );
int fitgnn_peer_open(const uint8_t* handle , void** dev_ptr);
int fitgnn_peer_close(void* dev_ptr);
int fitgnn_peer_free(void* dev_ptr);
int fitgnn_split_bf16(const float* X, int64_t ldx, int64_t rows, int cols, void* hi, void* lo,
                      int64_t ldo, void* stream);

typedef struct fitgnn_weights {
  int n_layers;
  int in_features, hidden, n_classes;
  const float* const* conv_weight;
  const float* const* conv_bias;
  const float* lt1_weight;
  const float* lt1_bias;
} fitgnn_weights;
size_t fitgnn_gcn_forward_workspace_bytes(const fitgnn_pack* pack, const fitgnn_weights* weights, int precision);
int fitgnn_gcn_forward(const fitgnn_pack* pack, const float* X, int64_t ldx, const fitgnn_weights* weights,
                       int head, int precision, float* out , int64_t ld_out, void* ws,
                       size_t ws_bytes, void* stream);

size_t fitgnn_gemm_tn_workspace_bytes(int64_t R, int out, int in);
int fitgnn_gemm_tn(const float* G, int64_t ldg, const float* A, int64_t lda, int64_t R, int out, int in,
                   float* dW, int64_t lddw, void* ws, size_t ws_bytes, void* stream);
int fitgnn_dropout(const float* X, int64_t ldx, int64_t rows, int cols, float p, uint64_t seed,
                   uint64_t offset, float* Y, int64_t ldy, void* stream);
int fitgnn_elu_dropout_backward(const float* G, int64_t ldg, const float* H, int64_t ldh, int64_t rows,
                                int cols, int act, float p, uint64_t seed, uint64_t offset, float* GZ,
                                int64_t ldo, void* stream);
int fitgnn_adam_step(float* param, const float* grad, float* exp_avg, float* exp_avg_sq, int64_t n, float lr,
                     float beta1, float beta2, float eps, float weight_decay, int64_t step, void* stream);

int fitgnn_segment_pool(const float* X, int64_t ldx, int width, const int32_t* rows,
                        const int32_t* seg_ptr, int64_t n_seg, int pool, float* Y, int64_t ldy,
                        void* stream);

size_t fitgnn_group_workspace_bytes(int64_t N, int64_t k);
int fitgnn_group_by_part(const int32_t* part, int64_t N, int64_t k, int32_t* members ,
                         int32_t* member_ptr , void* ws, size_t ws_bytes, void* stream);
int fitgnn_project_features(const int32_t* members, const int32_t* member_ptr, int64_t k,
                            const double* cweight , const float* X, int64_t ldx,
                            int F, float* Xc, int64_t ldxc, void* stream);
size_t fitgnn_project_adj_workspace_bytes(int64_t E);
int fitgnn_project_adj_plan(const int64_t* edge_index, int64_t E, int64_t N, const int32_t* part,
                            int64_t k, void* ws, size_t ws_bytes, int64_t* host_nnz, void* stream);
int fitgnn_project_adj_fill(void* ws, size_t ws_bytes, int64_t k, int64_t* out_row, int64_t* out_col,
                            int32_t* out_cnt, int32_t* out_rowptr , void* stream);

size_t fitgnn_sort_workspace_bytes(int64_t n);
int fitgnn_sort_u64(uint64_t* keys, uint32_t* vals, int64_t n, int key_bits, void* ws,
                    size_t ws_bytes, void* stream);
int fitgnn_scan_i32(const int32_t* in, int32_t* out, int64_t n, int with_total, void* ws,
                    size_t ws_bytes, void* stream);
size_t fitgnn_scan_workspace_bytes(int64_t n);

#ifdef __cplusplus
}
#endif
#endif
```

Before: 759.7 million.

## Fuse last hidden GEMM with classifier head in tcgen05 CTA-pair kernel

Adds a head-fused variant of the tcgen05 GEMM kernel. After the ELU epilogue writes fp16 hidden activations back into TMEM, the MMA warp issues a TMEM-sourced (ts) MMA against resident hi/lo classifier weights. Per-N-tile partial logits go to a global workspace, and the last tile to finish, detected with an atomic counter, sums them and applies bias and softmax/log-softmax. This removes the round trip of the hidden state through global memory and one kernel launch. In exchange it adds a memset, atomics, partial-sum traffic, tighter shared-memory and TMEM budgets, and a harder-to-verify synchronisation scheme. It is enabled by default when the shape conditions hold.

```diff
diff --git a/fitgnn_b200/_lib.py b/fitgnn_b200/_lib.py
--- a/fitgnn_b200/_lib.py
+++ b/fitgnn_b200/_lib.py
@@ -73,6 +73,9 @@
     "fitgnn_split_f16": (c_i32, [c_void, c_i64, c_i64, c_i32, c_void, c_void, c_i64, c_void]),
     "fitgnn_gemm_f16": (c_i32, [c_void, c_i64, c_void, c_void, c_i64, c_void, c_void, c_i64, c_i32, c_i32, c_i32, c_i32, c_void,
                                 c_i64, c_i32, c_void, c_void]),
+    "fitgnn_gemm_f16_head_fused_workspace_bytes": (c_size, [c_i64, c_i32]),
+    "fitgnn_gemm_f16_head_fused": (c_i32, [c_void, c_i64, c_void, c_i64, c_void, c_void, c_i64, c_i32, c_i32, c_i32, c_void, c_void,
+                                           c_i64, c_void, c_i32, c_i32, c_void, c_void, c_i64, c_void, c_size, c_void]),
     "fitgnn_gemm_f16_head_rows_peers": (c_i32, [c_void, c_i64, c_void, c_void, c_i64, c_void, c_i64, c_i32, c_i32, c_i32, c_i32,
                                                 c_void, C.POINTER(c_void), c_i32, c_i64, c_void]),
     "fitgnn_gcn_transform_aggregate_f16": (c_i32, [c_i32, c_void, c_void, c_i64, c_void, c_void, c_i64, c_void, c_i64, c_i32,
diff --git a/fitgnn_b200/csrc/capi.cu b/fitgnn_b200/csrc/capi.cu
--- a/fitgnn_b200/csrc/capi.cu
+++ b/fitgnn_b200/csrc/capi.cu
@@ -61,6 +61,11 @@
                 const uint64_t* agg_desc, const float* agg_dinv, const int32_t* row_map, float* const* peers, int n_peers,
                 const float* row_scale, int agg_defer_scale, cudaStream_t st, int64_t m_batch_rows = 0, int w_batch_rows = 0,
                 int64_t w_rows_total = 0, int in_f16 = 0, int out_f16 = 0, int agg_pre = 0);
+size_t gemm_f16_head_fused_workspace_bytes(int64_t M, int N);
+int gemm_f16_head_fused(const void* A, int64_t lda, const void* W, int64_t ldw, const float* row_scale, const float* bias,
+                        int64_t M, int K, int N, int act, const void* Wl_hi, const void* Wl_lo, int64_t ldwl, const float* bl,
+                        int C, int head, const int32_t* row_map, float* Y, int64_t ldy, void* workspace, size_t ws_bytes,
+                        cudaStream_t st);
 
 int gcn_layer_fused(const int32_t* rowptr, const int32_t* col, const float* dinv, const float* X, int64_t ldx, int width,
                     const int32_t* src_index, const int32_t* out_rows, int64_t M, const void* W_hi, const void* W_lo,
@@ -217,6 +222,26 @@
                      nullptr, row_map, nullptr, 0, row_scale, 0, as_stream(stream), 0, 0, 0, 1, out_f16 ? 1 : 0);
 }
 
+extern "C" size_t fitgnn_gemm_f16_head_fused_workspace_bytes(int64_t M, int N) {
+  return M > 0 && N > 0 ? gemm_f16_head_fused_workspace_bytes(M, N) : 0;
+}
+
+extern "C" int fitgnn_gemm_f16_head_fused(const void* A, int64_t lda, const void* W, int64_t ldw, const float* row_scale,
+                                          const float* bias, int64_t M, int K, int N, int act, const void* Wl_hi,
+                                          const void* Wl_lo, int64_t ldwl, const float* bl, int C, int head,
+                                          const int32_t* row_map, float* Y, int64_t ldy, void* workspace, size_t ws_bytes,
+                                          void* stream) {
+  FG_REQUIRE(A && W && Wl_hi && Wl_lo && bl && Y && M >= 0 && K > 0 && N > 0 && C > 0, FITGNN_EINVAL,
+             "gemm_f16_head_fused: bad arguments (M=%lld K=%d N=%d C=%d)", (long long)M, K, N, C);
+  FG_REQUIRE(lda >= K && ldw >= K && ldwl >= N && ldy >= C, FITGNN_EINVAL, "gemm_f16_head_fused: leading dimension too small");
+  FG_REQUIRE(act == FITGNN_ACT_NONE || act == FITGNN_ACT_ELU, FITGNN_EINVAL, "gemm_f16_head_fused: unknown act %d", act);
+  FG_REQUIRE(head >= FITGNN_HEAD_IDENTITY && head <= FITGNN_HEAD_SOFTMAX, FITGNN_EINVAL, "gemm_f16_head_fused: unknown head %d",
+             head);
+  if (M == 0) return FITGNN_OK;
+  return gemm_f16_head_fused(A, lda, W, ldw, row_scale, bias, M, K, N, act, Wl_hi, Wl_lo, ldwl, bl, C, head, row_map, Y, ldy,
+                             workspace, ws_bytes, as_stream(stream));
+}
+
 extern "C" int fitgnn_gcn_transform_aggregate_f16(int in_f16, const void* A_hi, const void* A_lo, int64_t lda, const void* W_hi,
                                                   const void* W_lo, int64_t ldw, const float* bias, int64_t M, int K, int N,
                                                   int act, const uint64_t* agg_desc, const float* dinv, int defer_row_scale,
diff --git a/fitgnn_b200/csrc/gemm_tcgen05.cu b/fitgnn_b200/csrc/gemm_tcgen05.cu
--- a/fitgnn_b200/csrc/gemm_tcgen05.cu
+++ b/fitgnn_b200/csrc/gemm_tcgen05.cu
@@ -48,6 +48,11 @@
   int w_planes;
   int l2_prefetch;
   int debug;
+  const float* head_bias;
+  int head_c;
+  int64_t head_m_pad;
+  float* head_part;
+  int32_t* head_cnt;
 };
 constexpr int EPI_WARP0 = 2;
 constexpr int ACC_STAGES = 2;
@@ -175,6 +180,15 @@
   asm volatile("tcgen05.commit.cta_group::2.mbarrier::arrive::one.shared::cluster.multicast::cluster.b64 [%0], %1;" ::"r"(bar),
                "h"(mask)
                : "memory");
+}
+__device__ __forceinline__ void umma_ts_pair(uint32_t tmem_d, uint32_t tmem_a, uint64_t b_desc, uint32_t idesc,
+                                             uint32_t accumulate) {
+  asm volatile(
+      "{\n\t.reg .pred p;\n\t"
+      "setp.ne.b32 p, %4, 0;\n\t"
+      "tcgen05.mma.cta_group::2.kind::f16 [%0], [%1], %2, %3, p;\n\t}"
+      ::"r"(tmem_d), "r"(tmem_a), "l"(b_desc), "r"(idesc), "r"(accumulate)
+      : "memory");
 }
 __device__ __forceinline__ void mbar_arrive_remote(uint32_t cluster_addr) {
   asm volatile("mbarrier.arrive.shared::cluster.b64 _, [%0];" ::"r"(cluster_addr) : "memory");
@@ -231,6 +245,14 @@
                :
                : "memory");
 }
+__device__ __forceinline__ void tmem_st16(uint32_t taddr, const uint32_t (&r)[16]) {
+  asm volatile(
+      "tcgen05.st.sync.aligned.32x32b.x16.b32 [%0], {%1,%2,%3,%4,%5,%6,%7,%8,%9,%10,%11,%12,%13,%14,%15,%16};"
+      ::"r"(taddr), "r"(r[0]), "r"(r[1]), "r"(r[2]), "r"(r[3]), "r"(r[4]), "r"(r[5]), "r"(r[6]), "r"(r[7]), "r"(r[8]),
+        "r"(r[9]), "r"(r[10]), "r"(r[11]), "r"(r[12]), "r"(r[13]), "r"(r[14]), "r"(r[15])
+      : "memory");
+}
+__device__ __forceinline__ void tmem_wait_st() { asm volatile("tcgen05.wait::st.sync.aligned;" ::: "memory"); }
 __device__ __forceinline__ void fence_before() { asm volatile("tcgen05.fence::before_thread_sync;" ::: "memory"); }
 __device__ __forceinline__ void fence_after() { asm volatile("tcgen05.fence::after_thread_sync;" ::: "memory"); }
 
@@ -244,7 +266,21 @@
   return s > 8 ? 8 : s;
 }
 
-template <int BLOCK_N, bool GATHER, int AGG, int EW, bool CTA2 = false>
+constexpr int HEAD_N = 64;
+constexpr int HEAD_COL = 64;
+constexpr int HEAD_MAX_C = 48;
+constexpr int HEAD_PITCH = 48;
+constexpr int HEAD_KB = 256 / BLOCK_K;
+constexpr uint32_t HEAD_W_TILE = (HEAD_N / 2) * BLOCK_K * 2;
+constexpr uint32_t HEAD_W_BYTES = 2 * HEAD_KB * HEAD_W_TILE;
+static_assert(HEAD_MAX_C <= HEAD_N && HEAD_COL + HEAD_N <= 144 && HEAD_COL >= 48, "head accumulator inside the free columns");
+static_assert(2 * 256 <= 512 && 8 * 16384 + HEAD_W_BYTES + 4 * A_PLANE_BYTES + 1024 + 256 <= 227 * 1024, "head-fused budgets");
+__host__ __device__ constexpr int head_a_col(int c) {
+  return c < 96 ? c / 2 : c < 192 ? 144 + (c - 96) / 2 : 192 + (c - 192) / 2;
+}
+static_assert(head_a_col(95) < 48 && head_a_col(96) == 144 && head_a_col(191) < 192 && head_a_col(255) < 224, "layout");
+
+template <int BLOCK_N, bool GATHER, int AGG, int EW, bool CTA2 = false, bool HEADF = false>
 __global__ void __launch_bounds__(64 + 32 * EW + (GATHER ? 32 * GATHER_WARPS : 0), 1)
 gemm_bf16x3_kernel(const GatherArgs ga, const EpiArgs ea, const __grid_constant__ CUtensorMap map_a_hi, const __grid_constant__ CUtensorMap map_a_lo,
                    const __grid_constant__ CUtensorMap map_w_hi, const __grid_constant__ CUtensorMap map_w_lo,
@@ -270,7 +306,8 @@
                 "2, 3 (256-column tile with an fp16-plane output) or 4 epilogue warps per TMEM lane quadrant");
   constexpr bool HALF_STAGE = BLOCK_N == 256 && (EW == EPI_WARPS_12 || (AGG && EW == EPI_WARPS_WIDE));
   const uint32_t WARP_STAGE = (HALF_STAGE || (CTA2 && ea.out_f16)) ? EPI_BOX_BYTES / 2 : EPI_BOX_BYTES;
-  const uint32_t STAGING_BYTES = EW * WARP_STAGE;
+  static_assert(!HEADF || (CTA2 && !GATHER && !AGG && BLOCK_N == 256 && EW == EPI_WARPS_12), "head-fused form: 12-warp CTA pairs");
+  const uint32_t STAGING_BYTES = HEADF ? 0u : EW * WARP_STAGE;
 
   extern __shared__ uint8_t smem_raw[];
   uint8_t* smem = reinterpret_cast<uint8_t*>(((uintptr_t)smem_raw + 1023) & ~(uintptr_t)1023);
@@ -279,10 +316,12 @@
   const uint32_t w_region_bytes = w_stationary ? (uint32_t)k_blocks * b_bytes : 0u;
   const uint32_t a_bytes = (a_single ? 1u : 2u) * A_PLANE_BYTES;
   const uint32_t stage_bytes_rt = w_stationary ? a_bytes : a_bytes + b_bytes;
-  uint8_t* staging = smem + w_region_bytes + (size_t)n_stages * stage_bytes_rt;
+  const uint32_t hw_bytes = HEADF ? HEAD_W_BYTES : 0u;
+  uint8_t* staging = smem + w_region_bytes + hw_bytes + (size_t)n_stages * stage_bytes_rt;
   uint64_t* bars = reinterpret_cast<uint64_t*>(staging + STAGING_BYTES);
   uint32_t* tmem_slot = reinterpret_cast<uint32_t*>(bars + 2 * MAX_STAGES + 2 * ACC_STAGES + 1);
-  const uint32_t smem_base = smem_u32(smem) + w_region_bytes;
+  const uint32_t smem_base = smem_u32(smem) + w_region_bytes + hw_bytes;
+  const uint32_t hw_base = smem_u32(smem) + w_region_bytes;
   const uint32_t w_base = smem_u32(smem);
   const uint32_t bar_base = smem_u32(bars);
   auto full_bar = [&](int s) { return bar_base + 8u * s; };
@@ -290,6 +329,9 @@
   auto tfull_bar = [&](int s) { return bar_base + 8u * (2 * MAX_STAGES + s); };
   auto tempty_bar = [&](int s) { return bar_base + 8u * (2 * MAX_STAGES + ACC_STAGES + s); };
   const uint32_t wfull_bar = bar_base + 8u * (2 * MAX_STAGES + 2 * ACC_STAGES);
+  auto aready_bar = [&](int s) { return bar_base + 8u * (24 + s); };
+  auto hfull_bar = [&](int s) { return bar_base + 8u * (26 + s); };
+  int32_t* head_slot = reinterpret_cast<int32_t*>(bars + 28);
 
   const int warp = threadIdx.x >> 5, lane = threadIdx.x & 31;
   const int n_tiles = (N + BLOCK_N - 1) / BLOCK_N;
@@ -332,6 +374,10 @@
     for (int s = 0; s < ACC_STAGES; ++s) {
       mbar_init(tfull_bar(s), 1);
       mbar_init(tempty_bar(s), CTA2 ? 2 * EW : EW);
+      if (HEADF) {
+        mbar_init(aready_bar(s), 2 * EW);
+        mbar_init(hfull_bar(s), 1);
+      }
     }
     asm volatile("fence.mbarrier_init.release.cluster;" ::: "memory");
   }
@@ -362,11 +408,17 @@
         if (elect_one()) {
           if (CTA2) {
             const uint32_t lbar = mapa_rank(wfull_bar, 0);
-            if (leader) mbar_arrive_expect_tx(wfull_bar, 2 * w_region_bytes);
+            if (leader) mbar_arrive_expect_tx(wfull_bar, 2 * (w_region_bytes + hw_bytes));
             for (int kb = 0; kb < k_blocks; ++kb) {
               tma_load_2d_pair(w_base + kb * b_bytes, &map_w_hi, lbar, kb * BLOCK_K, n0 + (int)cta_rank * B_ROWS);
               if (!w_single)
                 tma_load_2d_pair(w_base + kb * b_bytes + B_PLANE_BYTES, &map_w_lo, lbar, kb * BLOCK_K, n0 + (int)cta_rank * B_ROWS);
+            }
+            if (HEADF) {
+              for (int kb = 0; kb < HEAD_KB; ++kb) {
+                tma_load_2d_pair(hw_base + (2 * kb) * HEAD_W_TILE, &map_y, lbar, n0 + kb * BLOCK_K, (int)cta_rank * (HEAD_N / 2));
+                tma_load_2d_pair(hw_base + (2 * kb + 1) * HEAD_W_TILE, &map_y_lo, lbar, n0 + kb * BLOCK_K, (int)cta_rank * (HEAD_N / 2));
+              }
             }
           } else {
             mbar_arrive_expect_tx(wfull_bar, w_region_bytes);
@@ -433,6 +485,28 @@
       uint32_t stage = 0, phase = 0;
       uint32_t it = 0;
       if (w_stationary && valid(w0)) mbar_wait(wfull_bar, 0);
+      constexpr uint32_t IDESC_HEAD = umma_idesc_f16(2 * BLOCK_M, HEAD_N);
+      bool head_due = false;
+      auto issue_head = [&](uint32_t t) {
+        const uint32_t st = tmem_base + (t % ACC_STAGES) * BLOCK_N;
+        __syncwarp();
+        if (elect_one()) {
+#pragma unroll
+          for (int j = 0; j < 256 / UMMA_K; ++j) {
+            const uint32_t kb = j / (BLOCK_K / UMMA_K);
+            const uint64_t adv = (uint64_t)(((j % (BLOCK_K / UMMA_K)) * UMMA_K * 2) >> 4);
+            const uint32_t a = st + (uint32_t)head_a_col(j * UMMA_K);
+            umma_ts_pair(st + HEAD_COL, a, umma_desc_sw128(hw_base + (2 * kb) * HEAD_W_TILE) + adv, IDESC_HEAD, j != 0);
+            umma_ts_pair(st + HEAD_COL, a, umma_desc_sw128(hw_base + (2 * kb + 1) * HEAD_W_TILE) + adv, IDESC_HEAD, 1);
+          }
+          umma_commit_pair(hfull_bar(t % ACC_STAGES));
+        }
+        __syncwarp();
+      };
+      auto head_ready = [&](uint32_t t) {
+        const bool ok = mbar_try_wait(aready_bar(t % ACC_STAGES), (t / ACC_STAGES) & 1u);
+        return __shfl_sync(0xffffffffu, ok ? 1 : 0, 0) != 0;
+      };
       for (Walk w = w0; valid(w); ++it, advance(w)) {
         const uint32_t acc = it % ACC_STAGES;
         const uint32_t acc_phase = (it / ACC_STAGES) & 1u;
@@ -473,7 +547,25 @@
           }
           __syncwarp();
           if (++stage == (uint32_t)n_stages) { stage = 0; phase ^= 1; }
-        }
+          if (HEADF && head_due && head_ready(it - 1)) {
+            fence_after();
+            issue_head(it - 1);
+            head_due = false;
+          }
+        }
+        if (HEADF) {
+          if (head_due) {
+            mbar_wait(aready_bar((it - 1) % ACC_STAGES), ((it - 1) / ACC_STAGES) & 1u);
+            fence_after();
+            issue_head(it - 1);
+          }
+          head_due = true;
+        }
+      }
+      if (HEADF && head_due) {
+        mbar_wait(aready_bar((it - 1) % ACC_STAGES), ((it - 1) / ACC_STAGES) & 1u);
+        fence_after();
+        issue_head(it - 1);
       }
     };
     if (leader) {
@@ -591,6 +683,146 @@
       ca = cb; cb = cc;
       wa = wb; sa = sb;
     }
+  } else if (HEADF) {
+    const int quad = warp & 3;
+    const int grp = (warp - EPI_WARP0) >> 2;
+    const int row_in_tile = quad * 32 + lane;
+    const int box_beg = 3 * grp, n_box = grp == 2 ? 2 : 3;
+    const bool bias_vec = (((uintptr_t)bias & 15) == 0);
+    const int C = ea.head_c;
+    const int c4 = (C + 3) / 4;
+    const int n_end = (ea.row_map && ldy == (int64_t)(4 * c4)) ? 4 * c4 : C;
+    const bool vec_ok = (ldy % 4 == 0) && (((uintptr_t)Y & 15) == 0);
+    auto arrive_leader = [&](uint32_t bar) {
+      if (lane == 0) {
+        if (!leader) mbar_arrive_remote(mapa_rank(bar, 0));
+        else mbar_arrive(bar);
+      }
+    };
+    auto combine = [&](int64_t m, int64_t rb) {
+      bool last = true;
+      if (n_tiles > 1) {
+        asm volatile("bar.sync 5, 128;" ::: "memory");
+        if (quad == 0 && lane == 0) {
+          __threadfence();
+          const int32_t old = atomicAdd(ea.head_cnt + rb, 1);
+          __threadfence();
+          *head_slot = old;
+        }
+        asm volatile("bar.sync 5, 128;" ::: "memory");
+        last = *(volatile int32_t*)head_slot == n_tiles - 1;
+      }
+      if (!last) return;
+      float z[HEAD_PITCH];
+#pragma unroll
+      for (int j = 0; j < HEAD_PITCH / 4; ++j) {
+        if (j >= c4) break;
+        float4 a = __ldcg(reinterpret_cast<const float4*>(ea.head_part + m * HEAD_PITCH) + j);
+        for (int t = 1; t < n_tiles; ++t) {
+          const float4 b = __ldcg(reinterpret_cast<const float4*>(ea.head_part + ((int64_t)t * ea.head_m_pad + m) * HEAD_PITCH) + j);
+          a.x += b.x; a.y += b.y; a.z += b.z; a.w += b.w;
+        }
+        z[4 * j] = a.x; z[4 * j + 1] = a.y; z[4 * j + 2] = a.z; z[4 * j + 3] = a.w;
+      }
+      float mx = -INFINITY;
+#pragma unroll
+      for (int c = 0; c < HEAD_PITCH; ++c)
+        if (c < C) {
+          z[c] += __ldg(ea.head_bias + c);
+          mx = fmaxf(mx, z[c]);
+        }
+      if (head != FITGNN_HEAD_IDENTITY) {
+        float sum = 0.f;
+#pragma unroll
+        for (int c = 0; c < HEAD_PITCH; ++c)
+          if (c < C) sum += __expf(z[c] - mx);
+        const float log_sum = logf(sum), inv_sum = 1.f / sum;
+#pragma unroll
+        for (int c = 0; c < HEAD_PITCH; ++c)
+          z[c] = head == FITGNN_HEAD_LOG_SOFTMAX ? z[c] - mx - log_sum : __expf(z[c] - mx) * inv_sum;
+      }
+#pragma unroll
+      for (int c = 0; c < HEAD_PITCH; ++c)
+        if (c >= C) z[c] = 0.f;
+      const int64_t dest = (m < M) ? (ea.row_map ? (int64_t)__ldg(ea.row_map + m) : m) : -1;
+      if (dest >= 0) {
+        float* y = Y + dest * ldy;
+#pragma unroll
+        for (int j = 0; j < HEAD_PITCH; j += 4) {
+          if (vec_ok && j + 4 <= n_end) {
+            *reinterpret_cast<float4*>(y + j) = make_float4(z[j], z[j + 1], z[j + 2], z[j + 3]);
+          } else {
+#pragma unroll
+            for (int u = 0; u < 4; ++u)
+              if (j + u < n_end) y[j + u] = z[j + u];
+          }
+        }
+      }
+    };
+    int64_t pend_rb = -1;
+    uint32_t it = 0;
+    for (Walk w = w0; valid(w); ++it, advance(w)) {
+      const uint32_t acc = it % ACC_STAGES;
+      const uint32_t acc_phase = (it / ACC_STAGES) & 1u;
+      const int64_t m = tile_row0(w) + row_in_tile;
+      const int n0 = w.nt * BLOCK_N;
+      const float rs = (ea.row_scale && m < M) ? __ldg(ea.row_scale + m) : 1.f;
+      mbar_wait(tfull_bar(acc), acc_phase);
+      fence_after();
+      const uint32_t tst = tmem_base + ((uint32_t)(quad * 32) << 16) + acc * BLOCK_N;
+      for (int i = 0; i < n_box; ++i) {
+        const int box = grp == 1 ? box_beg + n_box - 1 - i : box_beg + i;
+        const int c0 = box * 32;
+        uint32_t r[32];
+        tmem_ld32_issue(tst + c0, r);
+        tmem_ld32_wait(r);
+        float v[32];
+#pragma unroll
+        for (int j = 0; j < 32; j += 4) {
+          const float4 b4 = !bias ? make_float4(0.f, 0.f, 0.f, 0.f)
+                            : bias_vec ? __ldg(reinterpret_cast<const float4*>(bias + n0 + c0 + j))
+                                       : make_float4(__ldg(bias + n0 + c0 + j), __ldg(bias + n0 + c0 + j + 1),
+                                                     __ldg(bias + n0 + c0 + j + 2), __ldg(bias + n0 + c0 + j + 3));
+          const float x[4] = {__uint_as_float(r[j]), __uint_as_float(r[j + 1]), __uint_as_float(r[j + 2]), __uint_as_float(r[j + 3])};
+          const float bb[4] = {b4.x, b4.y, b4.z, b4.w};
+#pragma unroll
+          for (int u = 0; u < 4; ++u) v[j + u] = ea.row_scale ? fmaf(x[u], rs, bb[u]) : (bias ? x[u] + bb[u] : x[u]);
+        }
+        if (act == FITGNN_ACT_ELU) {
+#pragma unroll
+          for (int j = 0; j < 32; ++j) v[j] = elu1(v[j]);
+        }
+        uint32_t h[16];
+#pragma unroll
+        for (int u = 0; u < 16; ++u) h[u] = pack_f16x2_rn(v[2 * u], v[2 * u + 1]);
+        tmem_st16(tst + (uint32_t)head_a_col(c0), h);
+      }
+      tmem_wait_st();
+      fence_before();
+      __syncwarp();
+      arrive_leader(aready_bar(acc));
+      if (grp != 2) {
+        arrive_leader(tempty_bar(acc));
+        continue;
+      }
+      if (pend_rb >= 0) combine(pend_rb * BLOCK_M + (row_in_tile & (BLOCK_M - 1)), pend_rb);
+      pend_rb = -1;
+      mbar_wait(hfull_bar(acc), acc_phase);
+      fence_after();
+      float* part = ea.head_part + ((int64_t)w.nt * ea.head_m_pad + m) * HEAD_PITCH;
+      for (int c0 = 0; c0 < HEAD_PITCH; c0 += 16) {
+        float p[16];
+        tmem_ld16(tst + HEAD_COL + c0, p);
+#pragma unroll
+        for (int j = 0; j < 16; j += 4)
+          if (c0 + j < 4 * c4) *reinterpret_cast<float4*>(part + c0 + j) = make_float4(p[j], p[j + 1], p[j + 2], p[j + 3]);
+      }
+      fence_before();
+      __syncwarp();
+      arrive_leader(tempty_bar(acc));
+      if (!(ea.debug & 2)) pend_rb = tile_row0(w) >> 7;
+    }
+    if (pend_rb >= 0) combine(pend_rb * BLOCK_M + (row_in_tile & (BLOCK_M - 1)), pend_rb);
   } else {
     const int quad = warp & 3;
     const int row_in_tile = quad * 32 + lane;
@@ -1199,6 +1431,86 @@
 #undef FG_TC
 }
 
+static size_t head_fused_part_bytes(int64_t M, int N) {
+  const int64_t m_pad = ceil_div(M, 2 * tc::BLOCK_M) * 2 * tc::BLOCK_M;
+  return ((size_t)ceil_div(N, 256) * (size_t)m_pad * tc::HEAD_PITCH * 4 + 255) / 256 * 256;
+}
+size_t gemm_f16_head_fused_workspace_bytes(int64_t M, int N) {
+  const int64_t m_pad = ceil_div(M, 2 * tc::BLOCK_M) * 2 * tc::BLOCK_M;
+  return head_fused_part_bytes(M, N) + (size_t)(m_pad / tc::BLOCK_M) * 4;
+}
+
+int gemm_f16_head_fused(const void* A, int64_t lda, const void* W, int64_t ldw, const float* row_scale, const float* bias,
+                        int64_t M, int K, int N, int act, const void* Wl_hi, const void* Wl_lo, int64_t ldwl, const float* bl,
+                        int C, int head, const int32_t* row_map, float* Y, int64_t ldy, void* workspace, size_t ws_bytes,
+                        cudaStream_t st) {
+  using namespace tc;
+  FG_REQUIRE(N % 256 == 0 && N / 256 <= 2, FITGNN_EUNSUP, "gemm_f16_head_fused: hidden width must be 256 or 512 (got %d)", N);
+  FG_REQUIRE(K % BLOCK_K == 0, FITGNN_EUNSUP, "gemm_f16_head_fused: K must be a multiple of 64 (got %d)", K);
+  FG_REQUIRE(C >= 1 && (C + 3) / 4 * 4 <= HEAD_MAX_C, FITGNN_EUNSUP, "gemm_f16_head_fused: 1..%d classes (got %d)", HEAD_MAX_C, C);
+  FG_REQUIRE(ws_bytes >= gemm_f16_head_fused_workspace_bytes(M, N) && ((uintptr_t)workspace & 15) == 0, FITGNN_EWS,
+             "gemm_f16_head_fused: workspace too small or not 16-byte aligned");
+  FG_REQUIRE(M < (1ll << 31) - 256, FITGNN_ERANGE, "gemm_f16_head_fused: M exceeds the TMA coordinate range");
+  int sms = sm_count() - tuning().sm_reserve;
+  if (sms < 2) sms = 2;
+  const int n_tiles = N / 256;
+  const int64_t m_pair_tiles = ceil_div(M, 2 * BLOCK_M);
+  const int k_blocks = K / BLOCK_K;
+  const size_t w_res = (size_t)k_blocks * 128 * BLOCK_K * 2;
+  const size_t FIXED = 1024 + 256;
+  constexpr size_t SMEM_LIMIT = 227 * 1024;
+  FG_REQUIRE(w_res + HEAD_W_BYTES + 2 * A_PLANE_BYTES + FIXED <= SMEM_LIMIT, FITGNN_EUNSUP,
+             "gemm_f16_head_fused: K = %d leaves no room for two A stages beside the resident weights", K);
+  int n_stages = (int)((SMEM_LIMIT - FIXED - w_res - HEAD_W_BYTES) / A_PLANE_BYTES);
+  if (n_stages > 8) n_stages = 8;
+  const size_t smem = w_res + HEAD_W_BYTES + (size_t)n_stages * A_PLANE_BYTES + FIXED;
+  int64_t pairs = m_pair_tiles * n_tiles < sms / 2 ? m_pair_tiles * n_tiles : sms / 2;
+  pairs = pairs / n_tiles * n_tiles;
+  FG_REQUIRE(pairs >= n_tiles, FITGNN_EUNSUP, "gemm_f16_head_fused: needs at least %d SM pairs", n_tiles);
+
+  CUtensorMap a_map, w_map, wl_hi, wl_lo;
+  FG_TRY(make_map(&a_map, A, M, K, lda, BLOCK_M));
+  FG_TRY(make_map(&w_map, W, N, K, ldw, BLOCK_M));
+  FG_TRY(make_map(&wl_hi, Wl_hi, C, N, ldwl, HEAD_N / 2));
+  FG_TRY(make_map(&wl_lo, Wl_lo, C, N, ldwl, HEAD_N / 2));
+  int32_t* cnt = reinterpret_cast<int32_t*>(static_cast<uint8_t*>(workspace) + head_fused_part_bytes(M, N));
+  FG_CUDA(cudaMemsetAsync(cnt, 0, (size_t)(m_pair_tiles * 2) * 4, st));
+  const GatherArgs ga{};
+  EpiArgs ea{};
+  ea.row_map = row_map;
+  ea.row_scale = row_scale;
+  ea.a_planes = 1;
+  ea.f16 = 1;
+  ea.w_planes = 1;
+  ea.l2_prefetch = tuning().gemm_prefetch;
+  ea.head_bias = bl;
+  ea.head_c = C;
+  ea.head_m_pad = m_pair_tiles * 2 * BLOCK_M;
+  ea.head_part = static_cast<float*>(workspace);
+  ea.head_cnt = cnt;
+
+  auto kern = gemm_bf16x3_kernel<256, false, 0, EPI_WARPS_12, true, true>;
+  static bool smem_configured = false;
+  if (!smem_configured) {
+    FG_CUDA(cudaFuncSetAttribute(kern, cudaFuncAttributeMaxDynamicSharedMemorySize, (int)SMEM_LIMIT));
+    smem_configured = true;
+  }
+  cudaLaunchConfig_t cfg = {};
+  cfg.gridDim = dim3((unsigned)(2 * pairs));
+  cfg.blockDim = dim3(64 + 32 * EPI_WARPS_12);
+  cfg.dynamicSmemBytes = smem;
+  cfg.stream = st;
+  cudaLaunchAttribute attr[1];
+  attr[0].id = cudaLaunchAttributeClusterDimension;
+  attr[0].val.clusterDim.x = 2;
+  attr[0].val.clusterDim.y = 1;
+  attr[0].val.clusterDim.z = 1;
+  cfg.attrs = attr;
+  cfg.numAttrs = 1;
+  FG_CUDA(cudaLaunchKernelEx(&cfg, kern, ga, ea, a_map, a_map, w_map, w_map, wl_hi, wl_lo, 0, bias, M, K, N, act, head, Y, ldy,
+                             1, n_stages));
+  return FITGNN_OK;
+}
 
 int gcn_layer_fused(const int32_t* rowptr, const int32_t* col, const float* dinv, const float* X, int64_t ldx, int width,
                     const int32_t* src_index, const int32_t* out_rows, int64_t M, const void* W_hi, const void* W_lo,
diff --git a/fitgnn_b200/engine.py b/fitgnn_b200/engine.py
--- a/fitgnn_b200/engine.py
+++ b/fitgnn_b200/engine.py
@@ -16,7 +16,7 @@
 
     def __init__(self, pack: Pack, state_dict, head="log_softmax", rows="core", precision="bf16x3",
                  with_head=True, fuse_layer0=False, fuse_aggregate="auto", align_policy="degree", out_map=None,
-                 blocked_spmm="auto", dense_spmm="lds", conv_fused=False):
+                 blocked_spmm="auto", dense_spmm="lds", conv_fused=False, head_fused=True):
         if precision not in ("bf16x3", "fp32", "fp16x2", "fp16"):
             raise ValueError(f"precision={precision!r}")
         self.pack = pack
@@ -113,6 +113,12 @@
         cf = os.environ.get("FITGNN_CONV_FUSED", "")
         conv_fused = {"0": False, "1": True}.get(cf, conv_fused)
         self.conv_fused = bool(conv_fused) and self.f16_hidden and self.apack is not None and self.H > 128
+        hf = os.environ.get("FITGNN_HEAD_FUSED", "")
+        head_fused = {"0": False, "1": True}.get(hf, head_fused)
+        self.head_fused = (bool(head_fused) and self.f16_hidden and self.w_single and self.apack is not None
+                           and not self.conv_fused and self.H % 256 == 0 and self.H <= 512 and ops.pad4(self.C) <= 48
+                           and self.Wl[1] is not None)
+        self._head_ws = None
         self.out_map = None
         if out_map is not None:
             assert with_head, "out_map needs the head"
@@ -304,6 +310,21 @@
                     nbytes=4 * (M * Ki + Ki * self.H + M * self.H) + 12 * M, flops=2 * M * Ki * self.H)
             K = self.H
         i = self.L - 1
+        if self.head_fused and peer_ptrs is None:
+            self.launches += 1
+            view = None
+            if out is None:
+                out = torch.empty(self.n_out, ops.pad4(self.C), dtype=torch.float32, device=X.device)
+                view = out[:, : self.C]
+            if self._head_ws is None or self._head_ws.device != X.device:
+                self._head_ws = ops.gemm_f16_head_fused_workspace(M, self.H, X.device)
+            self._timed(f"gemm{i}_head", lambda: ops.gemm_f16_head_fused(
+                A, self.W[i], self.b[i], ops.ACT_ELU, self.Wl, self.bl, self.head, out,
+                row_scale=ap.dinv if self.defer_scale else None, row_map=self._head_map, workspace=self._head_ws,
+                K=K, N=self.H, C=self.C),
+                nbytes=2 * M * K + 2 * K * self.H + 4 * self.H * self.C + 4 * self.n_out * self.C + 4 * M,
+                flops=2 * M * K * self.H + 2 * M * self.H * self.C)
+            return out if view is None else view
         if self.f16_hidden:
             self.launches += 2
             h = self._timed(f"gemm{i}", lambda: ops.gemm_f16(A, self.W[i], self.b[i], ops.ACT_ELU, row_scale=ap.dinv if self.defer_scale else None,
diff --git a/fitgnn_b200/ops.py b/fitgnn_b200/ops.py
--- a/fitgnn_b200/ops.py
+++ b/fitgnn_b200/ops.py
@@ -494,6 +494,27 @@
     return out
 
 
+def gemm_f16_head_fused_workspace(M, N, device):
+    nbytes = int(lib().fitgnn_gemm_f16_head_fused_workspace_bytes(M, N))
+    return torch.empty(max(nbytes, 16), dtype=torch.uint8, device=device)
+
+
+def gemm_f16_head_fused(A, W, bias, act, Wl, bl, head, out, row_scale=None, row_map=None, workspace=None, K=None, N=None, C=None):
+    w_hi, w_lo = W
+    wl_hi, wl_lo = Wl
+    assert A.dtype == torch.float16 and w_hi.dtype == torch.float16 and w_lo is None and wl_lo is not None
+    M = A.shape[0]
+    K = A.shape[1] if K is None else K
+    N = w_hi.shape[0] if N is None else N
+    C = wl_hi.shape[0] if C is None else C
+    if workspace is None:
+        workspace = gemm_f16_head_fused_workspace(M, N, A.device)
+    check(lib().fitgnn_gemm_f16_head_fused(ptr(A), A.stride(0), ptr(w_hi), w_hi.stride(0), ptr(row_scale), ptr(bias), M, K, N, act,
+                                           ptr(wl_hi), ptr(wl_lo), wl_hi.stride(0), ptr(bl), C, head, ptr(row_map), ptr(out),
+                                           out.stride(0), ptr(workspace), workspace.numel(), stream_ptr()))
+    return out
+
+
 def gemm_f16_head_rows_peers(A, W, bias, act, head, row_map, peer_ptrs, ldy, K=None, N=None):
     w_hi, w_lo = W
     M = A.shape[0]
diff --git a/include/fitgnn.h b/include/fitgnn.h
--- a/include/fitgnn.h
+++ b/include/fitgnn.h
@@ -151,6 +151,11 @@
                                     const float* bias, int64_t M, int K, int N, int act, int head,
                                     const int32_t* row_map, float* const* host_peer_bases, int n_peers,
                                     int64_t ldy, void* stream);
+size_t fitgnn_gemm_f16_head_fused_workspace_bytes(int64_t M, int N);
+int fitgnn_gemm_f16_head_fused(const void* A, int64_t lda, const void* W, int64_t ldw, const float* row_scale,
+                               const float* bias, int64_t M, int K, int N, int act, const void* Wl_hi, const void* Wl_lo,
+                               int64_t ldwl, const float* bl, int C, int head, const int32_t* row_map, float* Y, int64_t ldy,
+                               void* workspace, size_t ws_bytes, void* stream);
 int fitgnn_gcn_transform_aggregate_f16(int in_f16, const void* A_hi, const void* A_lo, int64_t lda, const void* W_hi,
                                        const void* W_lo, int64_t ldw, const float* bias, int64_t M, int K, int N,
                                        int act, const uint64_t* agg_desc, const float* dinv, int defer_row_scale,
```

New measurement: 453.5 million (median of 6 runs). 0.597x the previous value.
